# fwereade/trivy

Measured on AMD Instinct MI355X. Metric: packages matched/sec (node), higher is better.
Workload: dtype u8; 1 GPU; c2-dpkg-10000x400; packages=4000000, packages_rank0=4000000, matches_rank0=20482442, kernel_variant=fused_k4_m2400_wseg_rec_r16, db_keys=150005, db_advisories=1709707

## Files before the change

### include/trivy_amd.h

```cpp
#ifndef TRIVY_AMD_H
#define TRIVY_AMD_H

#include <stddef.h>
#include <stdint.h>

#ifdef __cplusplus
extern "C" {
#endif

#define TVM_ABI_VERSION 1

enum {
  TVM_OK = 0,
  TVM_EDETECT = 1,
  TVM_EUNSUPPORTED_OS = 2,
  TVM_EINVAL = 3,
  TVM_EDEVICE = 4,
  TVM_EUNSUPPORTED_TYPE = 5,
};

typedef struct tvm_db tvm_db;
typedef struct tvm_engine tvm_engine;
typedef struct tvm_batch tvm_batch;

typedef struct {
  const char* p;
  size_t n;
} tvm_str;

typedef struct {
  tvm_str id, name, version, release, arch;
  int64_t epoch;
  tvm_str src_name, src_version, src_release;
  int64_t src_epoch;
  tvm_str modularitylabel;
  int32_t has_build_info;
  const tvm_str* content_sets;
  size_t n_content_sets;
  tvm_str nvr, build_arch;
  tvm_str file_path;
} tvm_package;

typedef struct {
  tvm_str family, release;
} tvm_repository;

enum {
  TVM_COPY_PKG_ID = 1,
  TVM_COPY_PKG_NAME = 2,
  TVM_COPY_IDENTIFIER = 4,
  TVM_COPY_LAYER = 8,
};

typedef struct {
  uint32_t pkg_index;
  uint32_t copy_flags;
  const char* vulnerability_id;
  const char* const* vendor_ids;
  size_t n_vendor_ids;
  const char* pkg_id;
  const char* pkg_name;
  const char* pkg_path;
  const char* installed_version;
  const char* fixed_version;
  int32_t status;
  const char* severity_source;
  const char* severity;
  int32_t has_data_source;
  const char* data_source_id;
  const char* data_source_name;
  const char* data_source_url;
  const char* custom_json;
} tvm_vuln;

typedef struct {
  tvm_vuln* vulns;
  size_t n;
  int32_t eosl;
  void* priv;
} tvm_result;

const char* tvm_version(void);
int tvm_abi_version(void);

tvm_db* tvm_db_new(void);
void tvm_db_free(tvm_db* db);
int tvm_db_put(tvm_db* db, const tvm_str* path, size_t depth, const char* value, size_t vlen);
int tvm_db_put_many(tvm_db* db, size_t n, const tvm_str* paths, size_t depth, const tvm_str* values);
int tvm_db_put_arena(tvm_db* db, size_t n, size_t depth, const char* arena, const uint64_t* off,
                     const uint32_t* len);
int tvm_db_put_bbolt(tvm_db* db, const void* bytes, size_t len, char* err, size_t errlen);
typedef int (*tvm_bbolt_visit)(void* ctx, const tvm_str* path, size_t depth, const char* value, size_t vlen);
int tvm_bbolt_walk(const void* bytes, size_t len, tvm_bbolt_visit visit, void* ctx, char* err, size_t errlen);
int tvm_db_finalize(tvm_db* db, char* err, size_t errlen);
void tvm_db_stats(const tvm_db* db, uint64_t out[5]);
void tvm_db_layout_stats(const tvm_db* db, uint64_t out[6]);
void tvm_db_row16_stats(const tvm_db* db, uint64_t out[10]);
int tvm_row16_eval_host(const tvm_db* db, const char* bucket, const char* name, size_t name_len, const char* version,
                        size_t version_len, uint8_t* path, uint8_t* result, size_t cap);
int tvm_row16_pair_host(const uint8_t* key, size_t key_len, int valid, uint64_t pfx, uint32_t row_adv, uint32_t row_tail,
                        uint64_t row_head, int lex);

tvm_engine* tvm_engine_open(tvm_db* db, int device, char* err, size_t errlen);
void tvm_engine_close(tvm_engine* e);
int tvm_engine_swap(tvm_engine* e, tvm_db* db, char* err, size_t errlen);
uint64_t tvm_engine_table_bytes(const tvm_engine* e);
int tvm_engine_dropin_stats(tvm_engine* e, uint64_t* out3);
int tvm_engine_verify(tvm_engine* e, char* err, size_t errlen);
int tvm_engine_set_variant(tvm_engine* e, int v);
const char* tvm_variant_name(int v);
int tvm_variant_grammar_sets(int v);
int tvm_engine_last_variant(tvm_engine* e);

int tvm_ospkg_detect(tvm_engine* e, const char* os_family, const char* os_name, const tvm_repository* repo,
                     const tvm_package* pkgs, size_t n, int64_t now_unix, tvm_result* out, char* err,
                     size_t errlen);
int tvm_ospkg_driver_detect(tvm_engine* e, const char* os_family, const char* os_ver, const tvm_repository* repo,
                            const tvm_package* pkgs, size_t n, int64_t now_unix, tvm_result* out, char* err,
                            size_t errlen);
int tvm_ospkg_is_supported(const char* os_family, const char* os_ver, int64_t now_unix);
void tvm_result_free(tvm_result* r);

const char* tvm_library_type(const char* lib_type);
int tvm_library_detect(tvm_engine* e, const char* lib_type, const tvm_package* pkgs, size_t n, tvm_result* out,
                       char* err, size_t errlen);
int tvm_library_detect_vulnerabilities(tvm_engine* e, const char* lib_type, tvm_str pkg_id, tvm_str pkg_name,
                                       tvm_str pkg_ver, tvm_result* out, char* err, size_t errlen);

tvm_batch* tvm_batch_new(void);
void tvm_batch_free(tvm_batch* b);
int64_t tvm_batch_add(tvm_batch* b, tvm_engine* e, const char* bucket, tvm_str name, tvm_str version);
enum { TVM_ATTR_ARCH = 1, TVM_ATTR_KSPLICE = 2, TVM_ATTR_CPESET = 4 };
int64_t tvm_batch_add_many_ex(tvm_batch* b, tvm_engine* e, const char* bucket, size_t n, const char* arena,
                              const uint64_t* name_off, const uint32_t* name_len, const uint64_t* ver_off,
                              const uint32_t* ver_len, const uint64_t* arch_off, const uint32_t* arch_len,
                              uint32_t flags);
int64_t tvm_batch_cpe_set(tvm_batch* b, tvm_engine* e, const tvm_str* content_sets, size_t n, tvm_str nvr);
typedef struct {
  const uint64_t* arch_off;
  const uint32_t* arch_len;
  const uint32_t* cpe_set;
} tvm_attr_cols;
int64_t tvm_batch_add_many_attrs(tvm_batch* b, tvm_engine* e, const char* bucket, size_t n, const char* arena,
                                 const uint64_t* name_off, const uint32_t* name_len, const uint64_t* ver_off,
                                 const uint32_t* ver_len, const tvm_attr_cols* attrs, uint32_t flags);
int64_t tvm_batch_add_many(tvm_batch* b, tvm_engine* e, const char* bucket, size_t n, const char* arena,
                           const uint64_t* name_off, const uint32_t* name_len, const uint64_t* ver_off,
                           const uint32_t* ver_len);
int64_t tvm_batch_add_targets(tvm_batch* b, tvm_engine* e, size_t n_targets, const tvm_str* buckets,
                              const uint64_t* target_end, const char* arena, const uint64_t* name_off,
                              const uint32_t* name_len, const uint64_t* ver_off, const uint32_t* ver_len);
int64_t tvm_batch_add_targets_attrs(tvm_batch* b, tvm_engine* e, size_t n_targets, const tvm_str* buckets,
                                    const uint32_t* target_flags, const uint64_t* target_end, const char* arena,
                                    const uint64_t* name_off, const uint32_t* name_len, const uint64_t* ver_off,
                                    const uint32_t* ver_len, const tvm_attr_cols* attrs);
int64_t tvm_batch_size(const tvm_batch* b);
int tvm_batch_upload(tvm_engine* e, tvm_batch* b, uint64_t match_cap, char* err, size_t errlen);
int tvm_match_launch(tvm_engine* e, tvm_batch* b, char* err, size_t errlen);
int tvm_engine_sync(tvm_engine* e, char* err, size_t errlen);
int tvm_device_sync(int device, char* err, size_t errlen);
void tvm_shutdown(void);
int tvm_match_status(tvm_engine* e, tvm_batch* b, uint64_t* n_matches, int64_t* err_pkg, uint64_t* err_bits);
int tvm_match_fetch(tvm_engine* e, tvm_batch* b, uint32_t* pairs, uint64_t cap, uint64_t* n_out);
int tvm_match_copy_device(tvm_engine* e, tvm_batch* b, void* dst, uint64_t cap, uint64_t* n_out);
int tvm_match_order_into(tvm_engine* e, tvm_batch* b, void* csr_adv_dev, void* row_end_dev, uint64_t cap,
                         uint64_t* n_out, char* err, size_t errlen);
int tvm_match_time(tvm_engine* e, tvm_batch* b, int steps, double* ms, char* err, size_t errlen);
uint64_t tvm_match_algorithmic_bytes(tvm_engine* e, tvm_batch* b);
int tvm_version_key(int grammar, const char* s, size_t n, uint8_t* out, size_t cap);
int tvm_version_class(int grammar, const char* s, size_t n);
int tvm_deb_fast_key_host(const char* s, size_t n, uint32_t shift, uint8_t* out, size_t cap);
int tvm_deb_fast_key_slot_host(const char* s, size_t n, uint32_t shift, uint8_t* kb, size_t kb_len);
int tvm_enc_bal_buckets_host(void);
int tvm_enc_bal_bucket_host(uint32_t version_len);
int tvm_enc_bal_item_host(const uint32_t* counts, uint32_t item, uint32_t* bucket, uint32_t* index);
enum { TVM_ISVULN_PAIRWISE = 0x100 };
int tvm_lib_is_vulnerable_host(int grammar, const char* ver, size_t ver_len, const char* advisory_json,
                               size_t json_len);
const char* tvm_db_advisory_vuln_id(const tvm_db* db, uint32_t adv);

int tvm_db_rows_many(const tvm_db* db, const char* bucket, size_t n, const char* arena, const uint64_t* name_off,
                     const uint32_t* name_len, uint32_t* out);
int tvm_batch_set_package_base(tvm_batch* b, uint32_t base);
int tvm_batch_upload_into(tvm_engine* e, tvm_batch* b, void* pkg_dev, void* adv_dev, uint64_t cap, char* err,
                          size_t errlen);

enum { TVM_PIPE_RAW = 1, TVM_PIPE_ADV32 = 2, TVM_PIPE_RH_MERGE = 4 };
int tvm_pipeline_prepare(tvm_engine* e, tvm_batch* b, uint64_t match_cap, uint32_t chunk_packages, uint32_t flags,
                         char* err, size_t errlen);
int tvm_pipeline_run(tvm_engine* e, tvm_batch* b, uint64_t* n_matches, int64_t* err_pkg, double* ms, char* err,
                     size_t errlen);
int tvm_pipeline_result(tvm_batch* b, const uint32_t** adv, const uint32_t** row_end, uint64_t* n_matches);
int tvm_pipeline_result_raw(tvm_batch* b, const void** adv, uint32_t* width, const uint32_t** row_end,
                            uint64_t* n_matches);
int tvm_pipeline_stats(tvm_batch* b, uint64_t out[5]);
int tvm_wire_encode(size_t n, const uint32_t* plat, const char* arena, const uint64_t* name_off, const uint32_t* name_len,
                    const uint64_t* ver_off, const uint32_t* ver_len, uint32_t chunk_packages, int threads, void* out,
                    uint64_t cap, uint64_t* bytes,
                    uint64_t* chunks, uint64_t chunks_cap, uint64_t* n_chunks, uint32_t* plats, uint32_t plats_cap,
                    uint32_t* n_plats);
int tvm_pipeline_times(tvm_batch* b, uint64_t* encode_us, uint64_t* prepare_us);
void tvm_pool_stats(uint64_t out[4]);
void tvm_pool_trim(void);
int tvm_runtime_info(int* hip_runtime, int* hip_driver, char* path, size_t pathlen);

typedef struct tvm_sbom tvm_sbom;
enum { TVM_SBOM_BORROW = 1 };
int tvm_sbom_decode_cyclonedx(const char* text, size_t len, uint32_t flags, tvm_sbom** out, char* err, size_t errlen);
void tvm_sbom_free(tvm_sbom* s);
int tvm_sbom_info(const tvm_sbom* s, int32_t* has_os, tvm_str* os_family, tvm_str* os_name, tvm_str* serial,
                  int64_t* version, size_t* n_apps);
int tvm_sbom_packages(const tvm_sbom* s, int64_t app, tvm_str* type, tvm_str* file_path, const tvm_package** pkgs,
                      size_t* n);
typedef struct {
  tvm_str purl, bom_ref, layer_digest, layer_diff_id;
  uint32_t present;
} tvm_sbom_extra;
int tvm_sbom_package_extra(const tvm_sbom* s, int64_t app, size_t i, tvm_sbom_extra* out);

int tvm_match_redhat_result(tvm_engine* e, tvm_batch* b, tvm_result* out, char* err, size_t errlen);
int tvm_match_redhat_merge(tvm_engine* e, tvm_batch* b, char* err, size_t errlen);
int tvm_match_redhat_vulns(tvm_engine* e, tvm_batch* b, const uint32_t* pairs, uint64_t n, tvm_result* out,
                           char* err, size_t errlen);
int tvm_match_redhat_merge_time(tvm_engine* e, tvm_batch* b, int steps, double* ms, char* err, size_t errlen);

typedef struct {
  const uint32_t* row_end;
  size_t n_pkgs;
  uint32_t first_pkg;
  const uint8_t* rec;
  uint32_t rec_width;
  size_t n;
  const tvm_vuln* adv_recs;
  size_t n_adv_recs;
  const tvm_vuln* grp_recs;
  size_t n_grp_recs;
  void* priv;
} tvm_vuln_set;
int tvm_match_vulns(tvm_engine* e, tvm_batch* b, tvm_vuln_set* out, char* err, size_t errlen);
int tvm_pipeline_vulns(tvm_engine* e, tvm_batch* b, tvm_vuln_set* out, char* err, size_t errlen);
void tvm_vuln_set_free(tvm_vuln_set* s);
int tvm_vuln_set_walk(const tvm_vuln_set* s, const tvm_batch* b, uint64_t* n_out, uint64_t* digest);
int tvm_batch_report_get(const tvm_batch* b, uint64_t first, uint64_t n, tvm_str* names, tvm_str* versions,
                         tvm_str* paths);

typedef struct {
  tvm_str vulnerability_id;
  tvm_str data_source_id;
  tvm_str severity_source;
  tvm_str severity;
  int32_t status;
  int32_t has_fixed_version;
} tvm_fill_in;
typedef struct {
  int32_t found;
  int32_t status;
  const char* severity;
  const char* severity_source;
  const char* primary_url;
  const char* vulnerability_json;
} tvm_fill_out;
typedef struct {
  tvm_fill_out* items;
  size_t n;
  void* priv;
} tvm_fill_result;
int tvm_fill_info(tvm_engine* e, const tvm_fill_in* in, size_t n, tvm_fill_result* out, char* err, size_t errlen);
void tvm_fill_result_free(tvm_fill_result* r);
int tvm_match_fill(tvm_engine* e, tvm_batch* b, char* err, size_t errlen);
int tvm_match_fill_fetch(tvm_engine* e, tvm_batch* b, uint32_t* out4, uint64_t cap, uint64_t* n_out);
int tvm_match_fill_time(tvm_engine* e, tvm_batch* b, int steps, double* ms, char* err, size_t errlen);
uint64_t tvm_match_fill_algorithmic_bytes(tvm_engine* e, tvm_batch* b);
const char* tvm_fill_source_name(tvm_engine* e, uint32_t id);

int tvm_batch_set_report(tvm_batch* b, uint64_t first, uint64_t n, const tvm_str* names, const tvm_str* versions,
                         const tvm_str* paths);

typedef struct {
  const tvm_str* ids;
  size_t n_ids;
  const uint32_t* id_ranks;
  const uint32_t* all_id;
  const uint32_t* all_prec;
  size_t n_all;
  const uint32_t* pkg_pkg;
  const uint32_t* pkg_id;
  const uint32_t* pkg_prec;
  size_t n_pkg;
  const uint32_t* pkg_class;
  const uint32_t* cls_class;
  const uint32_t* cls_id;
  const uint32_t* cls_prec;
  size_t n_cls;
} tvm_ignore_rules;

typedef struct {
  uint32_t severity_mask;
  uint32_t ignore_status_mask;
  const tvm_ignore_rules* ignore;
  const uint32_t* vex_pkgs;
  const uint32_t* vex_id_index;
  size_t n_vex;
  const tvm_str* vex_ids;
  size_t n_vex_ids;
  const uint32_t* vex_id_ranks;
} tvm_filter_opts;
int tvm_vuln_rank_many(tvm_engine* e, const tvm_str* ids, size_t n, uint32_t* ranks);
int tvm_match_filter(tvm_engine* e, tvm_batch* b, const tvm_filter_opts* o, uint64_t* n_kept, uint64_t* n_ignored,
                     char* err, size_t errlen);
int tvm_match_filter_fetch(tvm_engine* e, tvm_batch* b, uint32_t* pairs, uint64_t cap, uint64_t* n_out);
int tvm_match_filter_ignored(tvm_engine* e, tvm_batch* b, uint32_t* triples, uint64_t cap, uint64_t* n_out);
int tvm_match_filter_time(tvm_engine* e, tvm_batch* b, const tvm_filter_opts* o, int steps, double* ms, char* err,
                          size_t errlen);

int tvm_pipeline_set_filter(tvm_engine* e, tvm_batch* b, const tvm_filter_opts* o, char* err, size_t errlen);
int tvm_pipeline_filter_stats(tvm_batch* b, uint64_t out[2]);

#ifdef __cplusplus
}
#endif
#endif
```

### trivy_amd/_lib.py

```python
import atexit
import ctypes
import os

_HERE = os.path.dirname(os.path.abspath(__file__))
LIB_PATH = os.environ.get("TVM_LIB_PATH") or os.path.join(_HERE, "libtrivy_amd.so")

TVM_OK, TVM_EDETECT, TVM_EUNSUPPORTED_OS, TVM_EINVAL, TVM_EDEVICE, TVM_EUNSUPPORTED_TYPE = 0, 1, 2, 3, 4, 5
COPY_PKG_ID, COPY_PKG_NAME, COPY_IDENTIFIER, COPY_LAYER = 1, 2, 4, 8


class Str(ctypes.Structure):
    _fields_ = [("p", ctypes.c_char_p), ("n", ctypes.c_size_t)]


class Package(ctypes.Structure):
    _fields_ = [
        ("id", Str), ("name", Str), ("version", Str), ("release", Str), ("arch", Str),
        ("epoch", ctypes.c_int64),
        ("src_name", Str), ("src_version", Str), ("src_release", Str),
        ("src_epoch", ctypes.c_int64),
        ("modularitylabel", Str),
        ("has_build_info", ctypes.c_int32),
        ("content_sets", ctypes.POINTER(Str)), ("n_content_sets", ctypes.c_size_t),
        ("nvr", Str), ("build_arch", Str),
        ("file_path", Str),
    ]


class RawStr(ctypes.Structure):
    _fields_ = [("p", ctypes.c_void_p), ("n", ctypes.c_size_t)]

    def bytes(self):
        return ctypes.string_at(self.p, self.n) if self.n else b""


class RawPackage(ctypes.Structure):
    _fields_ = [(n, RawStr if t is Str else t) for n, t in Package._fields_]


class SbomExtra(ctypes.Structure):
    _fields_ = [("purl", RawStr), ("bom_ref", RawStr), ("layer_digest", RawStr), ("layer_diff_id", RawStr),
                ("present", ctypes.c_uint32)]


class Repository(ctypes.Structure):
    _fields_ = [("family", Str), ("release", Str)]


class Vuln(ctypes.Structure):
    _fields_ = [
        ("pkg_index", ctypes.c_uint32), ("copy_flags", ctypes.c_uint32),
        ("vulnerability_id", ctypes.c_char_p),
        ("vendor_ids", ctypes.POINTER(ctypes.c_char_p)), ("n_vendor_ids", ctypes.c_size_t),
        ("pkg_id", ctypes.c_char_p), ("pkg_name", ctypes.c_char_p), ("pkg_path", ctypes.c_char_p),
        ("installed_version", ctypes.c_char_p), ("fixed_version", ctypes.c_char_p),
        ("status", ctypes.c_int32),
        ("severity_source", ctypes.c_char_p), ("severity", ctypes.c_char_p),
        ("has_data_source", ctypes.c_int32),
        ("data_source_id", ctypes.c_char_p), ("data_source_name", ctypes.c_char_p),
        ("data_source_url", ctypes.c_char_p),
        ("custom_json", ctypes.c_char_p),
    ]


class VulnSet(ctypes.Structure):
    _fields_ = [("row_end", ctypes.POINTER(ctypes.c_uint32)), ("n_pkgs", ctypes.c_size_t),
                ("first_pkg", ctypes.c_uint32), ("rec", ctypes.c_void_p), ("rec_width", ctypes.c_uint32),
                ("n", ctypes.c_size_t), ("adv_recs", ctypes.POINTER(Vuln)), ("n_adv_recs", ctypes.c_size_t),
                ("grp_recs", ctypes.POINTER(Vuln)), ("n_grp_recs", ctypes.c_size_t), ("priv", ctypes.c_void_p)]


class AttrCols(ctypes.Structure):
    _fields_ = [("arch_off", ctypes.c_void_p), ("arch_len", ctypes.c_void_p), ("cpe_set", ctypes.c_void_p)]


class Result(ctypes.Structure):
    _fields_ = [("vulns", ctypes.POINTER(Vuln)), ("n", ctypes.c_size_t), ("eosl", ctypes.c_int32),
                ("priv", ctypes.c_void_p)]


class FillIn(ctypes.Structure):
    _fields_ = [("vulnerability_id", Str), ("data_source_id", Str), ("severity_source", Str), ("severity", Str),
                ("status", ctypes.c_int32), ("has_fixed_version", ctypes.c_int32)]


class FillOut(ctypes.Structure):
    _fields_ = [("found", ctypes.c_int32), ("status", ctypes.c_int32), ("severity", ctypes.c_char_p),
                ("severity_source", ctypes.c_char_p), ("primary_url", ctypes.c_char_p),
                ("vulnerability_json", ctypes.c_char_p)]


class FillResult(ctypes.Structure):
    _fields_ = [("items", ctypes.POINTER(FillOut)), ("n", ctypes.c_size_t), ("priv", ctypes.c_void_p)]


class IgnoreRulesC(ctypes.Structure):
    _fields_ = [("ids", ctypes.POINTER(Str)), ("n_ids", ctypes.c_size_t), ("id_ranks", ctypes.c_void_p),
                ("all_id", ctypes.c_void_p), ("all_prec", ctypes.c_void_p), ("n_all", ctypes.c_size_t),
                ("pkg_pkg", ctypes.c_void_p), ("pkg_id", ctypes.c_void_p), ("pkg_prec", ctypes.c_void_p),
                ("n_pkg", ctypes.c_size_t), ("pkg_class", ctypes.c_void_p),
                ("cls_class", ctypes.c_void_p), ("cls_id", ctypes.c_void_p), ("cls_prec", ctypes.c_void_p),
                ("n_cls", ctypes.c_size_t)]


class FilterOpts(ctypes.Structure):
    _fields_ = [("severity_mask", ctypes.c_uint32), ("ignore_status_mask", ctypes.c_uint32),
                ("ignore", ctypes.POINTER(IgnoreRulesC)),
                ("vex_pkgs", ctypes.c_void_p), ("vex_id_index", ctypes.c_void_p), ("n_vex", ctypes.c_size_t),
                ("vex_ids", ctypes.POINTER(Str)), ("n_vex_ids", ctypes.c_size_t), ("vex_id_ranks", ctypes.c_void_p)]


_P = ctypes.c_void_p
_SIG = [
    ("tvm_version", ctypes.c_char_p, []),
    ("tvm_abi_version", ctypes.c_int, []),
    ("tvm_db_new", _P, []),
    ("tvm_db_free", None, [_P]),
    ("tvm_db_put", ctypes.c_int, [_P, ctypes.POINTER(Str), ctypes.c_size_t, ctypes.c_char_p, ctypes.c_size_t]),
    ("tvm_db_put_many", ctypes.c_int, [_P, ctypes.c_size_t, ctypes.c_void_p, ctypes.c_size_t, ctypes.c_void_p]),
    ("tvm_db_put_bbolt", ctypes.c_int, [_P, ctypes.c_char_p, ctypes.c_size_t, ctypes.c_char_p, ctypes.c_size_t]),
    ("tvm_bbolt_walk", ctypes.c_int, [ctypes.c_char_p, ctypes.c_size_t, ctypes.c_void_p, ctypes.c_void_p,
                                      ctypes.c_char_p, ctypes.c_size_t]),
    ("tvm_db_put_arena", ctypes.c_int, [_P, ctypes.c_size_t, ctypes.c_size_t, ctypes.c_void_p, ctypes.c_void_p,
                                        ctypes.c_void_p]),
    ("tvm_db_finalize", ctypes.c_int, [_P, ctypes.c_char_p, ctypes.c_size_t]),
    ("tvm_db_stats", None, [_P, ctypes.POINTER(ctypes.c_uint64)]),
    ("tvm_db_layout_stats", None, [_P, ctypes.POINTER(ctypes.c_uint64)]),
    ("tvm_db_row16_stats", None, [_P, ctypes.POINTER(ctypes.c_uint64)]),
    ("tvm_row16_eval_host", ctypes.c_int, [_P, ctypes.c_char_p, ctypes.c_char_p, ctypes.c_size_t, ctypes.c_char_p,
                                           ctypes.c_size_t, ctypes.c_void_p, ctypes.c_void_p, ctypes.c_size_t]),
    ("tvm_row16_pair_host", ctypes.c_int, [ctypes.c_char_p, ctypes.c_size_t, ctypes.c_int, ctypes.c_uint64, ctypes.c_uint32,
                                           ctypes.c_uint32, ctypes.c_uint64, ctypes.c_int]),
    ("tvm_engine_open", _P, [_P, ctypes.c_int, ctypes.c_char_p, ctypes.c_size_t]),
    ("tvm_engine_close", None, [_P]),
    ("tvm_engine_swap", ctypes.c_int, [_P, _P, ctypes.c_char_p, ctypes.c_size_t]),
    ("tvm_engine_table_bytes", ctypes.c_uint64, [_P]),
    ("tvm_engine_verify", ctypes.c_int, [_P, ctypes.c_char_p, ctypes.c_size_t]),
    ("tvm_engine_set_variant", ctypes.c_int, [_P, ctypes.c_int]),
    ("tvm_variant_name", ctypes.c_char_p, [ctypes.c_int]),
    ("tvm_variant_grammar_sets", ctypes.c_int, [ctypes.c_int]),
    ("tvm_engine_last_variant", ctypes.c_int, [_P]),
    ("tvm_ospkg_detect", ctypes.c_int, [_P, ctypes.c_char_p, ctypes.c_char_p, ctypes.POINTER(Repository),
                                        ctypes.POINTER(Package), ctypes.c_size_t, ctypes.c_int64,
                                        ctypes.POINTER(Result), ctypes.c_char_p, ctypes.c_size_t]),
    ("tvm_ospkg_driver_detect", ctypes.c_int, [_P, ctypes.c_char_p, ctypes.c_char_p, ctypes.POINTER(Repository),
                                               ctypes.POINTER(Package), ctypes.c_size_t, ctypes.c_int64,
                                               ctypes.POINTER(Result), ctypes.c_char_p, ctypes.c_size_t]),
    ("tvm_ospkg_is_supported", ctypes.c_int, [ctypes.c_char_p, ctypes.c_char_p, ctypes.c_int64]),
    ("tvm_result_free", None, [ctypes.POINTER(Result)]),
    ("tvm_batch_new", _P, []),
    ("tvm_batch_free", None, [_P]),
    ("tvm_batch_add", ctypes.c_int64, [_P, _P, ctypes.c_char_p, Str, Str]),
    ("tvm_batch_add_many", ctypes.c_int64, [_P, _P, ctypes.c_char_p, ctypes.c_size_t, ctypes.c_void_p,
                                             ctypes.c_void_p, ctypes.c_void_p, ctypes.c_void_p, ctypes.c_void_p]),
    ("tvm_batch_add_many_ex", ctypes.c_int64, [_P, _P, ctypes.c_char_p, ctypes.c_size_t, ctypes.c_char_p, ctypes.c_void_p,
                                               ctypes.c_void_p, ctypes.c_void_p, ctypes.c_void_p, ctypes.c_void_p,
                                               ctypes.c_void_p, ctypes.c_uint32]),
    ("tvm_batch_size", ctypes.c_int64, [_P]),
    ("tvm_batch_add_targets", ctypes.c_int64, [_P, _P, ctypes.c_size_t, ctypes.POINTER(Str), ctypes.c_void_p,
                                               ctypes.c_char_p, ctypes.c_void_p, ctypes.c_void_p, ctypes.c_void_p,
                                               ctypes.c_void_p]),
    ("tvm_batch_add_targets_attrs", ctypes.c_int64, [_P, _P, ctypes.c_size_t, ctypes.POINTER(Str), ctypes.c_void_p,
                                                     ctypes.c_void_p, ctypes.c_char_p, ctypes.c_void_p, ctypes.c_void_p,
                                                     ctypes.c_void_p, ctypes.c_void_p, ctypes.c_void_p]),
    ("tvm_batch_cpe_set", ctypes.c_int64, [_P, _P, ctypes.c_void_p, ctypes.c_size_t, Str]),
    ("tvm_batch_add_many_attrs", ctypes.c_int64, [_P, _P, ctypes.c_char_p, ctypes.c_size_t, ctypes.c_char_p,
                                                  ctypes.c_void_p, ctypes.c_void_p, ctypes.c_void_p, ctypes.c_void_p,
                                                  ctypes.c_void_p, ctypes.c_uint32]),
    ("tvm_match_redhat_result", ctypes.c_int, [_P, _P, ctypes.POINTER(Result), ctypes.c_char_p, ctypes.c_size_t]),
    ("tvm_match_redhat_merge", ctypes.c_int, [_P, _P, ctypes.c_char_p, ctypes.c_size_t]),
    ("tvm_match_redhat_merge_time", ctypes.c_int, [_P, _P, ctypes.c_int, ctypes.POINTER(ctypes.c_double),
                                                   ctypes.c_char_p, ctypes.c_size_t]),
    ("tvm_match_redhat_vulns", ctypes.c_int, [_P, _P, _P, ctypes.c_uint64, ctypes.POINTER(Result), ctypes.c_char_p,
                                              ctypes.c_size_t]),
    ("tvm_batch_upload", ctypes.c_int, [_P, _P, ctypes.c_uint64, ctypes.c_char_p, ctypes.c_size_t]),
    ("tvm_match_launch", ctypes.c_int, [_P, _P, ctypes.c_char_p, ctypes.c_size_t]),
    ("tvm_engine_sync", ctypes.c_int, [_P, ctypes.c_char_p, ctypes.c_size_t]),
    ("tvm_device_sync", ctypes.c_int, [ctypes.c_int, ctypes.c_char_p, ctypes.c_size_t]),
    ("tvm_shutdown", None, []),
    ("tvm_pipeline_times", ctypes.c_int, [_P, ctypes.POINTER(ctypes.c_uint64), ctypes.POINTER(ctypes.c_uint64)]),
    ("tvm_pool_stats", None, [ctypes.POINTER(ctypes.c_uint64)]),
    ("tvm_sbom_decode_cyclonedx", ctypes.c_int, [ctypes.c_void_p, ctypes.c_size_t, ctypes.c_uint32,
                                                 ctypes.POINTER(ctypes.c_void_p),
                                                 ctypes.c_char_p, ctypes.c_size_t]),
    ("tvm_sbom_free", None, [ctypes.c_void_p]),
    ("tvm_sbom_info", ctypes.c_int, [ctypes.c_void_p, ctypes.POINTER(ctypes.c_int32), ctypes.POINTER(RawStr),
                                     ctypes.POINTER(RawStr), ctypes.POINTER(RawStr), ctypes.POINTER(ctypes.c_int64),
                                     ctypes.POINTER(ctypes.c_size_t)]),
    ("tvm_sbom_packages", ctypes.c_int, [ctypes.c_void_p, ctypes.c_int64, ctypes.POINTER(RawStr), ctypes.POINTER(RawStr),
                                         ctypes.POINTER(ctypes.POINTER(RawPackage)), ctypes.POINTER(ctypes.c_size_t)]),
    ("tvm_sbom_package_extra", ctypes.c_int, [ctypes.c_void_p, ctypes.c_int64, ctypes.c_size_t,
                                              ctypes.POINTER(SbomExtra)]),
    ("tvm_wire_encode", ctypes.c_int, [ctypes.c_size_t, ctypes.c_void_p, ctypes.c_char_p, ctypes.c_void_p,
                                       ctypes.c_void_p, ctypes.c_void_p, ctypes.c_void_p,
                                       ctypes.c_uint32, ctypes.c_int, ctypes.c_void_p, ctypes.c_uint64,
                                       ctypes.POINTER(ctypes.c_uint64), ctypes.c_void_p, ctypes.c_uint64,
                                       ctypes.POINTER(ctypes.c_uint64), ctypes.c_void_p, ctypes.c_uint32,
                                       ctypes.POINTER(ctypes.c_uint32)]),
    ("tvm_pool_trim", None, []),
    ("tvm_match_status", ctypes.c_int, [_P, _P, ctypes.POINTER(ctypes.c_uint64), ctypes.POINTER(ctypes.c_int64),
                                        ctypes.POINTER(ctypes.c_uint64)]),
    ("tvm_match_fetch", ctypes.c_int, [_P, _P, ctypes.c_void_p, ctypes.c_uint64, ctypes.POINTER(ctypes.c_uint64)]),
    ("tvm_match_copy_device", ctypes.c_int, [_P, _P, ctypes.c_void_p, ctypes.c_uint64, ctypes.POINTER(ctypes.c_uint64)]),
    ("tvm_match_order_into", ctypes.c_int, [_P, _P, ctypes.c_void_p, ctypes.c_void_p, ctypes.c_uint64,
                                            ctypes.POINTER(ctypes.c_uint64), ctypes.c_char_p, ctypes.c_size_t]),
    ("tvm_match_time", ctypes.c_int, [_P, _P, ctypes.c_int, ctypes.POINTER(ctypes.c_double), ctypes.c_char_p,
                                      ctypes.c_size_t]),
    ("tvm_match_algorithmic_bytes", ctypes.c_uint64, [_P, _P]),
    ("tvm_db_rows_many", ctypes.c_int, [_P, ctypes.c_char_p, ctypes.c_size_t, ctypes.c_void_p, ctypes.c_void_p,
                                        ctypes.c_void_p, ctypes.c_void_p]),
    ("tvm_batch_set_package_base", ctypes.c_int, [_P, ctypes.c_uint32]),
    ("tvm_batch_upload_into", ctypes.c_int, [_P, _P, ctypes.c_void_p, ctypes.c_void_p, ctypes.c_uint64,
                                             ctypes.c_char_p, ctypes.c_size_t]),
    ("tvm_pipeline_prepare", ctypes.c_int, [_P, _P, ctypes.c_uint64, ctypes.c_uint32, ctypes.c_uint32, ctypes.c_char_p,
                                            ctypes.c_size_t]),
    ("tvm_pipeline_run", ctypes.c_int, [_P, _P, ctypes.POINTER(ctypes.c_uint64), ctypes.POINTER(ctypes.c_int64),
                                        ctypes.POINTER(ctypes.c_double), ctypes.c_char_p, ctypes.c_size_t]),
    ("tvm_pipeline_result", ctypes.c_int, [_P, ctypes.POINTER(ctypes.c_void_p), ctypes.POINTER(ctypes.c_void_p),
                                           ctypes.POINTER(ctypes.c_uint64)]),
    ("tvm_pipeline_result_raw", ctypes.c_int, [_P, ctypes.POINTER(ctypes.c_void_p), ctypes.POINTER(ctypes.c_uint32),
                                               ctypes.POINTER(ctypes.c_void_p), ctypes.POINTER(ctypes.c_uint64)]),
    ("tvm_pipeline_stats", ctypes.c_int, [_P, ctypes.POINTER(ctypes.c_uint64)]),
    ("tvm_version_key", ctypes.c_int, [ctypes.c_int, ctypes.c_char_p, ctypes.c_size_t, ctypes.c_void_p,
                                       ctypes.c_size_t]),
    ("tvm_engine_dropin_stats", ctypes.c_int, [_P, ctypes.POINTER(ctypes.c_uint64)]),
    ("tvm_deb_fast_key_host", ctypes.c_int, [ctypes.c_char_p, ctypes.c_size_t, ctypes.c_uint32, ctypes.c_void_p,
                                             ctypes.c_size_t]),
    ("tvm_deb_fast_key_slot_host", ctypes.c_int, [ctypes.c_char_p, ctypes.c_size_t, ctypes.c_uint32, ctypes.c_void_p,
                                                  ctypes.c_size_t]),
    ("tvm_enc_bal_buckets_host", ctypes.c_int, []),
    ("tvm_enc_bal_bucket_host", ctypes.c_int, [ctypes.c_uint32]),
    ("tvm_enc_bal_item_host", ctypes.c_int, [ctypes.POINTER(ctypes.c_uint32), ctypes.c_uint32,
                                             ctypes.POINTER(ctypes.c_uint32), ctypes.POINTER(ctypes.c_uint32)]),
    ("tvm_db_advisory_vuln_id", ctypes.c_char_p, [_P, ctypes.c_uint32]),
    ("tvm_version_class", ctypes.c_int, [ctypes.c_int, ctypes.c_char_p, ctypes.c_size_t]),
    ("tvm_lib_is_vulnerable_host", ctypes.c_int, [ctypes.c_int, ctypes.c_char_p, ctypes.c_size_t, ctypes.c_char_p,
                                                  ctypes.c_size_t]),
    ("tvm_library_type", ctypes.c_char_p, [ctypes.c_char_p]),
    ("tvm_library_detect", ctypes.c_int, [_P, ctypes.c_char_p, ctypes.POINTER(Package), ctypes.c_size_t,
                                          ctypes.POINTER(Result), ctypes.c_char_p, ctypes.c_size_t]),
    ("tvm_library_detect_vulnerabilities", ctypes.c_int, [_P, ctypes.c_char_p, Str, Str, Str, ctypes.POINTER(Result),
                                                          ctypes.c_char_p, ctypes.c_size_t]),
    ("tvm_fill_info", ctypes.c_int, [_P, ctypes.POINTER(FillIn), ctypes.c_size_t, ctypes.POINTER(FillResult),
                                     ctypes.c_char_p, ctypes.c_size_t]),
    ("tvm_fill_result_free", None, [ctypes.POINTER(FillResult)]),
    ("tvm_match_fill", ctypes.c_int, [_P, _P, ctypes.c_char_p, ctypes.c_size_t]),
    ("tvm_match_fill_fetch", ctypes.c_int, [_P, _P, ctypes.c_void_p, ctypes.c_uint64, ctypes.POINTER(ctypes.c_uint64)]),
    ("tvm_match_fill_time", ctypes.c_int, [_P, _P, ctypes.c_int, ctypes.POINTER(ctypes.c_double), ctypes.c_char_p,
                                           ctypes.c_size_t]),
    ("tvm_match_fill_algorithmic_bytes", ctypes.c_uint64, [_P, _P]),
    ("tvm_fill_source_name", ctypes.c_char_p, [_P, ctypes.c_uint32]),
    ("tvm_match_filter", ctypes.c_int, [_P, _P, ctypes.POINTER(FilterOpts), ctypes.POINTER(ctypes.c_uint64),
                                        ctypes.POINTER(ctypes.c_uint64), ctypes.c_char_p, ctypes.c_size_t]),
    ("tvm_match_filter_fetch", ctypes.c_int, [_P, _P, ctypes.c_void_p, ctypes.c_uint64,
                                              ctypes.POINTER(ctypes.c_uint64)]),
    ("tvm_match_filter_ignored", ctypes.c_int, [_P, _P, ctypes.c_void_p, ctypes.c_uint64,
                                                ctypes.POINTER(ctypes.c_uint64)]),
    ("tvm_vuln_rank_many", ctypes.c_int, [_P, ctypes.POINTER(Str), ctypes.c_size_t, ctypes.c_void_p]),
    ("tvm_batch_set_report", ctypes.c_int, [_P, ctypes.c_uint64, ctypes.c_uint64, ctypes.POINTER(Str),
                                            ctypes.POINTER(Str), ctypes.POINTER(Str)]),
    ("tvm_match_vulns", ctypes.c_int, [_P, _P, ctypes.POINTER(VulnSet), ctypes.c_char_p, ctypes.c_size_t]),
    ("tvm_runtime_info", ctypes.c_int, [ctypes.c_void_p, ctypes.c_void_p, ctypes.c_char_p, ctypes.c_size_t]),
    ("tvm_vuln_set_walk", ctypes.c_int, [ctypes.POINTER(VulnSet), _P, ctypes.c_void_p, ctypes.c_void_p]),
    ("tvm_pipeline_vulns", ctypes.c_int, [_P, _P, ctypes.POINTER(VulnSet), ctypes.c_char_p, ctypes.c_size_t]),
    ("tvm_vuln_set_free", None, [ctypes.POINTER(VulnSet)]),
    ("tvm_batch_report_get", ctypes.c_int, [_P, ctypes.c_uint64, ctypes.c_uint64, ctypes.POINTER(RawStr),
                                            ctypes.POINTER(RawStr), ctypes.POINTER(RawStr)]),
    ("tvm_match_filter_time", ctypes.c_int, [_P, _P, ctypes.POINTER(FilterOpts), ctypes.c_int,
                                             ctypes.POINTER(ctypes.c_double), ctypes.c_char_p, ctypes.c_size_t]),
    ("tvm_pipeline_set_filter", ctypes.c_int, [_P, _P, ctypes.POINTER(FilterOpts), ctypes.c_char_p, ctypes.c_size_t]),
    ("tvm_pipeline_filter_stats", ctypes.c_int, [_P, ctypes.POINTER(ctypes.c_uint64)]),
]

EXPORTED = [s[0] for s in _SIG]

_lib = None


def lib():
    global _lib
    if _lib is None:
        if not os.path.exists(LIB_PATH):
            raise RuntimeError(f"trivy_amd native library not built: {LIB_PATH} (run __graft_entry__.build())")
        L = ctypes.CDLL(LIB_PATH)
        for name, res, args in _SIG:
            f = getattr(L, name)
            f.restype = res
            f.argtypes = args
        _lib = L
        atexit.register(L.tvm_shutdown)
    return _lib


def s(x):
    if x is None:
        return Str(None, 0)
    b = x.encode() if isinstance(x, str) else bytes(x)
    st = Str(b, len(b))
    st._keep = b
    return st


def errbuf():
    return ctypes.create_string_buffer(4096)


def runtime_info():
    rt, drv, path = ctypes.c_int(), ctypes.c_int(), ctypes.create_string_buffer(1024)
    lib().tvm_runtime_info(ctypes.byref(rt), ctypes.byref(drv), path, len(path))
    fmt = lambda v: f"{v // 10_000_000}.{v // 100_000 % 100}.{v % 100_000}"
    return {"hip_runtime": fmt(rt.value), "hip_driver": fmt(drv.value), "libamdhip64": path.value.decode()}
```

### trivy_amd/csrc/capi.cpp

```cpp
#include "../../include/trivy_amd.h"

#include <dlfcn.h>

#include <algorithm>
#include <atomic>
#include <chrono>
#include <cstdio>
#include <cstring>
#include <deque>
#include <memory>
#include <mutex>
#include <new>
#include <shared_mutex>
#include <string>
#include <unordered_map>
#include <vector>

#include "db.h"
#include "drivers.h"
#include "export.h"
#include "engine.h"
#include "libdb.h"
#include "libver.h"
#include "bbolt.h"
// ... 321 lines not shown
      if (!(r.hi_len & KEY_INF)) {
        const int c = key_cmp(kw.data(), kl, d.key_words.data() + o.hi_off, r.hi_len & KEY_LEN_MASK);
        m = (r.hi_len & KEY_INCL) ? c <= 0 : c < 0;
      }
      if (m && !(r.lo_len & KEY_INF)) {
        const int c = key_cmp(kw.data(), kl, d.key_words.data() + o.lo_off, r.lo_len & KEY_LEN_MASK);
        m = (r.lo_len & KEY_INCL) ? c >= 0 : c > 0;
      }
      m = (m && valid) || (r.adv & ROW_ALWAYS);
    }
    if (path) path[i] = (h.tail & 0xFFu) == R16_FALLBACK ? 2 : slow ? 1 : 0;
    if (result) result[i] = m ? 1 : 0;
  }
  return int(cnt);
}

int tvm_row16_pair_host(const uint8_t* key, size_t key_len, int valid, uint64_t pfx, uint32_t row_adv, uint32_t row_tail,
                        uint64_t row_head, int lex) {
  if ((!key && key_len) || key_len > 0x3FFF) return -1;
  uint64_t k[3] = {0, 0, 0};
  for (size_t i = 0; i < key_len && i < 24; i++) k[i / 8] |= uint64_t(key[i]) << (8 * (7 - i % 8));
  const uint32_t kl = valid ? uint32_t(key_len) : 0u, P = uint32_t(pfx) & 0xFFu;
  if (!valid) k[0] = k[1] = k[2] = 0;
  Row16 r;
  r.adv = row_adv;
  r.tail = row_tail;
  r.head = row_head;
  uint64_t ph;
  uint32_t pt;
  bool slow = false, m;
  if (lex) {
    row16_pkg_lex(k[0], k[1], k[2], kl, P, row16_prefix_cmp(k[0], kl, pfx), valid != 0, ph, pt);
    m = row16_test_lex(ph, pt, r, slow);
  } else {
    row16_pkg(k[0], k[1], k[2], kl, P, row16_prefix_cmp(k[0], kl, pfx), valid != 0, ph, pt);
    m = row16_test(ph, pt, r, slow);
  }
  return (m ? 1 : 0) | (slow ? 2 : 0);
}

const char* tvm_db_advisory_vuln_id(const tvm_db* db, uint32_t adv) {
  return adv < db->db.advs.size() ? db->db.advs[adv].vuln_id.c_str() : nullptr;
}

static std::atomic<uint64_t> g_used_devices{0};

tvm_engine* tvm_engine_open(tvm_db* db, int device, char* err, size_t errlen) {
  if (device >= 0 && device < 64) g_used_devices.fetch_or(uint64_t(1) << device);
  if (!db || !db->finalized) {
    set_err(err, errlen, "tvm_engine_open: DB not finalized");
    return nullptr;
  }
  std::string e;
  Engine* eng = Engine::open(db->db, device, e);
  if (!eng) {
    set_err(err, errlen, e);
    return nullptr;
  }
  FillEngine* fill = FillEngine::open(db->vt, device, e);
  if (!fill) {
    delete eng;
    set_err(err, errlen, e);
    return nullptr;
  }
  auto* t = new tvm_engine();
  t->eng.reset(eng);
  t->fill.reset(fill);
  t->db = db;
  t->device = device;
  return t;
}

void tvm_engine_close(tvm_engine* e) { delete e; }

void tvm_shutdown(void) {
  const uint64_t used = g_used_devices.load();
  for (int d = 0; d < 64; d++)
    if ((used >> d) & 1u)
      if (hipSetDevice(d) == hipSuccess) (void)hipDeviceSynchronize();
  WorkerPool::shutdown_all();
  release_encoders();
  pool_close();
}

int tvm_device_sync(int device, char* err, size_t errlen) {
  int ndev = 0;
  if (hipGetDeviceCount(&ndev) != hipSuccess || device < 0 || device >= ndev) {
    set_err(err, errlen, "tvm_device_sync: no such HIP device");
    return TVM_EDEVICE;
  }
  (void)hipSetDevice(device);
  hipError_t st = hipDeviceSynchronize();
  if (st == hipSuccess) st = hipGetLastError();
  if (st != hipSuccess) {
    set_err(err, errlen, std::string("tvm_device_sync: ") + hipGetErrorString(st));
    return TVM_EDEVICE;
  }
  return TVM_OK;
}

int tvm_engine_swap(tvm_engine* e, tvm_db* db, char* err, size_t errlen) {
  if (!e || !db || !db->finalized) return TVM_EINVAL;
  std::string msg;
  Engine* fresh = Engine::open(db->db, e->device, msg);
  FillEngine* fresh_fill = fresh ? FillEngine::open(db->vt, e->device, msg) : nullptr;
  if (!fresh || !fresh_fill) {
    delete fresh;
    set_err(err, errlen, msg);
    return TVM_EDEVICE;
  }
  std::unique_lock<std::shared_mutex> lk(e->mu);
  (void)hipSetDevice(e->device);
  e->eng.reset(fresh);
  e->fill.reset(fresh_fill);
  e->db = db;
  e->gen++;
  if (e->rh_rank) {
    (void)hipFree(e->rh_rank);
    e->rh_rank = nullptr;
  }
  if (e->cls) {
    (void)hipFree(e->cls);
    e->cls = nullptr;
  }
  return TVM_OK;
}

uint64_t tvm_engine_table_bytes(const tvm_engine* e) { return e ? e->eng->table_bytes() : 0; }

int tvm_engine_dropin_stats(tvm_engine* e, uint64_t* out3) {
  if (!e || !out3) return TVM_EINVAL;
  std::shared_lock<std::shared_mutex> lk(e->mu);
  e->eng->dropin_stats(out3);
  return TVM_OK;
}

int tvm_engine_verify(tvm_engine* e, char* err, size_t errlen) {
  if (!e) return TVM_EINVAL;
  std::unique_lock<std::shared_mutex> lk(e->mu);
  std::string msg;
  if (!e->eng->verify(msg)) {
    set_err(err, errlen, msg);
    return TVM_EDEVICE;
  }
  return TVM_OK;
}

int tvm_engine_set_variant(tvm_engine* e, int v) {
  if (!e) return -1;
  std::unique_lock<std::shared_mutex> lk(e->mu);
  return v < 0 ? e->eng->variant() : e->eng->set_variant(v);
}

const char* tvm_variant_name(int v) { return variant_name(v); }
int tvm_variant_grammar_sets(int v) { return variant_grammar_sets(v); }

int tvm_engine_last_variant(tvm_engine* e) {
  if (!e) return -1;
  std::shared_lock<std::shared_mutex> lk(e->mu);
  return e->eng->last_launched();
}

static int detect_common(tvm_engine* e, bool full, const char* fam, const char* ver, const tvm_repository* repo,
                         const tvm_package* pkgs, size_t n, int64_t now, tvm_result* out, char* err,
                         size_t errlen) {
  if (!e || !fam || !ver || !out || (n && !pkgs)) return TVM_EINVAL;
  memset(out, 0, sizeof(*out));
  std::shared_lock<std::shared_mutex> lk(e->mu);
  std::vector<Pkg> p = to_pkgs(pkgs, n);
  Repo r;
  if (repo) {
    r.family = sv(repo->family);
    r.release = sv(repo->release);
  }
  std::vector<Vuln> vulns;
  std::string msg;
  bool eosl = false;
  if (full) {
    DetectStatus st = ospkg_detect(*e->eng, fam, ver, repo ? &r : nullptr, p, now, vulns, eosl, msg);
    if (st != DETECT_OK) {
      set_err(err, errlen, msg);
      return st == DETECT_UNSUPPORTED_OS ? TVM_EUNSUPPORTED_OS : TVM_EDETECT;
    }
  } else {
    const OsDriver* d = find_os_driver(fam);
    if (!d) {
      set_err(err, errlen, "unsupported os");
      return TVM_EUNSUPPORTED_OS;
    }
    if (!d->detect(*e->eng, ver, repo ? &r : nullptr, p, now, vulns, msg)) {
      set_err(err, errlen, msg);
      return TVM_EDETECT;
    }
  }
  export_result(e->eng->db(), std::move(vulns), eosl, out);
  return TVM_OK;
}

int tvm_ospkg_detect(tvm_engine* e, const char* f, const char* v, const tvm_repository* repo, const tvm_package* pkgs,
                     size_t n, int64_t now, tvm_result* out, char* err, size_t errlen) {
  return detect_common(e, true, f, v, repo, pkgs, n, now, out, err, errlen);
}

int tvm_ospkg_driver_detect(tvm_engine* e, const char* f, const char* v, const tvm_repository* repo,
                            const tvm_package* pkgs, size_t n, int64_t now, tvm_result* out, char* err,
                            size_t errlen) {
  return detect_common(e, false, f, v, repo, pkgs, n, now, out, err, errlen);
}

int tvm_ospkg_is_supported(const char* fam, const char* ver, int64_t now) {
  const OsDriver* d = fam ? find_os_driver(fam) : nullptr;
  if (!d || !ver) return -1;
  return d->is_supported(fam, ver, now) ? 1 : 0;
}

void tvm_result_free(tvm_result* r) {
  if (!r) return;
  delete static_cast<ResultStore*>(r->priv);
  memset(r, 0, sizeof(*r));
}


tvm_batch* tvm_batch_new(void) { return new tvm_batch(); }

void tvm_batch_free(tvm_batch* b) {
  if (!b) return;
  b->pipe.reset();
  if (b->order_scratch) {
    (void)hipSetDevice(b->device);
    (void)hipFree(b->order_scratch);
  }
  if (b->uploaded) {
    (void)hipSetDevice(b->device);
    for (void* p : {static_cast<void*>(b->dev.pk), static_cast<void*>(b->dev.tile_off), static_cast<void*>(b->dev.arena),
                    static_cast<void*>(b->dev.attr), static_cast<void*>(b->dev.cpe_bits), static_cast<void*>(b->dev.rec),
                    static_cast<void*>(b->dev.tail), static_cast<void*>(b->dev.spill),
                    static_cast<void*>(b->external_out ? nullptr : b->m.pkg),
                    static_cast<void*>(b->external_out ? nullptr : b->m.adv), static_cast<void*>(b->m.dir),
                    static_cast<void*>(b->m.ctl),
                    static_cast<void*>(b->fill_out)})
      if (p) (void)hipFree(p);
  }
  delete b;
}

static void reserve_more(HostBatch& hb, size_t n) {
  const size_t want = hb.pk.size() + n;
  if (want > hb.pk.capacity()) hb.pk.reserve(std::max(want, 2 * hb.pk.capacity()));
}

int64_t tvm_batch_add(tvm_batch* b, tvm_engine* e, const char* bucket, tvm_str name, tvm_str version) {
  if (!b || !e || !bucket || b->uploaded || b->pinned) return -1;
  std::shared_lock<std::shared_mutex> lk(e->mu);
  if (!bind(b, e)) return -1;
  b->target_begin.push_back(uint32_t(b->hb.pk.size()));
  int32_t plat = e->eng->db().find_plat(bucket);
  b->hb.add(plat < 0 ? 0xFFFFFFFFu : uint32_t(plat), sv(name), sv(version));
  return int64_t(b->hb.pk.size() - 1);
}

int64_t tvm_batch_add_many(tvm_batch* b, tvm_engine* e, const char* bucket, size_t n, const char* arena,
                           const uint64_t* name_off, const uint32_t* name_len, const uint64_t* ver_off,
                           const uint32_t* ver_len) {
  if (!b || !e || !bucket || b->uploaded || b->pinned ||
      (n && (!arena || !name_off || !name_len || !ver_off || !ver_len)))
    return -1;
  std::shared_lock<std::shared_mutex> lk(e->mu);
  if (!bind(b, e)) return -1;
  int32_t plat = e->eng->db().find_plat(bucket);
  const uint32_t pid = plat < 0 ? 0xFFFFFFFFu : uint32_t(plat);
  const int64_t first = int64_t(b->hb.pk.size());
  b->target_begin.push_back(uint32_t(first));
  reserve_more(b->hb, n);
  for (size_t i = 0; i < n; i++)
    b->hb.add(pid, std::string_view(arena + name_off[i], name_len[i]), std::string_view(arena + ver_off[i], ver_len[i]));
  return first;
}

int64_t tvm_batch_add_many_ex(tvm_batch* b, tvm_engine* e, const char* bucket, size_t n, const char* arena,
                              const uint64_t* name_off, const uint32_t* name_len, const uint64_t* ver_off,
                              const uint32_t* ver_len, const uint64_t* arch_off, const uint32_t* arch_len,
                              uint32_t flags) {
  if (flags & TVM_ATTR_CPESET) return -1;
  tvm_attr_cols cols{arch_off, arch_len, nullptr};
  return tvm_batch_add_many_attrs(b, e, bucket, n, arena, name_off, name_len, ver_off, ver_len, &cols, flags);
}

int64_t tvm_batch_cpe_set(tvm_batch* b, tvm_engine* e, const tvm_str* content_sets, size_t n, tvm_str nvr) {
  if (!b || !e || b->uploaded || b->pinned || (n && !content_sets)) return -1;
  std::shared_lock<std::shared_mutex> lk(e->mu);
  if (!bind(b, e)) return -1;
  const DB& db = e->eng->db();
  HostBatch& hb = b->hb;
  const uint32_t words = std::max<uint32_t>((db.n_cpe + 31) / 32, 1);
  if (hb.cpe_words == 0) hb.cpe_words = words;
  if (hb.cpe_words != words) return -1;
  std::vector<std::string_view> repos, nvrs;
  for (size_t i = 0; i < n; i++) repos.push_back(sv(content_sets[i]));
  nvrs.push_back(sv(nvr));
  const size_t id = hb.cpe_bits.size() / words;
  hb.cpe_bits.resize(hb.cpe_bits.size() + words, 0u);
  uint32_t* bits = hb.cpe_bits.data() + id * words;
  for (int64_t c : db.redhat_cpes(repos, nvrs))
    if (c >= 0 && uint64_t(c) < uint64_t(words) * 32) bits[c >> 5] |= 1u << (c & 31);
  return int64_t(id);
}

int64_t tvm_batch_add_many_attrs(tvm_batch* b, tvm_engine* e, const char* bucket, size_t n, const char* arena,
                                 const uint64_t* name_off, const uint32_t* name_len, const uint64_t* ver_off,
                                 const uint32_t* ver_len, const tvm_attr_cols* cols, uint32_t flags) {
  const uint32_t known = TVM_ATTR_ARCH | TVM_ATTR_KSPLICE | TVM_ATTR_CPESET;
  if (!b || !e || !bucket || b->uploaded || b->pinned || (flags & ~known) ||
      ((flags & TVM_ATTR_KSPLICE) && (flags & TVM_ATTR_CPESET)) ||
      (n && (!arena || !name_off || !name_len || !ver_off || !ver_len)) ||
      (n && (flags & (TVM_ATTR_ARCH | TVM_ATTR_CPESET)) && !cols) ||
      (n && (flags & TVM_ATTR_ARCH) && (!cols->arch_off || !cols->arch_len)) ||
      (n && (flags & TVM_ATTR_CPESET) && !cols->cpe_set))
    return -1;
  std::shared_lock<std::shared_mutex> lk(e->mu);
  if (!bind(b, e)) return -1;
  const DB& db = e->eng->db();
  const size_t n_sets = b->hb.cpe_words ? b->hb.cpe_bits.size() / b->hb.cpe_words : 0;
  if (flags & TVM_ATTR_CPESET)
    for (size_t i = 0; i < n; i++)
      if (cols->cpe_set[i] >= n_sets) return -1;
  int32_t plat = db.find_plat(bucket);
  const uint32_t pid = plat < 0 ? 0xFFFFFFFFu : uint32_t(plat);
  const int64_t first = int64_t(b->hb.pk.size());
  b->target_begin.push_back(uint32_t(first));
  reserve_more(b->hb, n);
  for (size_t i = 0; i < n; i++) {
    const std::string_view ver(arena + ver_off[i], ver_len[i]);
    uint2 a = make_uint2(PA_ARCH_NONE, 0xFFFFFFFFu);
    if (flags & TVM_ATTR_ARCH) {
      const std::string_view arch(arena + cols->arch_off[i], cols->arch_len[i]);
      a.x = db.arch_id(arch) | (arch == "noarch" ? PA_NOARCH : 0u);
    }
    if (flags & TVM_ATTR_KSPLICE) {
      const size_t dash = ver.find('-');
      a.y = db.ksplice_id(extract_ksplice(dash == std::string_view::npos ? std::string_view() : ver.substr(dash + 1)));
    }
    if (flags & TVM_ATTR_CPESET) a.y = cols->cpe_set[i];
    if (flags) b->hb.add(pid, std::string_view(arena + name_off[i], name_len[i]), ver, a);
    else b->hb.add(pid, std::string_view(arena + name_off[i], name_len[i]), ver);
  }
  return first;
}

static int64_t add_targets_bulk(tvm_batch* b, tvm_engine* e, size_t n_targets, const tvm_str* buckets,
                                const uint32_t* tflags, const uint64_t* target_end, const char* arena,
                                const uint64_t* name_off, const uint32_t* name_len, const uint64_t* ver_off,
                                const uint32_t* ver_len, const tvm_attr_cols* cols) {
  const uint32_t known = TVM_ATTR_ARCH | TVM_ATTR_KSPLICE | TVM_ATTR_CPESET;
  if (!b || !e || b->uploaded || b->pinned || (n_targets && (!buckets || !target_end))) return -1;
  const uint64_t n = n_targets ? target_end[n_targets - 1] : 0;
  if (n && (!arena || !name_off || !name_len || !ver_off || !ver_len)) return -1;
  uint32_t any_flags = 0;
  for (size_t t = 0; t < n_targets; t++) {
    if (t && target_end[t] < target_end[t - 1]) return -1;
    const uint32_t f = tflags ? tflags[t] : 0u;
    if ((f & ~known) || ((f & TVM_ATTR_KSPLICE) && (f & TVM_ATTR_CPESET))) return -1;
    any_flags |= f;
  }
  if (((any_flags & TVM_ATTR_ARCH) && (!cols || !cols->arch_off || !cols->arch_len)) ||
      ((any_flags & TVM_ATTR_CPESET) && (!cols || !cols->cpe_set)))
    return -1;
  std::shared_lock<std::shared_mutex> lk(e->mu);
  if (!bind(b, e)) return -1;
  const DB& db = e->eng->db();
  HostBatch& hb = b->hb;
  const uint64_t s0 = hb.pk.size(), a0 = hb.arena.size();
  if (s0 + n >= (uint64_t(1) << 32)) return -1;
  std::vector<uint32_t> pid(n_targets);
  std::string_view last_bucket;
  uint32_t last_pid = 0xFFFFFFFFu;
  for (size_t t = 0; t < n_targets; t++) {
    const std::string_view bk = sv(buckets[t]);
    if (t == 0 || bk != last_bucket) {
      const int32_t plat = db.find_plat(bk);
      last_pid = plat < 0 ? 0xFFFFFFFFu : uint32_t(plat);
      last_bucket = bk;
    }
    pid[t] = last_pid;
  }
  const size_t n_sets = hb.cpe_words ? hb.cpe_bits.size() / hb.cpe_words : 0;
  WorkerPool& wp = WorkerPool::get();
  const size_t K = n ? std::min<size_t>(size_t(wp.size()) * 8, std::max<uint64_t>(1, n / 4096)) : 0;
  auto piece = [&](size_t k) { return std::make_pair(n * k / K, n * (k + 1) / K); };
  auto target_of = [&](uint64_t j) {
// ... 254 lines not shown
  oa.pkg_base = b->dev.pkg_base;
  if (hipMemsetAsync(b->order_scratch, 0, size_t(nt + 1) * 8, st) != hipSuccess) return TVM_EDEVICE;
  launch_order(nt, st, oa);
  const hipError_t le = hipGetLastError();
  const hipError_t se = le == hipSuccess ? hipStreamSynchronize(st) : le;
  if (se != hipSuccess) {
    set_err(err, errlen, std::string("order kernel: ") + hipGetErrorString(se));
    return TVM_EDEVICE;
  }
  return TVM_OK;
}

int tvm_match_time(tvm_engine* e, tvm_batch* b, int steps, double* ms, char* err, size_t errlen) {
  if (!e || !b || !b->uploaded || steps <= 0 || !ms) return TVM_EINVAL;
  std::shared_lock<std::shared_mutex> lk(e->mu);
  if (!bind(b, e)) {
    set_err(err, errlen, kStale);
    return TVM_EINVAL;
  }
  (void)hipSetDevice(e->device);
  hipEvent_t t0 = nullptr, t1 = nullptr;
  hipStream_t st = e->eng->stream();
  std::string msg;
  int rc = TVM_OK;
  if (hipEventCreate(&t0) != hipSuccess || hipEventCreate(&t1) != hipSuccess || hipEventRecord(t0, st) != hipSuccess) {
    msg = "hipEvent setup failed";
    rc = TVM_EDEVICE;
  }
  b->merged = false;
  b->st_valid = false;
  for (int i = 0; rc == TVM_OK && i < steps; i++)
    if (!e->eng->launch(b->dev, b->m, st, msg)) rc = TVM_EDEVICE;
  float f = 0;
  if (rc == TVM_OK && (hipEventRecord(t1, st) != hipSuccess || hipEventSynchronize(t1) != hipSuccess ||
                       hipEventElapsedTime(&f, t0, t1) != hipSuccess)) {
    msg = "hipEvent timing failed";
    rc = TVM_EDEVICE;
  }
  if (t0) (void)hipEventDestroy(t0);
  if (t1) (void)hipEventDestroy(t1);
  if (rc != TVM_OK) {
    set_err(err, errlen, msg);
    return rc;
  }
  *ms = f;
  return TVM_OK;
}

uint64_t tvm_match_algorithmic_bytes(tvm_engine* e, tvm_batch* b) {
  if (!e || !b) return 0;
  const DB& db = e->eng->db();
  uint64_t bytes = 0, off = 0;
  for (const uint2& d : b->hb.pk) {
    const uint32_t nlen = d.y & 0xFFFF, vlen = d.y >> 16;
    const std::string_view name(reinterpret_cast<const char*>(b->hb.arena.data()) + off, nlen);
    off += nlen + vlen;
    bytes += 8 + nlen + vlen;
    if (d.x >= db.plats.size()) continue;
    bytes += 24;
    int32_t k = db.find_key(d.x, name);
    if (k < 0) continue;
    bytes += nlen;
    const std::string ks = db.keys[size_t(k)].name;
    uint64_t h = pkg_key_hash(d.x, reinterpret_cast<const uint8_t*>(ks.data()), uint32_t(ks.size()));
    for (uint64_t i = h & db.slot_mask; db.slot_hash[i]; i = (i + 1) & db.slot_mask) {
      if (db.slot_key[i] != uint32_t(k)) continue;
      const SlotVal& v = db.slot_val[i];
      uint32_t cls = 0;
      if (v.name_len & SLOT_CLS_SPLIT) {
        struct Sink {
          void put(uint8_t) {}
        } sk;
        const char* ver = name.data() + nlen;
        if (!encode_version_cls(db.plat_info[d.x].cmp, reinterpret_cast<const uint8_t*>(ver), vlen, sk, cls)) cls = 0;
      }
      const uint2 rr = slot_rows(v.name_len, v.row_begin, v.row_count, cls);
      for (uint32_t r = 0; r < rr.y; r++) {
        const Row& row = db.rows[rr.x + r];
        bytes += sizeof(Row);
        if (!(row.hi_len & KEY_INF) && (row.hi_len & KEY_LEN_MASK) > 16) bytes += (row.hi_len & KEY_LEN_MASK) - 16;
        if (!(row.lo_len & KEY_INF)) bytes += row.lo_len & KEY_LEN_MASK;
      }
      break;
    }
  }
  uint64_t m = 0;
  if (b->uploaded) tvm_match_status(e, b, &m, nullptr, nullptr);
  return bytes + 8 * m;
}

int tvm_version_key(int grammar, const char* s, size_t n, uint8_t* out, size_t cap) {
  struct Sink {
    uint8_t* o;
    size_t cap, n = 0;
    void put(uint8_t b) {
      if (n < cap) o[n] = b;
      n++;
    }
  } sink{out, cap};
  if (grammar <= 0 || grammar > 255 || !s) return -1;
  uint32_t cls = 0;
  if (!encode_version_cls(uint8_t(grammar), reinterpret_cast<const uint8_t*>(s), uint32_t(n), sink, cls)) return -1;
  return int(sink.n);
}

int tvm_version_class(int grammar, const char* s, size_t n) {
  struct Sink {
    void put(uint8_t) {}
  } sink;
  uint32_t cls = 0;
  if (grammar <= 0 || grammar > 255 || !s) return -1;
  if (!encode_version_cls(uint8_t(grammar), reinterpret_cast<const uint8_t*>(s), uint32_t(n), sink, cls)) return -1;
  return int(cls);
}

int tvm_deb_fast_key_host(const char* s, size_t n, uint32_t shift, uint8_t* out, size_t cap) {
  if (!s || n > 4096 || shift > 3) return -3;
  uint8_t tab[128];
  for (uint32_t c = 0; c < 128; c++) tab[c] = deb_fast_code(c);
  std::vector<uint32_t> buf((shift + n) / 4 + 4, 0xA5A5A5A5u);
  uint8_t* b = reinterpret_cast<uint8_t*>(buf.data()) + shift;
  std::memcpy(b, s, n);
  uint8_t kb[kFastKeyStride];
  std::memset(kb, 0xEE, sizeof kb);
  uint32_t len = 0;
  const uint32_t st = deb_fast_key(b, uint32_t(n), kb, tab, len);
  if (st == FAST_INVALID) return -1;
  if (st == FAST_FALLBACK) return -2;
  for (uint32_t i = 0; i < len && i < cap; i++) out[i] = kb[i];
  return int(len);
}

int tvm_deb_fast_key_slot_host(const char* s, size_t n, uint32_t shift, uint8_t* kb, size_t kb_len) {
  if (!s || !kb || n > 4096 || shift > 3 || kb_len < kFastKeyStride) return -3;
  uint8_t tab[128];
  for (uint32_t c = 0; c < 128; c++) tab[c] = deb_fast_code(c);
  std::vector<uint32_t> buf((shift + n) / 4 + 4, 0xA5A5A5A5u);
  uint8_t* b = reinterpret_cast<uint8_t*>(buf.data()) + shift;
  std::memcpy(b, s, n);
  uint32_t len = 0;
  const uint32_t st = deb_fast_key(b, uint32_t(n), kb, tab, len);
  return st == FAST_INVALID ? -1 : st == FAST_FALLBACK ? -2 : int(len);
}

int tvm_enc_bal_buckets_host(void) { return int(kEncBuckets); }
int tvm_enc_bal_bucket_host(uint32_t version_len) { return int(enc_bal_bucket(version_len)); }
int tvm_enc_bal_item_host(const uint32_t* counts, uint32_t item, uint32_t* bucket, uint32_t* index) {
  if (!counts || !bucket || !index) return -1;
  uint32_t b = 0, i = 0;
  if (!enc_bal_item(counts, item, b, i)) return 0;
  *bucket = b;
  *index = i;
  return 1;
}

int tvm_lib_is_vulnerable_host(int grammar, const char* ver, size_t ver_len, const char* advisory_json,
                               size_t json_len) {
  Advisory a;
  std::string e;
  if (!ver || !advisory_json || !decode_advisory(std::string_view(advisory_json, json_len), a, e)) return -1;
  const bool pairwise = (grammar & TVM_ISVULN_PAIRWISE) != 0;
  grammar &= ~TVM_ISVULN_PAIRWISE;
  if (grammar == CMP_MAVEN && (pairwise || !mvn_hybrid(a.vulnerable, a.patched, a.unaffected)))
    return mvn_is_vulnerable(a.vulnerable, a.patched, a.unaffected, std::string(ver, ver_len));
  const LibRows r = lib_compile_advisory(uint8_t(grammar), a.vulnerable, a.patched, a.unaffected);
  return lib_rows_contain(uint8_t(grammar), r, std::string(ver, ver_len)) ? 1 : 0;
}

int tvm_library_detect(tvm_engine* e, const char* lib_type, const tvm_package* pkgs, size_t n, tvm_result* out,
                       char* err, size_t errlen) {
  if (!e || !lib_type || !out || (n && !pkgs)) return TVM_EINVAL;
  memset(out, 0, sizeof(*out));
  std::shared_lock<std::shared_mutex> lk(e->mu);
  std::vector<Pkg> p = to_pkgs(pkgs, n);
  std::vector<Vuln> vulns;
  std::string msg;
  const DetectStatus st = library_detect(*e->eng, lib_type, p, vulns, msg);
  if (st == DETECT_UNSUPPORTED_OS) return TVM_EUNSUPPORTED_TYPE;
  if (st != DETECT_OK) {
    set_err(err, errlen, msg);
    return TVM_EDETECT;
  }
  export_result(e->eng->db(), std::move(vulns), false, out);
  return TVM_OK;
}

int tvm_library_detect_vulnerabilities(tvm_engine* e, const char* lib_type, tvm_str pkg_id, tvm_str pkg_name,
                                       tvm_str pkg_ver, tvm_result* out, char* err, size_t errlen) {
  if (!e || !lib_type || !out) return TVM_EINVAL;
  memset(out, 0, sizeof(*out));
  std::shared_lock<std::shared_mutex> lk(e->mu);
  std::vector<Pkg> p(1);
  p[0].id = sv(pkg_id);
  p[0].name = sv(pkg_name);
  p[0].version = sv(pkg_ver);
  std::vector<Vuln> vulns;
  std::string msg;
  const DetectStatus st = library_detect_vulnerabilities(*e->eng, lib_type, p, vulns, msg);
  if (st == DETECT_UNSUPPORTED_OS) return TVM_EUNSUPPORTED_TYPE;
  if (st != DETECT_OK) {
    set_err(err, errlen, msg);
    return TVM_EDETECT;
  }
  export_result(e->eng->db(), std::move(vulns), false, out);
  return TVM_OK;
}

const char* tvm_library_type(const char* lib_type) { return lib_type ? library_ecosystem(lib_type) : nullptr; }

}


namespace {

struct FillPriv {
  std::vector<tvm_fill_out> items;
  std::deque<std::string> strs;
};

}

int tvm_fill_info(tvm_engine* e, const tvm_fill_in* in, size_t n, tvm_fill_result* out, char* err, size_t errlen) {
  if (!e || !out || (n && !in)) return TVM_EINVAL;
  *out = tvm_fill_result{nullptr, 0, nullptr};
  std::shared_lock<std::shared_mutex> lk(e->mu);
  const VulnTable& vt = e->fill->table();
  std::vector<uint4> items(n);
  std::vector<uint8_t> arena;
  for (size_t i = 0; i < n; i++) {
    const tvm_fill_in& x = in[i];
    const size_t len = std::min<size_t>(x.vulnerability_id.n, 0xFFFF);
    const uint32_t src = vt.source_id(std::string_view(x.data_source_id.p ? x.data_source_id.p : "", x.data_source_id.n));
    uint4 it;
    it.x = uint32_t(arena.size());
    it.y = uint32_t(len) | (src << 16);
    it.z = uint32_t(x.status & 0xFF) | (x.has_fixed_version ? FI_FIXED : 0u) | (x.severity_source.n ? FI_SEV_SRC : 0u);
    it.w = FILL_NOT_FOUND;
    if (len) arena.insert(arena.end(), x.vulnerability_id.p, x.vulnerability_id.p + len);
    items[i] = it;
  }
  std::vector<uint4> dec;
  std::string msg;
  if (!e->fill->run_host(items, arena, dec, msg)) {
    set_err(err, errlen, msg);
    return TVM_EDEVICE;
  }
  auto* priv = new FillPriv();
  priv->items.resize(n);
  auto keep = [&](std::string s) -> const char* {
    priv->strs.push_back(std::move(s));
    return priv->strs.back().c_str();
  };
  for (size_t i = 0; i < n; i++) {
    const tvm_fill_in& x = in[i];
    const uint4 d = dec[i];
    tvm_fill_out& o = priv->items[i];
    o.status = int32_t(d.y);
    if (!x.has_fixed_version && x.status != 0 && (x.status & ~0xFF)) o.status = x.status;
    o.severity = o.severity_source = o.primary_url = "";
    o.vulnerability_json = nullptr;
    o.found = d.x != FILL_NOT_FOUND && x.vulnerability_id.n <= 0xFFFF;
    if (!o.found) continue;
    const uint32_t code = d.z & 0xFFFFu, ssrc = d.z >> 16;
    std::string_view extra_src;
    int64_t extra_val = 0;
    if (code == SEV_KEEP) {
      const std::string_view sev(x.severity.p ? x.severity.p : "", x.severity.n);
      extra_src = std::string_view(x.severity_source.p, x.severity_source.n);
      extra_val = fill_new_severity(sev);
      o.severity = keep(std::string(sev));
      o.severity_source = keep(std::string(extra_src));
    } else {
      o.severity = vt.severity_string(d.x, code).c_str();
      o.severity_source = ssrc == SRC_NONE ? "" : vt.source_name(ssrc).c_str();
    }
    o.primary_url = keep(vt.primary_url(d.x, d.w));
    o.vulnerability_json = keep(vt.vulnerability_json(d.x, o.severity, extra_src, extra_val));
  }
  out->items = priv->items.data();
  out->n = n;
  out->priv = priv;
  return TVM_OK;
}

void tvm_fill_result_free(tvm_fill_result* r) {
  if (!r) return;
  delete static_cast<FillPriv*>(r->priv);
  *r = tvm_fill_result{nullptr, 0, nullptr};
}

int tvm_match_fill(tvm_engine* e, tvm_batch* b, char* err, size_t errlen) {
  if (!e || !b || !b->uploaded) return TVM_EINVAL;
  std::shared_lock<std::shared_mutex> lk(e->mu);
  if (!bind(b, e)) {
    set_err(err, errlen, kStale);
    return TVM_EINVAL;
  }
  (void)hipSetDevice(e->device);
  const DevMatches& m = cur(b);
  if (b->fill_cap < m.cap) {
    if (b->fill_out) (void)hipFree(b->fill_out);
    b->fill_out = nullptr;
    b->fill_cap = 0;
    if (hipMalloc(&b->fill_out, std::max<uint64_t>(m.cap, 1) * (sizeof(uint4) + sizeof(uint2))) != hipSuccess) {
      set_err(err, errlen, "hipMalloc(fill decisions) failed");
      return TVM_EDEVICE;
// ... 1235 lines not shown
```

### trivy_amd/csrc/engine.h

```cpp
#pragma once
#include <hip/hip_runtime.h>

#include <atomic>
#include <memory>
#include <cstdint>
#include <mutex>
#include <string>
#include <string_view>
#include <utility>
#include <vector>

#include "common.h"

namespace tvm {

class DB;

constexpr int kTile = 256;
constexpr int kGroup = 64;
constexpr int kGroupsPerTile = kTile / kGroup;

struct DevDB {
  const Slot* slots = nullptr;
  const uint8_t* slot_fp = nullptr;
  uint64_t slot_mask = 0;
  const uint8_t* name_arena = nullptr;
  const Row* rows = nullptr;
  const RowOff* row_off = nullptr;
  const Row16* rows16 = nullptr;
  const uint64_t* key_words = nullptr;
  const PlatInfo* plats = nullptr;
  uint32_t n_plats = 0;
  const RowAux* aux = nullptr;
  const uint32_t* aux_ids = nullptr;
};

template <class T>
struct NoInitAlloc : std::allocator<T> {
  template <class U>
  struct rebind {
    using other = NoInitAlloc<U>;
  };
  NoInitAlloc() = default;
  template <class U>
  NoInitAlloc(const NoInitAlloc<U>&) noexcept {}
  template <class U>
  void construct(U* p) noexcept {
    ::new (static_cast<void*>(p)) U;
  }
  template <class U, class... A>
  void construct(U* p, A&&... a) {
    ::new (static_cast<void*>(p)) U(std::forward<A>(a)...);
  }
};
template <class T>
using BulkVec = std::vector<T, NoInitAlloc<T>>;

struct HostBatch {
  BulkVec<uint2> pk;
  BulkVec<uint8_t> arena;
  BulkVec<uint64_t> tile_off;
  BulkVec<uint2> attr;
  std::vector<uint32_t> cpe_bits;
  uint32_t cpe_words = 0;
  void add(uint32_t plat, std::string_view name, std::string_view ver);
  void add(uint32_t plat, std::string_view name, std::string_view ver, uint2 a);
  size_t size() const { return pk.size(); }
  uint32_t n_tiles() const { return uint32_t((pk.size() + kTile - 1) / kTile); }
  uint32_t n_groups() const { return uint32_t((pk.size() + kGroup - 1) / kGroup); }
  uint64_t name_off(size_t i) const;
  void name_offsets(std::vector<uint64_t>& off) const;
  std::string_view name(size_t i) const;
  std::string_view version(size_t i) const;
  void clear();
};

struct PkgRec {
  uint4 meta;
  uint64_t k0, k1, k2;
};

struct DevBatch {
  uint2* pk = nullptr;
  uint64_t* tile_off = nullptr;
  uint8_t* arena = nullptr;
  uint2* attr = nullptr;
  uint32_t* cpe_bits = nullptr;
  uint32_t cpe_words = 0;
  uint32_t n_cpe_sets = 0;
  uint32_t n = 0;
  uint32_t n_tiles = 0;
  uint64_t arena_bytes = 0;
  uint64_t spill_words = 0;
  uint32_t gm = 0;
  uint32_t pkg_base = 0;
  uint64_t* spill = nullptr;
  uint64_t spill_cap = 0;
  uint32_t* tile_map = nullptr;
  uint32_t n_lean_tiles = 0;
  PkgRec* rec = nullptr;
  uint4* tail = nullptr;
};

struct TileDir {
  unsigned long long base;
  uint32_t count;
  uint32_t pad;
};
struct DevMatches {
  uint32_t* pkg = nullptr;
  uint32_t* adv = nullptr;
  uint64_t cap = 0;
  TileDir* dir = nullptr;
  uint32_t dir_cap = 0;
  unsigned long long* ctl = nullptr;
  unsigned long long* ctl_next = nullptr;
  unsigned long long* ctl_mem = nullptr;
};
enum : uint32_t { ERR_SPILL = 1, ERR_TILES = 2, ERR_BOUNDS = 8 };

struct CopyOutArgs {
  const TileDir* dir = nullptr;
  const uint32_t* pkg = nullptr;
  const uint32_t* adv = nullptr;
  uint32_t* row_end_h = nullptr;
  uint32_t* adv_h = nullptr;
  unsigned long long* chunk_base = nullptr;
  uint32_t c = 0;
  uint32_t t0 = 0, t1 = 0;
  uint32_t pkg_base = 0;
  uint64_t cap = 0;
  uint32_t packed = 0;
  uint64_t adv_units = 0;
  uint64_t row_end_units = 0;
  unsigned long long* ctl = nullptr;
};
constexpr uint32_t kCopyRunMax = kTile;
constexpr uint32_t kCopyLdsWords = 2 * kCopyRunMax + 8 + (kTile / 64) * kTile;
constexpr uint32_t kCopyWorkgroups = 256;

__device__ __forceinline__ uint32_t copy_block_scan(uint32_t v, uint32_t* red, uint32_t tid, uint32_t& tot) {
  const uint32_t lane = tid & 63, wave = tid >> 6;
  uint32_t x = v;
#pragma unroll
  for (int o = 1; o < 64; o <<= 1) {
    const uint32_t y = __shfl_up(x, o, 64);
    if (lane >= uint32_t(o)) x += y;
  }
  __syncthreads();
  if (lane == 63) red[wave] = x;
  __syncthreads();
  uint32_t pre = 0;
  tot = 0;
#pragma unroll
  for (int w = 0; w < kTile / 64; w++) {
    const uint32_t r = red[w];
    pre += uint32_t(w) < wave ? r : 0u;
    tot += r;
  }
  return pre + x - v;
}

__device__ __forceinline__ uint32_t copy_block_sum(uint32_t v, uint32_t* red, uint32_t tid) {
#pragma unroll
  for (int o = 32; o > 0; o >>= 1) v += __shfl_xor(v, o, 64);
  __syncthreads();
  if ((tid & 63) == 0) red[tid >> 6] = v;
  __syncthreads();
  uint32_t s = 0;
#pragma unroll
  for (int w = 0; w < kTile / 64; w++) s += red[w];
  return s;
}

__device__ __forceinline__ void copy_out_tile_wave(const CopyOutArgs& a, uint32_t t, uint64_t b, uint32_t lane,
                                                   uint32_t* cw) {
  const TileDir d = a.dir[t];
  const bool fits = d.base + d.count <= a.cap && b + d.count <= a.cap;
  const uint32_t p_first = t * kTile;
  reinterpret_cast<uint4*>(cw)[lane] = make_uint4(0, 0, 0, 0);
  __builtin_amdgcn_fence(__ATOMIC_RELEASE, "wavefront");
  __builtin_amdgcn_wave_barrier();
  if (fits)
    for (uint32_t i0 = 0; i0 < d.count; i0 += 4 * 64) {
      uint32_t q[4];
#pragma unroll
      for (int u = 0; u < 4; u++) {
        const uint32_t i = i0 + u * 64 + lane;
        q[u] = i < d.count ? a.pkg[d.base + i] - a.pkg_base - p_first : kTile;
      }
#pragma unroll
      for (int u = 0; u < 4; u++)
        if (q[u] < kTile) atomicAdd(&cw[q[u]], 1u);
    }
  __builtin_amdgcn_fence(__ATOMIC_ACQ_REL, "wavefront");
  __builtin_amdgcn_wave_barrier();
  const uint4 c4 = reinterpret_cast<const uint4*>(cw)[lane];
  const uint32_t s0 = c4.x, s1 = s0 + c4.y, s2 = s1 + c4.z, s3 = s2 + c4.w;
  uint32_t x = s3;
#pragma unroll
  for (int o = 1; o < 64; o <<= 1) {
    const uint32_t y = __shfl_up(x, o, 64);
    if (lane >= uint32_t(o)) x += y;
  }
  const uint32_t e = uint32_t(b) + x - s3;
  if (p_first / 4 + lane < a.row_end_units)
    reinterpret_cast<uint4*>(a.row_end_h)[p_first / 4 + lane] = make_uint4(e + s0, e + s1, e + s2, e + s3);
  else
    atomicOr(a.ctl + 3, (unsigned long long)ERR_BOUNDS);
  if (a.packed) {
    const uint64_t B0 = 3 * b, B1 = 3 * (b + d.count), U0 = B0 >> 4;
    uint64_t nu = fits && d.count ? ((B1 + 15) >> 4) - U0 : 0;
    if (nu && U0 + nu > a.adv_units) {
      if (lane == 0) atomicOr(a.ctl + 3, (unsigned long long)ERR_BOUNDS);
      nu = 0;
    }
    uint8_t* dst = reinterpret_cast<uint8_t*>(a.adv_h);
    constexpr int kP = 2;
    for (uint64_t j0 = 0; j0 < nu; j0 += uint64_t(kP) * 64) {
      uint32_t id[kP][6];
#pragma unroll
      for (int k = 0; k < kP; k++) {
        const uint64_t j = j0 + uint64_t(k) * 64 + lane, g0 = ((U0 + j) * 16) / 3;
#pragma unroll
        for (int tt = 0; tt < 6; tt++) {
          const int64_t i = int64_t(g0 + tt) - int64_t(b);
          id[k][tt] = (j < nu && i >= 0 && i < int64_t(d.count)) ? a.adv[d.base + uint64_t(i)] : 0u;
        }
      }
#pragma unroll
      for (int k = 0; k < kP; k++) {
        const uint64_t j = j0 + uint64_t(k) * 64 + lane;
        if (j >= nu) continue;
        const uint64_t G0 = (U0 + j) * 16, g0 = G0 / 3;
        const uint32_t r = uint32_t(G0 - g0 * 3);
        uint32_t wv[4] = {0, 0, 0, 0};
#pragma unroll
        for (int q = 0; q < 16; q++) {
          const uint32_t tt = (r + q) / 3, kb = (r + q) % 3;
          wv[q >> 2] |= ((id[k][tt] >> (8 * kb)) & 0xFFu) << (8 * (q & 3));
        }
        if (G0 >= B0 && G0 + 16 <= B1) {
          reinterpret_cast<uint4*>(dst)[U0 + j] = make_uint4(wv[0], wv[1], wv[2], wv[3]);
        } else {
#pragma unroll
          for (int q = 0; q < 16; q++)
            if (G0 + q >= B0 && G0 + q < B1) dst[G0 + q] = uint8_t(wv[q >> 2] >> (8 * (q & 3)));
        }
      }
    }
    return;
  }
  const uint64_t u0 = b >> 2;
  uint64_t nu = fits && d.count ? ((b + d.count + 3) >> 2) - u0 : 0;
  if (nu && u0 + nu > a.adv_units) {
    if (lane == 0) atomicOr(a.ctl + 3, (unsigned long long)ERR_BOUNDS);
    nu = 0;
  }
  const uint32_t sh = uint32_t(b & 3);
  constexpr int kU = 4;
  for (uint64_t j0 = 0; j0 < nu; j0 += uint64_t(kU) * 64) {
    uint32_t v[kU][4];
#pragma unroll
    for (int k = 0; k < kU; k++) {
      const uint64_t j = j0 + uint64_t(k) * 64 + lane;
#pragma unroll
      for (int w = 0; w < 4; w++) {
        const int64_t i = int64_t(j * 4 + w) - int64_t(sh);
        v[k][w] = (j < nu && i >= 0 && i < int64_t(d.count)) ? a.adv[d.base + uint64_t(i)] : 0u;
      }
    }
#pragma unroll
    for (int k = 0; k < kU; k++) {
      const uint64_t j = j0 + uint64_t(k) * 64 + lane;
      if (j >= nu) continue;
      const int64_t i0 = int64_t(j * 4) - int64_t(sh);
      if (i0 >= 0 && i0 + 4 <= int64_t(d.count)) {
        reinterpret_cast<uint4*>(a.adv_h)[u0 + j] = make_uint4(v[k][0], v[k][1], v[k][2], v[k][3]);
      } else {
#pragma unroll
        for (int w = 0; w < 4; w++)
          if (i0 + w >= 0 && i0 + w < int64_t(d.count)) a.adv_h[(u0 + j) * 4 + w] = v[k][w];
      }
    }
  }
}

__device__ __forceinline__ void copy_out_tiles(const CopyOutArgs& a, uint32_t wg, uint32_t n_wg, uint32_t* lds) {
  unsigned long long* pre = reinterpret_cast<unsigned long long*>(lds);
  uint32_t* red = lds + 2 * kCopyRunMax;
  const uint32_t tid = threadIdx.x, lane = tid & 63, wave = tid >> 6;
  uint32_t* cw = red + 8 + wave * kTile;
  const uint32_t nt = a.t1 - a.t0;
  const uint32_t r0 = a.t0 + uint32_t(uint64_t(nt) * wg / n_wg), r1 = a.t0 + uint32_t(uint64_t(nt) * (wg + 1) / n_wg);
  uint32_t before = 0;
  for (uint32_t u = a.t0 + tid; u < r0; u += kTile) before += a.dir[u].count;
  unsigned long long b = a.chunk_base[a.c] + copy_block_sum(before, red, tid);
  for (uint32_t s0 = r0; s0 < r1; s0 += kCopyRunMax) {
    const uint32_t s1 = min(r1, s0 + kCopyRunMax);
    uint32_t tot;
    const uint32_t ex = copy_block_scan(s0 + tid < s1 ? a.dir[s0 + tid].count : 0u, red, tid, tot);
    pre[tid] = b + ex;
    __syncthreads();
    for (uint32_t t = s0 + wave; t < s1; t += kTile / 64) copy_out_tile_wave(a, t, pre[t - s0], lane, cw);
    b += tot;
    __syncthreads();
  }
  if (wg == n_wg - 1 && tid == 0) a.chunk_base[a.c + 1] = b;
}

class Engine {
 public:
  ~Engine();
  static Engine* open(const DB& db, int device, std::string& err);
  int device() const { return dev_; }
  hipStream_t stream() const { return stream_; }
  uint64_t table_bytes() const { return table_bytes_; }

  bool alloc_batch(const HostBatch& hb, DevBatch& b, std::string& err, bool pooled = false);
  bool upload(const HostBatch& hb, DevBatch& b, std::string& err);
  uint32_t grammar_set(const HostBatch& hb) const;
  uint64_t scratch_words(const HostBatch& hb) const;
  static void free_batch(int device, DevBatch& b, bool pooled = false);
  bool alloc_matches(uint64_t cap, uint32_t n_pkgs, DevMatches& m, std::string& err, bool pooled = false);
  static void free_matches(int device, DevMatches& m, bool pooled = false);

  bool launch(const DevBatch& b, DevMatches& m, hipStream_t stream, std::string& err);
  bool launch_tiles(const DevBatch& b, const DevMatches& m, uint32_t t_begin, uint32_t t_end, hipStream_t probe_st,
                    hipStream_t sweep_st, hipEvent_t ev, std::string& err, const CopyOutArgs* co = nullptr,
                    unsigned long long* ctl_zero = nullptr, const uint32_t* tmap = nullptr, uint32_t tmap_n = 0,
                    uint32_t gm = 0);

  static bool fetch_ordered(const DevMatches& m, uint32_t n_pkgs, uint64_t total, std::vector<uint2>& out,
                            hipStream_t st, std::string& err);

  bool match_host(const HostBatch& hb, std::vector<uint2>& out, int64_t& err_pkg, std::string& err);
  void dropin_stats(uint64_t out[3]);

  const DB& db() const { return *db_; }
  const PlatInfo* device_plats() const { return d_.plats; }

  int set_variant(int v);
  int last_launched() const { return last_launched_; }
  bool verify(std::string& err);
  int variant() const { return variant_; }

 private:
  int dev_ = 0;
  int variant_ = 0;
  std::atomic<int> last_launched_{-1};
  hipStream_t stream_ = nullptr;
  const DB* db_ = nullptr;
  DevDB d_;
  std::vector<void*> allocs_;
  uint64_t table_bytes_ = 0;
  struct Dropin;
  struct DropinReq;
  std::unique_ptr<Dropin> dropin_;
  std::mutex dropin_init_mu_;
  Dropin* dropin(std::string& err);
  bool dropin_run(Dropin& d, DropinReq* const* reqs, size_t n, std::string& err);
};

int num_variants();
const char* variant_name(int v);
int variant_grammar_sets(int v);
int resolve_variant(int v, uint32_t gm);

}
```

### trivy_amd/csrc/engine.hip

```cpp
#include "engine.h"
#include "host_par.h"
#include "pool.h"

#include <algorithm>
#include <mutex>
#include <memory>
#include <deque>
#include <condition_variable>
#include <cstdlib>
#include <cstring>

#include "db.h"
#include "match_kernel.h"
#include "match_variants.h"
#include "pipeline.h"

namespace tvm {

ProbeFn probe_fn_DEB();
#ifdef TVM_DIAG
ProbeFn probe_fn_DEB_diag(int d);
#endif
ProbeFn probe_fn_OS();
ProbeFn probe_fn_ALL();
// ... 20 lines not shown
constexpr int kNumVariants = 1 + kNumTuned;
constexpr bool kFusedVariant[] = {
#define TVM_F_(F, K, MB, NAME) F != 0,
    TVM_MATCH_VARIANTS(TVM_F_)
#undef TVM_F_
};

FusedFn fused_fn(uint32_t gm, int vi) {
  switch (grammar_index(gm)) {
    case 0: return fused_table_DEB()[vi - 1];
    case 1: return fused_table_OS()[vi - 1];
    case 3: return fused_table_LEAN()[vi - 1];
    default: return fused_table_ALL()[vi - 1];
  }
}


ProbeFn probe_fn(uint32_t gm) {
#ifdef TVM_DIAG
  static const int diag = std::getenv("TVM_PROBE_DIAG") ? std::atoi(std::getenv("TVM_PROBE_DIAG")) : 0;
  if (diag && grammar_index(gm) == 0) return probe_fn_DEB_diag(diag);
#endif
  switch (grammar_index(gm)) {
    case 0: return probe_fn_DEB();
    case 1: return probe_fn_OS();
    default: return probe_fn_ALL();
  }
}

bool hip_ok(hipError_t e, const char* what, std::string& err) {
  if (e == hipSuccess) return true;
  err = std::string(what) + ": " + hipGetErrorString(e);
  return false;
}

template <class T>
bool upload_vec(const std::vector<T>& v, T** dst, std::vector<void*>& allocs, uint64_t& bytes, std::string& err) {
  size_t n = std::max<size_t>(v.size(), 1) * sizeof(T);
  void* p = nullptr;
  if (!hip_ok(hipMalloc(&p, n), "hipMalloc(tables)", err)) return false;
  allocs.push_back(p);
  if (!v.empty() && !hip_ok(hipMemcpy(p, v.data(), v.size() * sizeof(T), hipMemcpyHostToDevice), "hipMemcpy(tables)", err))
    return false;
  bytes += n;
  *dst = static_cast<T*>(p);
  return true;
}

template <class T>
bool dmalloc(T** p, size_t count, const char* what, std::string& err, int pool_dev = -1) {
  void* q = nullptr;
  const size_t bytes = std::max<size_t>(count, 1) * sizeof(T);
  if (pool_dev >= 0) {
    q = pool_device_get(pool_dev, bytes, what, err);
    if (!q) return false;
  } else if (!hip_ok(hipMalloc(&q, bytes), what, err)) {
    return false;
  }
  *p = static_cast<T*>(q);
  return true;
}

void dfree(void* p, bool pooled, int device) {
  if (!p) return;
  if (pooled) pool_device_put(device, p);
  else (void)hipFree(p);
}

}

int num_variants() { return kNumVariants; }
const char* variant_name(int v) {
  if (v == 0) return "auto";
  return v > 0 && v < kNumVariants ? kVariantNames[v - 1] : nullptr;
}
int variant_grammar_sets(int v) {
  if (v == 0) return 15;
  if (v < 0 || v >= kNumVariants) return 0;
  if (!kFusedVariant[v - 1]) return 15;
  return (fused_table_DEB()[v - 1] ? 1 : 0) | (fused_table_OS()[v - 1] ? 2 : 0) | (fused_table_ALL()[v - 1] ? 4 : 0) |
         (fused_table_LEAN()[v - 1] ? 8 : 0);
}

int resolve_variant(int v, uint32_t gm) {
  if (v != 0) return v;
  const int gi = grammar_index(gm);
  return 1 + (gi == 0 ? kAutoVariant : gi == 1 ? kAutoVariantOS : gi == 3 ? kAutoVariantLean : kAutoVariantFiltered);
}


Engine::~Engine() {
  if (dev_ >= 0) (void)hipSetDevice(dev_);
  if (stream_) (void)hipStreamSynchronize(stream_);
  dropin_.reset();
  for (void* p : allocs_) (void)hipFree(p);
  if (stream_) (void)hipStreamDestroy(stream_);
}

Engine* Engine::open(const DB& db, int device, std::string& err) {
  int ndev = 0;
  if (hipGetDeviceCount(&ndev) != hipSuccess || ndev == 0) {
    err = "no HIP device available (trivy_amd requires an MI355X / gfx950 GPU)";
    return nullptr;
  }
  if (device < 0 || device >= ndev) {
    err = "invalid HIP device index";
    return nullptr;
  }
  Engine* e = new Engine();
  e->dev_ = device;
  e->db_ = &db;
  if (const char* v = std::getenv("TVM_VARIANT")) e->set_variant(std::atoi(v));
  if (!hip_ok(hipSetDevice(device), "hipSetDevice", err) ||
      !hip_ok(hipStreamCreateWithFlags(&e->stream_, hipStreamNonBlocking), "hipStreamCreate", err)) {
    delete e;
    return nullptr;
  }
  Slot* sl; uint8_t* fp; uint8_t* na; Row* rows; RowOff* ro; Row16* r16; uint64_t* kw; PlatInfo* pl; RowAux* ax; uint32_t* ai;
  bool ok = upload_vec(db.aux, &ax, e->allocs_, e->table_bytes_, err) &&
            upload_vec(db.aux_ids, &ai, e->allocs_, e->table_bytes_, err) &&
            upload_vec(db.slots, &sl, e->allocs_, e->table_bytes_, err) &&
            upload_vec(db.slot_fp, &fp, e->allocs_, e->table_bytes_, err) &&
            upload_vec(db.name_arena, &na, e->allocs_, e->table_bytes_, err) &&
            upload_vec(db.rows, &rows, e->allocs_, e->table_bytes_, err) &&
            upload_vec(db.row_off, &ro, e->allocs_, e->table_bytes_, err) &&
            upload_vec(db.rows16, &r16, e->allocs_, e->table_bytes_, err) &&
            upload_vec(db.key_words, &kw, e->allocs_, e->table_bytes_, err) &&
            upload_vec(db.plat_info, &pl, e->allocs_, e->table_bytes_, err);
  if (!ok) {
    delete e;
    return nullptr;
  }
  e->d_.slots = sl;
  e->d_.slot_fp = fp;
  e->d_.slot_mask = db.slot_mask;
  e->d_.name_arena = na;
  e->d_.rows = rows;
  e->d_.row_off = ro;
  e->d_.rows16 = r16;
  e->d_.key_words = kw;
  e->d_.plats = pl;
  e->d_.aux = ax;
  e->d_.aux_ids = ai;
  e->d_.n_plats = uint32_t(db.plats.size());
  return e;
}

int Engine::set_variant(int v) {
  const int old = variant_;
  if (v >= 0 && v < kNumVariants) variant_ = v;
  return old;
}

uint32_t Engine::grammar_set(const HostBatch& hb) const {
  const auto& pi = db_->plat_info;
  std::atomic<uint32_t> gm{0};
  range_for(hb.pk.size(), 1 << 18, [&](size_t a, size_t b) {
    uint32_t g = 0, last = 0xFFFFFFFFu;
    for (size_t i = a; i < b; i++) {
      const uint32_t p = hb.pk[i].x;
      if (p != last && p < pi.size()) g |= 1u << pi[p].cmp;
      last = p;
    }
    gm.fetch_or(g, std::memory_order_relaxed);
  });
  return gm.load() & GM_ALL;
}

uint64_t Engine::scratch_words(const HostBatch& hb) const {
  const auto& pi = db_->plat_info;
  std::atomic<uint64_t> total{0};
  range_for(hb.pk.size(), 1 << 18, [&](size_t a, size_t b) {
    uint64_t w = 0;
    for (size_t i = a; i < b; i++) {
      const uint2 d = hb.pk[i];
      const uint32_t vlen = d.y >> 16;
      const uint32_t need = (key_bound_any(vlen) + 7) / 8;
      const bool mvn = d.x < pi.size() && pi[d.x].cmp == CMP_MAVEN;
      if (need > (mvn ? 2u : kKeyWords)) w += need;
      if (mvn) w += (uint64_t(kMvnPackedWords) * std::min<uint32_t>(2 * vlen + 3, kMvnMaxTok) + 1) / 2;
    }
    total.fetch_add(w, std::memory_order_relaxed);
  });
  return total.load();
}

bool Engine::alloc_batch(const HostBatch& hb, DevBatch& b, std::string& err, bool pooled) {
  (void)hipSetDevice(dev_);
  const int pd = pooled ? dev_ : -1;
  b.n = uint32_t(hb.pk.size());
  b.n_tiles = hb.n_tiles();
  b.arena_bytes = hb.arena.size();
  b.gm = grammar_set(hb);
  b.spill_words = scratch_words(hb);
  if (!hb.attr.empty() && hb.attr.size() != hb.pk.size()) {
    err = "batch attributes do not cover every package";
    return false;
  }
  b.spill_cap = std::max<uint64_t>(b.spill_words, 64);
  const uint64_t alloc_words = b.spill_cap;
  if (const char* cap = std::getenv("TVM_TEST_SPILL_CAP"))
    b.spill_cap = std::min<uint64_t>(b.spill_cap, std::strtoull(cap, nullptr, 10));
  return dmalloc(&b.spill, alloc_words, "hipMalloc(batch scratch)", err, pd) &&
         dmalloc(&b.pk, hb.pk.size(), "hipMalloc(batch)", err, pd) &&
         dmalloc(&b.tile_off, size_t(b.n_tiles) * kGroupsPerTile + 1, "hipMalloc(group offsets)", err, pd) &&
         dmalloc(&b.arena, (hb.arena.size() + 32 + 15) & ~size_t(15), "hipMalloc(batch arena)", err, pd) &&
         (hb.attr.empty() || dmalloc(&b.attr, hb.attr.size(), "hipMalloc(batch attr)", err, pd)) &&
         dmalloc(&b.rec, hb.pk.size(), "hipMalloc(package records)", err, pd) &&
         dmalloc(&b.tail, hb.pk.size(), "hipMalloc(key tails)", err, pd);
}

static void xcd_order(const HostBatch& hb, const std::vector<uint64_t>& w, std::vector<uint32_t>& order) {
  const uint32_t n = uint32_t(order.size());
  std::vector<uint32_t> by_plat(n);
  for (uint32_t t = 0; t < n; t++) by_plat[t] = t;
  std::stable_sort(by_plat.begin(), by_plat.end(),
                   [&](uint32_t x, uint32_t y) { return hb.pk[size_t(x) * kTile].x < hb.pk[size_t(y) * kTile].x; });
  uint64_t total = 0;
  for (uint64_t x : w) total += x;
  std::vector<uint32_t> run_of(n);
  uint64_t acc = 0;
  for (uint32_t t : by_plat) {
    run_of[t] = uint32_t(std::min<uint64_t>(kXcds - 1, total ? acc * kXcds / total : 0));
    acc += w[t];
  }
  std::vector<std::vector<uint32_t>> runs(kXcds);
  for (uint32_t t : order) runs[run_of[t]].push_back(t);
  std::vector<size_t> next(kXcds, 0);
  for (uint32_t b = 0; b < n; b++) {
    uint32_t r = b % kXcds;
    for (uint32_t k = 0; k < kXcds && next[r] == runs[r].size(); k++) r = (r + 1) % kXcds;
    order[b] = runs[r][next[r]++];
  }
}

bool Engine::upload(const HostBatch& hb, DevBatch& b, std::string& err) {
  if (!alloc_batch(hb, b, err)) return false;
  std::vector<uint64_t> toff(hb.tile_off.begin(), hb.tile_off.end());
  toff.resize(size_t(hb.n_tiles()) * kGroupsPerTile + 1, hb.arena.size());
  if (!hb.pk.empty() && !hip_ok(hipMemcpy(b.pk, hb.pk.data(), hb.pk.size() * sizeof(uint2), hipMemcpyHostToDevice),
                                "H2D batch", err))
    return false;
  if (!hip_ok(hipMemcpy(b.tile_off, toff.data(), toff.size() * 8, hipMemcpyHostToDevice), "H2D tile offsets", err))
    return false;
  if (!hb.arena.empty() &&
      !hip_ok(hipMemcpy(b.arena, hb.arena.data(), hb.arena.size(), hipMemcpyHostToDevice), "H2D arena", err))
    return false;
  if (!hb.attr.empty() &&
      !hip_ok(hipMemcpy(b.attr, hb.attr.data(), hb.attr.size() * sizeof(uint2), hipMemcpyHostToDevice), "H2D attr", err))
    return false;
  static const bool no_order = std::getenv("TVM_NO_TILE_ORDER") != nullptr;
  if (((b.gm & ~GM_OS) != 0 ? b.n_tiles > 1 : b.n_tiles >= 1024) && !no_order) {
    const auto& pi = db_->plat_info;
    std::vector<uint64_t> off;
    hb.name_offsets(off);
    std::vector<uint64_t> w(b.n_tiles, 0);
    range_for(b.n_tiles, 64, [&](size_t t0, size_t t1) {
      for (size_t t = t0; t < t1; t++) {
        uint64_t s = 0;
        for (size_t p = t * kTile; p < std::min(hb.pk.size(), (t + 1) * kTile); p++) {
          const uint32_t plat = hb.pk[p].x;
          if (plat >= pi.size()) continue;
          const std::string_view name(reinterpret_cast<const char*>(hb.arena.data()) + off[p], hb.pk[p].y & 0xFFFFu);
          s += 1 + uint64_t(db_->key_rows(plat, name)) * (pi[plat].cmp == CMP_MAVEN ? 8 : 1);
        }
        w[t] = s;
      }
    });
    std::vector<uint8_t> full(b.n_tiles, 1);
    static const bool no_lean = std::getenv("TVM_NO_LEAN") != nullptr;
    if (grammar_index(b.gm) == 2 && !no_lean)
      range_for(b.n_tiles, 64, [&](size_t t0, size_t t1) {
        for (size_t t = t0; t < t1; t++) {
          bool f = false;
          for (size_t p = t * kTile; p < std::min(hb.pk.size(), (t + 1) * kTile) && !f; p++) {
            const uint32_t plat = hb.pk[p].x;
            f = plat < pi.size() && ((GM_LEAN >> pi[plat].cmp) & 1u) == 0;
          }
          full[t] = f;
        }
      });
    std::vector<uint32_t> order(b.n_tiles);
    for (uint32_t t = 0; t < b.n_tiles; t++) order[t] = t;
    b.n_lean_tiles = 0;
    for (uint32_t t = 0; t < b.n_tiles; t++) b.n_lean_tiles += full[t] ? 0 : 1;
    static const char* ord = std::getenv("TVM_TILE_ORDER");
    const uint32_t n_full = b.n_tiles - b.n_lean_tiles;
    const bool split = n_full && n_full < b.n_tiles && n_full * kSplitFull <= b.n_tiles;
    const int mode = split || (ord && std::strcmp(ord, "lean") == 0) ? 0 : (ord && std::strcmp(ord, "full") == 0) ? 1 : 2;
    std::stable_sort(order.begin(), order.end(), [&](uint32_t x, uint32_t y) {
      if (mode == 0 && full[x] != full[y]) return full[x] < full[y];
      if (mode == 1 && full[x] != full[y]) return full[x] > full[y];
      return w[x] > w[y];
    });
    if (mode == 2 && grammar_index(b.gm) == 2 && !(ord && std::strcmp(ord, "w") == 0) && b.n_tiles >= 8 * kXcds)
      xcd_order(hb, w, order);
    if (!dmalloc(&b.tile_map, order.size(), "hipMalloc(tile order)", err) ||
        !hip_ok(hipMemcpy(b.tile_map, order.data(), order.size() * 4, hipMemcpyHostToDevice), "H2D tile order", err))
      return false;
  }
  if (!hb.cpe_bits.empty() && hb.cpe_words) {
    if (!dmalloc(&b.cpe_bits, hb.cpe_bits.size(), "hipMalloc(cpe sets)", err) ||
        !hip_ok(hipMemcpy(b.cpe_bits, hb.cpe_bits.data(), hb.cpe_bits.size() * 4, hipMemcpyHostToDevice), "H2D cpe", err))
      return false;
    b.cpe_words = hb.cpe_words;
    b.n_cpe_sets = uint32_t(hb.cpe_bits.size() / hb.cpe_words);
  }
  return true;
}

void Engine::free_batch(int device, DevBatch& b, bool pooled) {
  (void)hipSetDevice(device);
  for (void* p : {static_cast<void*>(b.pk), static_cast<void*>(b.tile_off), static_cast<void*>(b.arena),
                  static_cast<void*>(b.attr), static_cast<void*>(b.rec), static_cast<void*>(b.tail),
                  static_cast<void*>(b.spill)})
    dfree(p, pooled, device);
  dfree(b.cpe_bits, false, device);
  dfree(b.tile_map, false, device);
  b = DevBatch{};
}

bool Engine::alloc_matches(uint64_t cap, uint32_t n_pkgs, DevMatches& m, std::string& err, bool pooled) {
  (void)hipSetDevice(dev_);
  const int pd = pooled ? dev_ : -1;
  m.cap = std::max<uint64_t>(cap, 1);
  m.dir_cap = std::max<uint32_t>((n_pkgs + kTile - 1) / kTile, 1);
  if (!dmalloc(&m.pkg, m.cap, "hipMalloc(matches)", err, pd) || !dmalloc(&m.adv, m.cap, "hipMalloc(matches)", err, pd) ||
      !dmalloc(&m.dir, m.dir_cap, "hipMalloc(tile dir)", err, pd) || !dmalloc(&m.ctl_mem, 16, "hipMalloc(ctl)", err, pd))
    return false;
  if (!hip_ok(hipMemset(m.ctl_mem, 0, 16 * sizeof(unsigned long long)), "memset(ctl)", err)) return false;
  m.ctl = m.ctl_mem;
  m.ctl_next = m.ctl_mem + 8;
  return true;
}

void Engine::free_matches(int device, DevMatches& m, bool pooled) {
  (void)hipSetDevice(device);
  for (void* p : {static_cast<void*>(m.pkg), static_cast<void*>(m.adv), static_cast<void*>(m.dir),
                  static_cast<void*>(m.ctl_mem ? m.ctl_mem : m.ctl)})
    dfree(p, pooled, device);
  m = DevMatches{};
}

bool Engine::fetch_ordered(const DevMatches& m, uint32_t n_pkgs, uint64_t total, std::vector<uint2>& out,
                           hipStream_t st, std::string& err) {
  out.clear();
  if (total > m.cap) {
    err = "match buffer too small";
    return false;
  }
  const uint32_t n_tiles = (n_pkgs + kTile - 1) / kTile;
  std::vector<TileDir> dir(n_tiles);
  std::vector<uint32_t> pk(total), ad(total);
  if ((n_tiles && !hip_ok(hipMemcpyAsync(dir.data(), m.dir, n_tiles * sizeof(TileDir), hipMemcpyDeviceToHost, st),
                          "D2H dir", err)) ||
      (total && (!hip_ok(hipMemcpyAsync(pk.data(), m.pkg, total * 4, hipMemcpyDeviceToHost, st), "D2H matches", err) ||
                 !hip_ok(hipMemcpyAsync(ad.data(), m.adv, total * 4, hipMemcpyDeviceToHost, st), "D2H matches", err))) ||
      !hip_ok(hipStreamSynchronize(st), "D2H matches", err))
    return false;
  out.reserve(total);
  for (const TileDir& d : dir)
    for (uint64_t i = d.base; i < d.base + d.count; i++) out.push_back(make_uint2(pk[i], ad[i]));
  return true;
}

bool Engine::launch_tiles(const DevBatch& b, const DevMatches& m, uint32_t t_begin, uint32_t t_end, hipStream_t pst,
                          hipStream_t sst, hipEvent_t ev, std::string& err, const CopyOutArgs* co,
                          unsigned long long* ctl_zero, const uint32_t* tmap, uint32_t tmap_n, uint32_t gm) {
  (void)hipSetDevice(dev_);
  if (t_end > b.n_tiles) t_end = b.n_tiles;
  if (t_begin >= t_end) return true;
  if (t_end > m.dir_cap) {
    err = "tile directory smaller than the batch";
    return false;
  }
  if (!gm) gm = b.gm;
  const int vi = resolve_variant(variant_, gm);
  if (tmap && (co || t_begin != 0 || t_end != b.n_tiles || !kFusedVariant[vi - 1] || tmap_n == 0)) {
    err = "a tile-list launch is a fused pass over the whole batch";
    return false;
  }
  last_launched_ = vi;
  const uint32_t nt = t_end - t_begin;
  const uint32_t p0 = t_begin * kTile;
  const uint32_t n = std::min<uint32_t>(b.n, t_end * kTile) - p0;
  ProbeArgs pa;
  pa.db = d_;
  pa.pk = b.pk + p0;
  pa.tile_off = b.tile_off + size_t(t_begin) * kGroupsPerTile;
  pa.arena = b.arena;
  pa.n = n;
  pa.p0 = p0;
  pa.n_total = b.n;
  pa.rec = b.rec + p0;
  pa.tail = b.tail + p0;
  pa.ctl = m.ctl;
  if (!b.spill || (b.spill_cap < b.spill_words && !std::getenv("TVM_TEST_SPILL_CAP"))) {
    err = "batch scratch missing or smaller than the batch needs";
    return false;
  }
  pa.spill = b.spill;
  pa.spill_cap = b.spill_cap;
  const bool fused = kFusedVariant[vi - 1];
  if (!fused && ctl_zero &&
      !hip_ok(hipMemsetAsync(ctl_zero, 0, 8 * sizeof(unsigned long long), pst), "memset(ctl)", err))
    return false;
  if (!fused) {
    if (co) launch_copy_out(pst, *co);
    probe_fn(b.gm)(nt, pst, pa);
    if (!hip_ok(hipGetLastError(), "probe kernel launch", err)) return false;
    if (sst != pst && (!hip_ok(hipEventRecord(ev, pst), "hipEventRecord", err) ||
                       !hip_ok(hipStreamWaitEvent(sst, ev, 0), "hipStreamWaitEvent", err)))
      return false;
  }
  SweepArgs sa;
  sa.db = d_;
  sa.rec = b.rec + p0;
  sa.tail = b.tail + p0;
  sa.spill = b.spill;
  sa.arena = b.arena;
  sa.attr = b.attr ? b.attr + p0 : nullptr;
  sa.cpe_bits = b.cpe_bits;
  sa.cpe_words = b.cpe_words;
  sa.n_cpe_sets = b.n_cpe_sets;
  sa.n = n;
  sa.p0 = p0;
  sa.out_base = b.pkg_base;
  sa.n_tiles = nt;
  sa.t0 = t_begin;
  sa.dir = m.dir;
  sa.out_pkg = m.pkg;
  sa.out_adv = m.adv;
  sa.out_cap = m.cap;
  sa.ctl = m.ctl;
  if (fused) {
    FusedArgs fa;
    fa.pa = pa;
    fa.sa = sa;
    if (co) {
      fa.co = *co;
      static const uint32_t n_copy = [] {
        const char* v = std::getenv("TVM_COPY_WG");
        return v ? uint32_t(std::max(1, std::atoi(v))) : 128u;
      }();
      fa.n_copy = n_copy;
    }
    if (!co && t_begin == 0 && t_end == b.n_tiles) fa.tile_map = tmap ? tmap : b.tile_map;
    fa.ctl_zero = co ? nullptr : ctl_zero;
    const FusedFn fn = fused_fn(gm, vi);
    if (!fn) {
      err = std::string("match-path variant ") + kVariantNames[vi - 1] + " is not built for this batch's grammar set";
      return false;
    }
    fn(tmap ? tmap_n : nt, pst, fa);
    return hip_ok(hipGetLastError(), "match kernel launch", err);
  }
  const bool filt = (b.gm & ~GM_DEB) != 0;
  sweep_table(filt)[vi - 1](nt, sst, sa);
  return hip_ok(hipGetLastError(), "sweep kernel launch", err);
}

bool Engine::launch(const DevBatch& b, DevMatches& m, hipStream_t st, std::string& err) {
  (void)hipSetDevice(dev_);
  unsigned long long* zero = nullptr;
  if (m.ctl_next) {
    std::swap(m.ctl, m.ctl_next);
    zero = m.ctl_next;
  } else if (!hip_ok(hipMemsetAsync(m.ctl, 0, 8 * sizeof(unsigned long long), st), "memset(ctl)", err)) {
    return false;
  }
  if (b.n_tiles == 0)
    return !zero || hip_ok(hipMemsetAsync(zero, 0, 8 * sizeof(unsigned long long), st), "memset(ctl)", err);
  const uint32_t nl = b.n_lean_tiles;
  if (nl && nl < b.n_tiles && (b.n_tiles - nl) * kSplitFull <= b.n_tiles && b.tile_map && grammar_index(b.gm) == 2 &&
      kFusedVariant[resolve_variant(variant_, b.gm) - 1] && kFusedVariant[resolve_variant(variant_, GM_LEAN) - 1]) {
    return launch_tiles(b, m, 0, b.n_tiles, st, st, nullptr, err, nullptr, zero, b.tile_map, nl, GM_LEAN) &&
           launch_tiles(b, m, 0, b.n_tiles, st, st, nullptr, err, nullptr, nullptr, b.tile_map + nl, b.n_tiles - nl,
                        b.gm);
  }
  return launch_tiles(b, m, 0, b.n_tiles, st, st, nullptr, err, nullptr, zero);
}

struct Engine::DropinReq {
  const HostBatch* hb = nullptr;
  std::vector<uint2>* out = nullptr;
  int64_t err_pkg = -1;
  std::string err;
  bool ok = false, done = false;
};

struct Engine::Dropin {
  int dev = 0;
  hipStream_t st = nullptr;
  DevBatch b;
  uint64_t cap_pk = 0, cap_rec = 0, cap_tail = 0, cap_groups = 0, cap_arena = 0, cap_attr = 0, cap_cpe = 0;
  uint64_t cap_dir = 0, cap_adv = 0;
  DevMatches m;
  uint8_t* pin = nullptr;
  size_t pin_cap = 0;
  std::mutex mu;
  std::condition_variable cv;
  std::deque<DropinReq*> pending;
  bool leading = false;
  uint64_t launches = 0, calls = 0, merged = 0;
  ~Dropin() {
    (void)hipSetDevice(dev);
    for (void* p : {static_cast<void*>(b.pk), static_cast<void*>(b.tile_off), static_cast<void*>(b.arena),
                    static_cast<void*>(b.attr), static_cast<void*>(b.cpe_bits), static_cast<void*>(b.rec),
                    static_cast<void*>(b.tail), static_cast<void*>(b.spill), static_cast<void*>(m.pkg),
                    static_cast<void*>(m.adv), static_cast<void*>(m.dir), static_cast<void*>(m.ctl)})
      if (p) (void)hipFree(p);
    if (pin) (void)hipHostFree(pin);
    if (st) (void)hipStreamDestroy(st);
  }
};

Engine::Dropin* Engine::dropin(std::string& err) {
  std::lock_guard<std::mutex> lk(dropin_init_mu_);
  if (!dropin_) {
    (void)hipSetDevice(dev_);
    auto d = std::make_unique<Dropin>();
    d->dev = dev_;
    if (!hip_ok(hipStreamCreateWithFlags(&d->st, hipStreamNonBlocking), "hipStreamCreate(drop-in)", err) ||
        !dmalloc(&d->m.ctl, 8, "hipMalloc(ctl)", err))
      return nullptr;
    dropin_ = std::move(d);
  }
  return dropin_.get();
}

void Engine::dropin_stats(uint64_t out[3]) {
  std::string e;
  Dropin* d = dropin(e);
  if (!d) {
    out[0] = out[1] = out[2] = 0;
    return;
  }
  std::lock_guard<std::mutex> lk(d->mu);
  out[0] = d->launches;
  out[1] = d->calls;
  out[2] = d->merged;
}

namespace {
template <class T>
bool grow_dev(T*& p, uint64_t& cap, uint64_t n, const char* what, std::string& err) {
  if (n <= cap && p) return true;
  if (p) (void)hipFree(p);
  p = nullptr;
  const uint64_t c = std::max<uint64_t>(n + n / 4, 64);
  if (!hip_ok(hipMalloc(reinterpret_cast<void**>(&p), c * sizeof(T)), what, err)) {
    cap = 0;
    return false;
  }
  cap = c;
  return true;
}
}

bool Engine::dropin_run(Dropin& d, DropinReq* const* reqs, size_t n, std::string& err) {
  (void)hipSetDevice(dev_);
  HostBatch merged;
  const HostBatch* hbp = reqs[0]->hb;
  std::vector<uint32_t> first(n + 1, 0);
  if (n > 1) {
    for (size_t k = 0; k < n; k++) {
      const HostBatch& h = *reqs[k]->hb;
      first[k] = uint32_t(merged.pk.size());
      merged.pk.insert(merged.pk.end(), h.pk.begin(), h.pk.end());
      merged.arena.insert(merged.arena.end(), h.arena.begin(), h.arena.end());
    }
    uint64_t o = 0;
    for (size_t j = 0; j < merged.pk.size(); j++) {
      if (j % kGroup == 0) merged.tile_off.push_back(o);
      o += (merged.pk[j].y & 0xFFFFu) + (merged.pk[j].y >> 16);
    }
    hbp = &merged;
  }
  const HostBatch& hb = *hbp;
  first[n] = uint32_t(hb.pk.size());
  DevBatch& b = d.b;
  b.n = uint32_t(hb.pk.size());
  b.n_tiles = hb.n_tiles();
  b.arena_bytes = hb.arena.size();
  b.gm = grammar_set(hb);
  b.spill_words = scratch_words(hb);
  if (!hb.attr.empty() && hb.attr.size() != hb.pk.size()) {
    err = "batch attributes do not cover every package";
    return false;
  }
  const uint64_t groups = uint64_t(b.n_tiles) * kGroupsPerTile + 1;
  const uint64_t arena_pad = (hb.arena.size() + 32 + 15) & ~uint64_t(15);
  if (!grow_dev(b.pk, d.cap_pk, b.n, "hipMalloc(drop-in batch)", err) ||
      !grow_dev(b.rec, d.cap_rec, b.n, "hipMalloc(drop-in records)", err) ||
      !grow_dev(b.tail, d.cap_tail, b.n, "hipMalloc(drop-in key tails)", err) ||
      !grow_dev(b.tile_off, d.cap_groups, groups, "hipMalloc(drop-in group offsets)", err) ||
      !grow_dev(b.arena, d.cap_arena, arena_pad, "hipMalloc(drop-in arena)", err) ||
      (!hb.attr.empty() && !grow_dev(b.attr, d.cap_attr, b.n, "hipMalloc(drop-in attr)", err)) ||
      (b.spill_words && !grow_dev(b.spill, b.spill_cap, b.spill_words, "hipMalloc(drop-in spill)", err)) ||
      (!hb.cpe_bits.empty() && !grow_dev(b.cpe_bits, d.cap_cpe, hb.cpe_bits.size(), "hipMalloc(drop-in cpe)", err)))
    return false;
  uint64_t mcap = std::max<uint64_t>(uint64_t(b.n) * 4, 1024);
  const uint32_t n_tiles = b.n_tiles;
  if (!grow_dev(d.m.dir, d.cap_dir, std::max<uint32_t>(n_tiles, 1), "hipMalloc(drop-in tile dir)", err)) return false;
  d.m.dir_cap = uint32_t(std::min<uint64_t>(d.cap_dir, 0xFFFFFFFFu));
  const size_t in_bytes = b.n * 8 + groups * 8 + hb.arena.size() + hb.attr.size() * 8 + hb.cpe_bits.size() * 4;
  auto stage = [&](size_t need) {
    if (need <= d.pin_cap) return true;
    if (d.pin) (void)hipHostFree(d.pin);
    d.pin = nullptr;
    d.pin_cap = 0;
    const size_t c = need + need / 4 + 4096;
    if (!hip_ok(hipHostMalloc(reinterpret_cast<void**>(&d.pin), c, hipHostMallocDefault), "hipHostMalloc(drop-in)",
                err))
      return false;
    d.pin_cap = c;
    return true;
  };
  if (!stage(in_bytes + 128)) return false;
  uint8_t* h = d.pin;
  size_t at = 0;
  auto h2d = [&](void* dst, const void* src, size_t bytes, const char* what) {
    if (!bytes) return true;
    std::memcpy(h + at, src, bytes);
    const bool r = hip_ok(hipMemcpyAsync(dst, h + at, bytes, hipMemcpyHostToDevice, d.st), what, err);
    at += bytes;
    return r;
  };
  std::vector<uint64_t> toff(hb.tile_off.begin(), hb.tile_off.end());
  toff.resize(groups, hb.arena.size());
// ... 151 lines not shown
```

### trivy_amd/csrc/match_kernel.h

```cpp
#pragma once
#include "engine.h"
#include "libver.h"
#include "match_variants.h"

namespace tvm {

constexpr uint32_t kStage = 12288;
constexpr uint32_t kKeyWords = 4;
constexpr uint32_t kMapCap = 4096;

struct ProbeArgs {
  DevDB db;
  const uint2* pk;
  const uint64_t* tile_off;
  const uint8_t* arena;
  uint32_t n;
  uint32_t p0;
  uint32_t n_total;
  PkgRec* rec;
  uint4* tail;
  unsigned long long* ctl;
  uint64_t* spill;
  uint64_t spill_cap;
};

struct SweepArgs {
  DevDB db;
  const PkgRec* rec;
  const uint4* tail;
  const uint64_t* spill;
  const uint8_t* arena;
  const uint2* attr;
  const uint32_t* cpe_bits;
  uint32_t cpe_words;
  uint32_t n_cpe_sets;
  uint32_t n;
  uint32_t p0;
  uint32_t out_base;
  uint32_t n_tiles;
  uint32_t t0;
  TileDir* dir;
  uint32_t* out_pkg;
  uint32_t* out_adv;
  uint64_t out_cap;
  unsigned long long* ctl;
};

struct FusedArgs {
  ProbeArgs pa;
  SweepArgs sa;
  CopyOutArgs co;
  uint32_t n_copy = 0;
  const uint32_t* tile_map = nullptr;
  unsigned long long* ctl_zero = nullptr;
};

using ProbeFn = void (*)(uint32_t n_tiles, hipStream_t st, const ProbeArgs& a);
using SweepFn = void (*)(uint32_t n_tiles, hipStream_t st, const SweepArgs& a);
using FusedFn = void (*)(uint32_t n_tiles, hipStream_t st, const FusedArgs& a);

namespace {

enum : uint32_t { KI_VALID = 1u << 31, KI_SPILL = 1u << 30, KI_MVN = 1u << 29, KI_H24 = 1u << 25, KI_LEN = 0x3FFFu,
                  KI_CLS_SHIFT = 26, KI_CLS_MASK = 7u, KI_P_SHIFT = 14, KI_P_MASK = 7u, KI_PFX_SHIFT = 17,
                  KI_PFX_MASK = 3u };

template <int T>
__device__ __forceinline__ uint32_t block_exscan(uint32_t* wsum, uint32_t v, uint32_t tid, uint32_t& excl) {
  constexpr int W = T / 64;
  const uint32_t lane = tid & 63, wave = tid >> 6;
  uint32_t x = v;
#pragma unroll
  for (int d = 1; d < 64; d <<= 1) {
    const uint32_t y = __shfl_up(x, d, 64);
    if (lane >= uint32_t(d)) x += y;
  }
  if (lane == 63) wsum[wave] = x;
  __syncthreads();
  uint32_t off = 0, tot = 0;
#pragma unroll
  for (int w = 0; w < W; w++) {
    const uint32_t t = wsum[w];
    off += (uint32_t(w) < wave) ? t : 0;
    tot += t;
  }
  excl = off + x - v;
  __syncthreads();
  return tot;
}


struct HeadSink {
  uint64_t* tail;
  uint64_t acc = 0, w0 = 0, w1 = 0, w2 = 0;
  uint32_t n = 0;
  __device__ explicit HeadSink(uint64_t* t) : tail(t) {}
  __device__ __forceinline__ void word(uint32_t w) {
    if (w == 0) w0 = acc;
    else if (w == 1) w1 = acc;
    else if (w < kKeyWords) tail[w - 2] = acc;
    if (w == 2) w2 = acc;
  }
  __device__ __forceinline__ void put(uint8_t b) {
    acc |= uint64_t(b) << (8 * (n & 7));
    if ((n & 7) == 7) {
      word(n >> 3);
      acc = 0;
    }
    n++;
  }
  __device__ __forceinline__ void flush() {
    if (n & 7) word(n >> 3);
  }
};

__device__ __forceinline__ uint64_t be_word(uint64_t w, uint32_t bytes) {
  if (bytes < 8) w &= (1ull << (8 * bytes)) - 1ull;
  return __builtin_bswap64(w);
}

template <class P>
__device__ __forceinline__ uint64_t name_word(const P* base, uint32_t sh, uint32_t i, uint32_t n) {
  const uint32_t d0 = base[2 * i], d1 = base[2 * i + 1], d2 = base[2 * i + 2];
  const uint32_t lo = __builtin_amdgcn_alignbyte(d1, d0, sh), hi = __builtin_amdgcn_alignbyte(d2, d1, sh);
  uint64_t w = uint64_t(lo) | (uint64_t(hi) << 32);
  const uint32_t left = n - 8 * i;
  if (left < 8) w &= (1ull << (8 * left)) - 1ull;
  return w;
}

template <class P>
__device__ __forceinline__ uint64_t name_hash(uint32_t plat, const uint8_t* s, uint32_t n) {
  const uintptr_t a = reinterpret_cast<uintptr_t>(s);
  const P* base = reinterpret_cast<const P*>(a & ~uintptr_t(3));
  const uint32_t sh = uint32_t(a & 3);
  uint64_t h = key_hash_seed2(plat, n);
  for (uint32_t i = 0; 8 * i < n; i++) h = key_hash_word(h, name_word(base, sh, i, n));
  return key_hash_fin(h);
}

template <class P>
__device__ __forceinline__ bool name_eq_slot(const uint8_t* s, uint32_t n, const uint4 q1, const uint4 q2,
                                             const uint4 q3, const uint8_t* arena) {
  static_assert(kSlotNameWords == 4, "four inline name words (q3.z / q3.w: Slot::pfx)");
  const uintptr_t a = reinterpret_cast<uintptr_t>(s);
  const P* base = reinterpret_cast<const P*>(a & ~uintptr_t(3));
  const uint32_t sh = uint32_t(a & 3);
  const uint64_t y[kSlotNameWords] = {q1.z | (uint64_t(q1.w) << 32), q2.x | (uint64_t(q2.y) << 32),
                                      q2.z | (uint64_t(q2.w) << 32), q3.x | (uint64_t(q3.y) << 32)};
  bool eq = true;
#pragma unroll
  for (uint32_t i = 0; i < kSlotNameWords; i++) eq &= (8 * i < n ? name_word(base, sh, i, n) : 0ull) == y[i];
  if (eq && n > 8 * kSlotNameWords) {
    const uint8_t* full = arena + q1.y;
    for (uint32_t i = 8 * kSlotNameWords; eq && i < n; i++) eq = full[i] == s[i];
  }
  return eq;
}

template <class P>
__device__ __forceinline__ void probe_lookup(const ProbeArgs& a, uint32_t p, uint32_t plat, const PlatInfo& pi,
                                            uint32_t nlen, const uint8_t* name, bool valid, uint64_t h,
                                            uint64_t start, bool found, uint4 q0, uint4 q0n, bool has_q0n,
                                            uint32_t& rbeg, uint32_t& cnt, uint32_t* sflags = nullptr,
                                            uint32_t cls = 0, uint64_t* pfx = nullptr);

__device__ __forceinline__ uint4 slot_head(const ProbeArgs& a, uint64_t i) {
  return reinterpret_cast<const uint4*>(a.db.slots + (i & a.db.slot_mask))[0];
}

__device__ __forceinline__ bool fp_chain(const ProbeArgs& a, uint64_t h, uint64_t& i) {
  i = h & a.db.slot_mask;
#ifdef TVM_EXP_NOFP
  return true;
#else
  const uint8_t want = slot_fp_of(h);
  for (;;) {
    const uint8_t f = a.db.slot_fp[i];
    if (f == 0) return false;
    if (f == want) return true;
    i = (i + 1) & a.db.slot_mask;
  }
#endif
}

struct ProbePre {
  uint64_t h, start;
  uint4 q0, q0n;
  bool found, has_q0n;
  uint32_t fast_st, fast_kl;
};

template <uint32_t GM, class P, int DIAG = 0, int PRE = 0>
__device__ __forceinline__ void probe_one(const ProbeArgs& a, uint32_t p, uint32_t plat, uint32_t nlen, uint32_t vlen,
                                          const uint8_t* name, const uint8_t* ver, uint64_t vglob, PkgRec& r,
                                          uint8_t* kb = nullptr, const uint8_t* tab = nullptr,
                                          const ProbePre* pre = nullptr) {
  const PlatInfo pi = a.db.plats[plat];
  constexpr bool kPre = GM == GM_DEB;
  uint64_t h = 0, start = 0;
  bool found = false;
  uint4 q0 = make_uint4(0, 0, 0, 0), q0n = q0;
  bool has_q0n = false;
  if constexpr (PRE != 0) {
    static_assert(GM == GM_DEB && DIAG == 0, "the balanced kernel is dpkg-only");
    h = pre->h;
    start = pre->start;
    found = pre->found;
    q0 = pre->q0;
    q0n = pre->q0n;
    has_q0n = pre->has_q0n;
  } else if (!(DIAG & 2)) {
    h = name_hash<P>(plat, name, nlen);
    found = fp_chain(a, h, start);
  }
  auto heads = [&]() {
    if ((DIAG & 2) || !found) return;
    q0 = slot_head(a, start);
    if constexpr (kPre) {
      has_q0n = !(start & 1);
      if (has_q0n) q0n = slot_head(a, start + 1);
    }
  };
  if constexpr (kPre && PRE == 0) heads();
  if (!(DIAG & 1) && kb && ((GM >> CMP_DEB) & 1u) && pi.cmp == CMP_DEB) {
    uint32_t kl = 0, st;
    if constexpr (PRE == 2) {
      st = pre->fast_st;
      kl = pre->fast_kl;
    } else {
      st = deb_fast_key(ver, (DIAG & 8) ? min(vlen, 12u) : vlen, kb, tab, kl);
    }
    if (st != FAST_FALLBACK) {
      const bool valid = st == FAST_OK;
      const uint32_t* kw = reinterpret_cast<const uint32_t*>(kb);
      uint32_t kinfo = (valid ? (kl & KI_LEN) | KI_VALID : 0u) | KI_H24, koff = 0;
      r.k0 = r.k1 = r.k2 = 0;
      if (valid) {
        const uint64_t m0 = uint64_t(kw[0]) | (uint64_t(kw[1]) << 32), m1 = uint64_t(kw[2]) | (uint64_t(kw[3]) << 32);
        r.k0 = be_word(m0, kl < 8 ? kl : 8);
        r.k1 = kl > 8 ? be_word(m1, kl < 16 ? kl - 8 : 8) : 0ull;
        r.k2 = kl > 16 ? be_word(uint64_t(kw[4]) | (uint64_t(kw[5]) << 32), kl < 24 ? kl - 16 : 8) : 0ull;
        static_assert(kFastKeyCap <= kKeyWords * 8, "fast keys fit head + tail slot");
        if (kl > (GM == GM_DEB ? 24u : 16u)) a.tail[p] = make_uint4(kw[4], kw[5], kw[6], kw[7]);
      }
      uint32_t cnt = 0, rbeg = 0;
      if constexpr (!kPre) heads();
      uint64_t pfx = 0;
      if (!(DIAG & 2)) probe_lookup<P>(a, p, plat, pi, nlen, name, (kinfo & KI_VALID) != 0, h, start, found, q0, q0n, has_q0n,
                                          rbeg, cnt, nullptr, 0, GM == GM_DEB ? &pfx : nullptr);
      if constexpr (GM == GM_DEB)
        kinfo |= ((uint32_t(pfx) & KI_P_MASK) << KI_P_SHIFT) | (row16_prefix_cmp(r.k0, kl, pfx) << KI_PFX_SHIFT);
      r.meta = make_uint4(rbeg, cnt, kinfo, koff);
      return;
    }
  }
  uint64_t* tslot = reinterpret_cast<uint64_t*>(a.tail + p);
  HeadSink hs(tslot);
  uint32_t cls = 0;
  bool valid = true;
  if (DIAG & 1) {
    hs.n = vlen;
    hs.w0 = vlen;
  } else {
    valid = encode_version_gm<GM>(pi.cmp, ver, vlen, hs, cls);
  }
  hs.flush();
  uint32_t kinfo = 0, koff = 0;
  const bool mvn_pkg = ((GM >> CMP_MAVEN) & 1u) && pi.cmp == CMP_MAVEN;
  if (valid && hs.n > (mvn_pkg ? 16u : kKeyWords * 8)) {
    const uint32_t need = (hs.n + 7) / 8;
    const unsigned long long o = atomicAdd(&a.ctl[2], (unsigned long long)need);
    if (o + need > a.spill_cap) {
      atomicOr(&a.ctl[3], (unsigned long long)ERR_SPILL);
      valid = false;
    } else {
      WordSink ws(a.spill + o);
      uint32_t cls2 = 0;
      encode_version_gm<GM>(pi.cmp, ver, vlen, ws, cls2);
      ws.flush();
      koff = uint32_t(o);
      kinfo |= KI_SPILL;
    }
  }
  uint32_t cnt = 0, rbeg = 0, sflags = 0;
  if constexpr (!kPre) heads();
  uint64_t pfx = 0;
  if (!(DIAG & 2)) probe_lookup<P>(a, p, plat, pi, nlen, name, valid, h, start, found, q0, q0n, has_q0n, rbeg, cnt,
                                   &sflags, cls, GM == GM_DEB ? &pfx : nullptr);
  if (((GM >> CMP_MAVEN) & 1u) && pi.cmp == CMP_MAVEN) {
    uint32_t off = 0, nt = 0;
    if (valid && (sflags & (cls == 1 ? SLOT_MVN_C1 : SLOT_MVN_C0))) {
      MvnParse mp;
      if (mvn_parse(ver, vlen, mp)) {
        const uint32_t need = (kMvnPackedWords * mp.n + 1) / 2;
        const unsigned long long o = atomicAdd(&a.ctl[2], (unsigned long long)need);
        if (o + need > a.spill_cap) {
          atomicOr(&a.ctl[3], (unsigned long long)ERR_SPILL);
          valid = false;
          cnt = rbeg = 0;
        } else {
          mvn_pack(mp, ver, reinterpret_cast<uint32_t*>(a.spill + o));
          off = uint32_t(o);
          nt = uint32_t(mp.n);
        }
      }
    }
    a.tail[p] = make_uint4(off, nt | (vlen << 16), uint32_t(vglob), uint32_t(vglob >> 32));
  }
  const uint32_t kl = hs.n;
  kinfo |= (kl & KI_LEN) | (valid ? KI_VALID : 0u) | ((cls & KI_CLS_MASK) << KI_CLS_SHIFT);
  if (pi.cmp == CMP_DEB) kinfo |= KI_H24;
  if (((GM >> CMP_MAVEN) & 1u) && pi.cmp == CMP_MAVEN && (sflags & (SLOT_MVN_C0 | SLOT_MVN_C1))) kinfo |= KI_MVN;
  r.k0 = valid && kl ? be_word(hs.w0, kl < 8 ? kl : 8) : 0ull;
  r.k1 = valid && kl > 8 ? be_word(hs.w1, kl < 16 ? kl - 8 : 8) : 0ull;
  r.k2 = valid && kl > 16 ? be_word(hs.w2, kl < 24 ? kl - 16 : 8) : 0ull;
  if constexpr (GM == GM_DEB)
    kinfo |= ((uint32_t(pfx) & KI_P_MASK) << KI_P_SHIFT) | (row16_prefix_cmp(r.k0, kl, pfx) << KI_PFX_SHIFT);
  r.meta = make_uint4(rbeg, cnt, kinfo, koff);
}

template <class P>
__device__ __forceinline__ void probe_lookup(const ProbeArgs& a, uint32_t p, uint32_t plat, const PlatInfo& pi,
                                            uint32_t nlen, const uint8_t* name, bool valid, uint64_t h,
                                            uint64_t start, bool found, uint4 q0, uint4 q0n, bool has_q0n,
                                            uint32_t& rbeg, uint32_t& cnt, uint32_t* sflags, uint32_t cls, uint64_t* pfx) {
  if (found && (valid || (pi.flags & PLAT_LOOKUP_FIRST))) {
    uint32_t step = 0;
    for (uint64_t i = start;; i = (i + 1) & a.db.slot_mask, step++) {
      const uint4* sp = reinterpret_cast<const uint4*>(a.db.slots + i);
      if (step == 1 && has_q0n) q0 = q0n;
      else if (step > 0) q0 = sp[0];
      const uint4 q1 = sp[1], q2 = sp[2], q3 = sp[3];
      const uint64_t sh = q0.x | (uint64_t(q0.y) << 32);
      if (sh == 0) break;
      if (sh != h) continue;
      if ((q1.x & SLOT_LEN_MASK) != nlen || !name_eq_slot<P>(name, nlen, q1, q2, q3, a.db.name_arena)) continue;
      if (q1.x & SLOT_POISONED) {
        atomicMax(&a.ctl[1], (unsigned long long)(a.n_total - (a.p0 + p)));
      } else if (valid) {
        const uint2 rr = slot_rows(q1.x, q0.z, q0.w, cls);
        rbeg = rr.x;
        cnt = rr.y;
        if (sflags) *sflags = q1.x & (SLOT_MVN_C0 | SLOT_MVN_C1);
        if (pfx) *pfx = q3.z | (uint64_t(q3.w) << 32);
      }
      break;
    }
  }
}

template <uint32_t STG = kStage>
__device__ __forceinline__ void stage_window(uint4* buf, const uint8_t* src8, uint32_t nv, uint32_t tid) {
  constexpr uint32_t SV = (STG / 16 + kTile - 1) / kTile;
  const uint4* src = reinterpret_cast<const uint4*>(src8);
  if (nv) {
    uint4 v[SV];
#pragma unroll
    for (uint32_t k = 0; k < SV; k++) v[k] = src[min(tid + k * kTile, nv - 1)];
#pragma unroll
    for (uint32_t k = 0; k < SV; k++)
      if (tid + k * kTile < nv) buf[tid + k * kTile] = v[k];
  }
  if (tid < 2) buf[nv + tid] = make_uint4(0, 0, 0, 0);
}

__device__ __forceinline__ uint32_t wave_exscan(uint32_t v, uint32_t lane) {
  uint32_t x = v;
#pragma unroll
  for (int d = 1; d < 64; d <<= 1) {
    const uint32_t y = __shfl_up(x, d, 64);
    if (lane >= uint32_t(d)) x += y;
  }
  return x - v;
}

template <uint32_t STG = kStage>
__device__ __forceinline__ void stage_window_wave(uint4* buf, const uint8_t* src8, uint32_t nv, uint32_t lane) {
  constexpr uint32_t SV = (STG / 4 / 16 + 63) / 64;
  const uint4* src = reinterpret_cast<const uint4*>(src8);
  if (nv) {
    uint4 v[SV];
#pragma unroll
    for (uint32_t k = 0; k < SV; k++) v[k] = src[min(lane + k * 64, nv - 1)];
#pragma unroll
    for (uint32_t k = 0; k < SV; k++)
      if (lane + k * 64 < nv) buf[lane + k * 64] = v[k];
  }
  if (lane < 2) buf[nv + lane] = make_uint4(0, 0, 0, 0);
}

template <uint32_t GM, int DIAG = 0>
__global__ __launch_bounds__(kTile) void probe_kernel(ProbeArgs a) {
  __shared__ uint4 stage[kStage / 16 + 2];
  __shared__ uint32_t wsum[kTile / 64];
  __shared__ uint32_t kbuf[kTile * kFastKeyStride / 4];
  __shared__ uint8_t tab[128];
  const uint32_t tid = threadIdx.x, t = blockIdx.x;
  if (tid < 128) tab[tid] = deb_fast_code(tid);
  const uint32_t p = t * kTile + tid;
  uint2 d = make_uint2(0xFFFFFFFFu, 0);
  if (p < a.n) d = a.pk[p];
  const uint64_t w0 = a.tile_off[t * kGroupsPerTile], w1 = a.tile_off[(t + 1) * kGroupsPerTile];
  const uint32_t nlen = d.y & 0xFFFFu, vlen = d.y >> 16;
  uint32_t off = 0;
  block_exscan<kTile>(wsum, nlen + vlen, tid, off);
  const uint64_t base16 = w0 & ~uint64_t(15);
  const bool staged = w1 - base16 <= kStage;
  if (staged) stage_window(stage, a.arena + base16, uint32_t((w1 - base16 + 15) / 16), tid);
  __syncthreads();
  PkgRec r;
  r.meta = make_uint4(0, 0, 0, 0);
  r.k0 = r.k1 = r.k2 = 0;
  if (p < a.n && d.x < a.db.n_plats) {
    if (staged) {
      const uint8_t* sb = reinterpret_cast<const uint8_t*>(stage) + uint32_t(w0 - base16) + off;
      probe_one<GM, uint32_t, DIAG>(a, p, d.x, nlen, vlen, sb, sb + nlen, w0 + off + nlen, r,
                                    reinterpret_cast<uint8_t*>(kbuf) + tid * kFastKeyStride, tab);
    } else {
      const uint8_t* gb = a.arena + w0 + off;
      probe_one<GM, uint32_t, DIAG>(a, p, d.x, nlen, vlen, gb, gb + nlen, w0 + off + nlen, r);
    }
  }
  if (p < a.n) a.rec[p] = r;
}


template <int FILT>
struct SweepShared {
  uint64_t k0[kTile], k1[kTile], k2[FILT < 2 ? kTile : 1];
  uint32_t kinfo[kTile];
  uint32_t koff[kTile];
  uint2 pattr[FILT ? kTile : 1];
  uint32_t nz_scan[kTile + 1];
  uint32_t nz_rd[kTile];
  uint32_t nz_q[kTile];
  uint32_t wsum[2][kTile / 64];
  uint32_t wsum2[2][8 * (kTile / 64)];
  uint32_t tile;
  unsigned long long base;
};

__device__ __forceinline__ uint32_t map_shift(uint32_t total) {
  uint32_t sh = 0;
  while ((total + (1u << sh) - 1) >> sh > kMapCap) sh++;
  return sh;
}

template <int FILT>
__device__ __forceinline__ bool mvn_pair(const SweepArgs& a, const uint32_t* ids, uint32_t p) {
  const uint4 t = a.tail[p];
  const MvnPackedView V{reinterpret_cast<const uint32_t*>(a.spill + t.x), int(t.y & 0xFFFFu),
                        a.arena + (uint64_t(t.z) | (uint64_t(t.w) << 32))};
  return mvn_program_eval(ids, V);
}

__device__ __forceinline__ uint32_t inline_pass(const SweepArgs& a, const Row& row, uint2 pa) {
  const uint32_t kind = row.lo_len & 15u, na = (row.lo_len >> 4) & 3u, nc = (row.lo_len >> 6) & 3u;
  if (kind & AUX_TAG) return row.off.lo_off == pa.y ? 1u : 0u;
  const uint32_t w[2] = {row.off.lo_off, row.off.hi_off};
  auto id = [&](uint32_t i) { return (w[i >> 1] >> (16 * (i & 1))) & 0xFFFFu; };
  if (kind & (AUX_ARCH_RH | AUX_ARCH_IN)) {
    bool ok = (kind & AUX_ARCH_RH) && (na == 0 || (pa.x & PA_NOARCH));
    const uint32_t arch = pa.x & PA_ARCH_MASK;
    for (uint32_t i = 0; i < na; i++) ok |= id(i) == arch;
    if (!ok) return 0;
  }
  if (kind & AUX_CPE) {
    if (pa.y >= a.n_cpe_sets) return 0;
    const uint32_t* set = a.cpe_bits + size_t(pa.y) * a.cpe_words;
    bool ok = false;
    for (uint32_t i = 0; i < nc; i++) {
      const uint32_t c = id(na + i);
      ok |= (c >> 5) < a.cpe_words && ((set[c >> 5] >> (c & 31)) & 1u);
    }
    if (!ok) return 0;
  }
  return 1;
}

template <int FILT, bool DEFER = false>
__device__ __forceinline__ uint32_t aux_pass(const SweepArgs& a, uint32_t ridx, uint2 pa, uint32_t ki, uint32_t p) {
#ifdef TVM_EXP_NOAUX
  if (FILT < 2) return 1;
#endif
  const RowAux x = a.db.aux[ridx];
  const uint32_t* ids = a.db.aux_ids + x.list_off;
  if ((x.kind & AUX_CLASS) && !((x.tag >> ((ki >> KI_CLS_SHIFT) & KI_CLS_MASK)) & 1u)) return 0;
  if (FILT >= 2 && (x.kind & AUX_MVN)) {
    if constexpr (DEFER) return 2;
    return mvn_pair<FILT>(a, ids, p) ? 1u : 0u;
  }
  if (x.kind & (AUX_ARCH_RH | AUX_ARCH_IN)) {
    bool ok = (x.kind & AUX_ARCH_RH) && (x.n_arch == 0 || (pa.x & PA_NOARCH));
    const uint32_t arch = pa.x & PA_ARCH_MASK;
    for (uint32_t i = 0; i < x.n_arch && !ok; i++) ok = ids[i] == arch;
    if (!ok) return 0;
  }
  if (x.kind & AUX_CPE) {
    if (pa.y >= a.n_cpe_sets) return 0;
    const uint32_t* set = a.cpe_bits + size_t(pa.y) * a.cpe_words;
    bool ok = false;
    for (uint32_t i = 0; i < x.n_cpe && !ok; i++) {
      const uint32_t c = ids[x.n_arch + i];
      ok = (c >> 5) < a.cpe_words && ((set[c >> 5] >> (c & 31)) & 1u);
    }
    if (!ok) return 0;
  }
  if ((x.kind & AUX_TAG) && x.tag != pa.y) return 0;
  return 1;
}

__device__ __forceinline__ int cmp_be(uint64_t a0, uint64_t a1, const uint64_t* atail, uint32_t na, uint64_t b0,
                                      uint64_t b1, const uint64_t* btail, uint32_t nb) {
  if (a0 != b0) return a0 < b0 ? -1 : 1;
  if (a1 != b1) return a1 < b1 ? -1 : 1;
  if (na <= 16 || nb <= 16) return (na > nb) - (na < nb);
  return key_cmp(atail, na - 16, btail, nb - 16);
}

__device__ __forceinline__ int cmp_head(uint64_t a0, uint64_t a1, uint64_t a2, uint32_t na, uint64_t b0, uint64_t b1,
                                        uint64_t b2, uint32_t nb, uint32_t hl, bool& tie) {
  const bool eq0 = a0 == b0, eq1 = eq0 && a1 == b1, eq = eq1 && a2 == b2;
  const bool lt = a0 < b0 || (eq0 && a1 < b1) || (eq1 && a2 < b2);
  tie = eq && na > hl && nb > hl;
  const int byl = (na > nb) - (na < nb);
  return eq ? byl : (lt ? -1 : 1);
}

template <int FILT, bool DEFER = false, class S>
__device__ __forceinline__ uint32_t eval_row(const SweepArgs& a, const S& s, uint32_t q, uint32_t p, const Row& row,
                                             uint32_t ridx) {
  const uint32_t ki = s.kinfo[q];
  const uint32_t kl = ki & KI_LEN;
  const bool h24 = FILT == 0 || (ki & KI_H24), c24 = FILT < 2 && h24;
  const uint64_t k0 = s.k0[q], k1 = s.k1[q], k2 = c24 ? s.k2[q] : 0ull;
  const uint32_t nh = row.hi_len & KEY_LEN_MASK, hl = c24 ? 24u : 16u;
  bool tie = false;
  int c = cmp_head(k0, k1, k2, kl, row.hi_pre0, row.hi_pre1, c24 ? row.hi_pre2 : 0ull, nh, hl, tie);
  const bool hi_inf = (row.hi_len & KEY_INF) != 0;
  if (tie && !hi_inf) {
    const uint64_t* ktail =
        (ki & KI_SPILL) ? a.spill + s.koff[q] + 2 : reinterpret_cast<const uint64_t*>(a.tail + p);
    const uint32_t w = hl / 8;
    const uint32_t hi_off = (h24 || (row.adv & ROW_INLINE)) ? a.db.row_off[ridx].hi_off : row.off.hi_off;
    c = key_cmp(ktail + (w - 2), kl - hl, a.db.key_words + hi_off + w, nh - hl);
  }
  bool m = hi_inf || ((row.hi_len & KEY_INCL) ? c <= 0 : c < 0);
  if (!(row.lo_len & KEY_INF) && m) {
    const uint64_t t24[2] = {__builtin_bswap64(c24 ? k2 : 0ull), 0ull};
    const uint64_t* ktail = (ki & KI_SPILL) ? a.spill + s.koff[q] + 2
                            : (c24 && kl <= 24) ? t24
                                                : reinterpret_cast<const uint64_t*>(a.tail + p);
    const uint64_t* lw = a.db.key_words + (h24 ? a.db.row_off[ridx].lo_off : row.off.lo_off);
    const uint32_t nl = row.lo_len & KEY_LEN_MASK;
    const uint64_t l0 = nl ? be_word(lw[0], nl < 8 ? nl : 8) : 0ull;
    const uint64_t l1 = nl > 8 ? be_word(lw[1], nl < 16 ? nl - 8 : 8) : 0ull;
    const int cl = cmp_be(k0, k1, ktail, kl, l0, l1, lw + 2, nl);
    m = (row.lo_len & KEY_INCL) ? cl >= 0 : cl > 0;
  }
  m = m && (ki & KI_VALID);
// ... 290 lines not shown
    s.nz_scan[nrank] = excl;
    s.nz_rd[nrank] = r.meta.x - excl;
    s.nz_q[nrank] = tid;
    if constexpr (kRec) {
      const uint32_t ki = r.meta.z;
      uint64_t hh;
      uint32_t ht;
      row16_pkg_lex(r.k0, r.k1, r.k2, ki & KI_LEN, (ki >> KI_P_SHIFT) & KI_P_MASK, (ki >> KI_PFX_SHIFT) & KI_PFX_MASK,
                    (ki & KI_VALID) != 0, hh, ht);
      hot.head[nrank] = hh;
      hot.tail[nrank] = ht;
    }
  }
  if (tid == 0) s.nz_scan[nnz] = total;
  __syncthreads();
  {
    const uint32_t shift = map_shift(total), nb = (total + (1u << shift) - 1) >> shift;
    const uint32_t per = (nb + kTile - 1) / kTile;
    uint32_t b = tid * per;
    const uint32_t be = min(b + per, nb);
    if (b < be) {
      uint32_t rr = pair_rank(s, nnz, b << shift);
      for (; b < be; b++) {
        while (s.nz_scan[rr + 1] <= (b << shift)) rr++;
        map[b] = uint8_t(rr);
      }
    }
    __syncthreads();
  }

  if constexpr (SEG != 0) {
    constexpr int MBW = MB / 4;
    constexpr int R16 = (SEG >> 2) & 3;
    const uint32_t seg = ((total + 4 * 64 - 1) / (4 * 64)) * 64;
    const uint32_t s0 = min(total, wave * seg), s1 = min(total, s0 + seg);
    uint32_t* madv_w = madv + wave * MBW;
    uint8_t* mq_w = mq + wave * MBW;
    const uint32_t nmw = sweep_seg<K, MBW, FILT, false, R16, kRec>(a, s, madv_w, mq_w, map, nnz, total, s0, s1, lane, 0, hot);
    if (lane == 0) s.wsum[0][wave] = nmw;
    __syncthreads();
    uint32_t woff = 0, nm = 0;
#pragma unroll
    for (int w = 0; w < kTile / 64; w++) {
      const uint32_t c = s.wsum[0][w];
      woff += (uint32_t(w) < wave) ? c : 0;
      nm += c;
    }
    if (tid == 0) {
      s.base = nm ? atomicAdd(&a.ctl[0], (unsigned long long)nm) : 0ull;
      TileDir e;
      e.base = s.base;
      e.count = nm;
      e.pad = 0;
      a.dir[a.t0 + t] = e;
    }
    __syncthreads();
    const unsigned long long base = s.base + woff;
    if (nmw <= uint32_t(MBW)) {
      const uint32_t pb = a.out_base + a.p0 + t * kTile;
      for (uint32_t i = lane; i < nmw; i += 64) {
        if (base + i < a.out_cap) {
          a.out_pkg[base + i] = pb + mq_w[i];
          a.out_adv[base + i] = madv_w[i];
        }
      }
    } else {
      sweep_seg<K, MBW, FILT, true, R16, kRec>(a, s, madv_w, mq_w, map, nnz, total, s0, s1, lane, base, hot);
    }
    return;
  }
  const bool mvn = FILT >= 2 && dq.cap && __syncthreads_or((r.meta.z & KI_MVN) != 0);
  const uint32_t nm = sweep<K, MB, FILT, false>(a, s, madv, mq, map, nnz, total, tid, 0, mvn, dq);

  if (tid == 0) {
    s.base = nm ? atomicAdd(&a.ctl[0], (unsigned long long)nm) : 0ull;
    TileDir e;
    e.base = s.base;
    e.count = nm;
    e.pad = 0;
    a.dir[a.t0 + t] = e;
  }
  __syncthreads();
  const unsigned long long base = s.base;
  if (nm <= uint32_t(MB)) {
    const uint32_t pb = a.out_base + a.p0 + t * kTile;
    for (uint32_t i = tid; i < nm; i += kTile) {
      if (base + i < a.out_cap) {
        a.out_pkg[base + i] = pb + mq[i];
        a.out_adv[base + i] = madv[i];
      }
    }
  } else {
    sweep<K, MB, FILT, true>(a, s, madv, mq, map, nnz, total, tid, base, mvn, dq);
  }
}

template <int K, int MB, int FILT>
__global__ __launch_bounds__(kTile) void sweep_kernel(SweepArgs a) {
  __shared__ SweepShared<FILT> s;
  __shared__ uint32_t madv[MB];
  __shared__ uint8_t mq[MB];
  __shared__ uint8_t map[kMapCap];
  constexpr uint32_t kQ = FILT >= 2 ? 512 : 1;
  __shared__ uint32_t dqj[kQ], dqres[FILT >= 2 ? kTile / 8 : 1];
  const uint32_t tid = threadIdx.x, t = blockIdx.x;
  const uint32_t p = t * kTile + tid;
  PkgRec r;
  r.meta = make_uint4(0, 0, 0, 0);
  r.k0 = r.k1 = r.k2 = 0;
  if (p < a.n) r = a.rec[p];
  sweep_tile<K, MB, FILT>(a, s, madv, mq, map, t, tid, r, DeferQ{dqj, dqres, FILT >= 2 ? kQ : 0u});
}

template <uint32_t GM, int K, int MB, int FILT, int DIAG = 0, int WPE = 1, int SEG = 0, uint32_t STG = kStage,
          bool MOVE = false>
__global__ __launch_bounds__(kTile, WPE) void fused_kernel(FusedArgs fa) {
  constexpr uint32_t kStageVec = STG / 16 + 8;
  constexpr uint32_t kMbufVec = (MB * 5 + 15) / 16;
  __shared__ uint4 buf[kStageVec > kMbufVec ? kStageVec : kMbufVec];
  struct SweepPart {
    SweepShared<FILT> s;
    uint8_t map[kMapCap];
  };
  constexpr bool kBal = (SEG & 32) != 0;
  static_assert(!kBal || (GM == GM_DEB && (SEG & 2) && DIAG == 0), "encoder balance: dpkg-only, per-wave staging");
  struct ProbePart {
    uint32_t kbuf[kTile * kFastKeyStride / 4];
    uint8_t tab[128];
    uint32_t bal_cnt[kBal ? kEncBuckets : 1];
    uint32_t bal_mixed;
    uint32_t bal_ver[kBal ? kTile : 1];
    uint8_t bal_list[kBal ? kEncBuckets * kTile : 1];
  };
  static_assert(sizeof(ProbePart) <= sizeof(SweepPart), "the probe's LDS fits in the sweep's");
  __shared__ union {
    SweepPart sw;
    ProbePart pr;
  } u;
  SweepShared<FILT>& s = u.sw.s;
  uint8_t* map = u.sw.map;
  constexpr bool kHot = ((SEG >> 2) & 3) == 3;
  __shared__ uint64_t hot_head[kHot ? kTile : 1];
  __shared__ uint32_t hot_tail[kHot ? kTile : 1];
  const ProbeArgs& a = fa.pa;
  if constexpr (MOVE) {
    if (blockIdx.x < fa.n_copy) {
      static_assert(sizeof(buf) >= kCopyLdsWords * 4, "the result move borrows the staging buffer");
      __builtin_amdgcn_s_setprio(3);
      copy_out_tiles(fa.co, blockIdx.x, fa.n_copy, reinterpret_cast<uint32_t*>(buf));
      return;
    }
  }
  const uint32_t tid = threadIdx.x;
  if (!MOVE && fa.ctl_zero && blockIdx.x == 0 && tid < 8) fa.ctl_zero[tid] = 0ull;
  const uint32_t t = MOVE ? blockIdx.x - fa.n_copy : (fa.tile_map ? fa.tile_map[blockIdx.x] : blockIdx.x);
  const uint32_t p = t * kTile + tid;
  uint2 d = make_uint2(0xFFFFFFFFu, 0);
  if (p < a.n) d = a.pk[p];
  constexpr bool kWaveStage = (SEG & 2) != 0;
  const uint32_t g = t * kGroupsPerTile + (kWaveStage ? (tid >> 6) : 0u);
  const uint64_t w0 = a.tile_off[g], w1 = a.tile_off[kWaveStage ? g + 1 : (t + 1) * kGroupsPerTile];
  if constexpr (kBal) {
    if (tid < kEncBuckets) u.pr.bal_cnt[tid] = 0;
    if (tid == kEncBuckets) u.pr.bal_mixed = 0;
    __syncthreads();
  }
  const uint32_t nlen = d.y & 0xFFFFu, vlen = d.y >> 16;
  uint32_t off = 0;
  uint4* sbuf = buf;
  const uint64_t base16 = w0 & ~uint64_t(15);
  bool staged;
  const bool own = p < a.n && d.x < a.db.n_plats;
  ProbePre pre;
  pre.h = pre.start = 0;
  pre.q0 = pre.q0n = make_uint4(0, 0, 0, 0);
  pre.found = pre.has_q0n = false;
  pre.fast_st = pre.fast_kl = 0;
  bool listed = false;
  if constexpr (kWaveStage) {
    off = wave_exscan(nlen + vlen, tid & 63);
    sbuf = buf + (tid >> 6) * (STG / 4 / 16 + 2);
    staged = w1 - base16 <= STG / 4;
    if (staged) stage_window_wave<STG>(sbuf, a.arena + base16, uint32_t((w1 - base16 + 15) / 16), tid & 63);
    if (tid < 128) u.pr.tab[tid] = deb_fast_code(tid);
    if constexpr (kBal) {
      if (!staged) {
        if ((tid & 63) == 0) u.pr.bal_mixed = 1;
      } else if (own) {
        const uint32_t noff = uint32_t(reinterpret_cast<const uint8_t*>(sbuf) - reinterpret_cast<const uint8_t*>(buf)) +
                              uint32_t(w0 - base16) + off;
        pre.h = name_hash<uint32_t>(d.x, reinterpret_cast<const uint8_t*>(buf) + noff, nlen);
        pre.found = fp_chain(a, pre.h, pre.start);
        if (pre.found) {
          pre.q0 = slot_head(a, pre.start);
          pre.has_q0n = !(pre.start & 1);
          if (pre.has_q0n) pre.q0n = slot_head(a, pre.start + 1);
          listed = a.db.plats[d.x].cmp == CMP_DEB;
          if (listed) {
            const uint32_t b = enc_bal_bucket(vlen);
            const uint32_t rank = atomicAdd(&u.pr.bal_cnt[b], 1u);
            u.pr.bal_list[b * kTile + rank] = uint8_t(tid);
            u.pr.bal_ver[tid] = (noff + nlen) | (vlen << 16);
          }
        }
      }
    }
    __syncthreads();
  } else {
    block_exscan<kTile>(s.wsum[0], nlen + vlen, tid, off);
    staged = w1 - base16 <= STG;
    if (staged) stage_window<STG>(buf, a.arena + base16, uint32_t((w1 - base16 + 15) / 16), tid);
    if (tid < 128) u.pr.tab[tid] = deb_fast_code(tid);
    __syncthreads();
  }
  PkgRec r;
  r.meta = make_uint4(0, 0, 0, 0);
  r.k0 = r.k1 = r.k2 = 0;
  if constexpr (kBal) {
    uint8_t* const kbytes = reinterpret_cast<uint8_t*>(u.pr.kbuf);
    const uint8_t* sb = reinterpret_cast<const uint8_t*>(sbuf) + uint32_t(w0 - base16) + off;
    const bool packed = u.pr.bal_mixed == 0;
    if (packed) {
      uint32_t cnt[kEncBuckets];
#pragma unroll
      for (uint32_t i = 0; i < kEncBuckets; i++) cnt[i] = u.pr.bal_cnt[i];
      uint32_t b = 0, idx = 0;
      if (enc_bal_item(cnt, tid, b, idx)) {
        const uint32_t q = u.pr.bal_list[b * kTile + idx], e = u.pr.bal_ver[q];
        uint8_t* kb = kbytes + q * kFastKeyStride;
        uint32_t kl = 0;
        const uint32_t st = deb_fast_key(reinterpret_cast<const uint8_t*>(buf) + (e & 0xFFFFu), e >> 16, kb, u.pr.tab, kl);
        static_assert(kFastKeyStride == 44 && kFastKeyCap + 5 <= 40, "slot bytes 40..43 are free");
        reinterpret_cast<uint32_t*>(kb)[10] = st | (kl << 8);
      }
      __syncthreads();
    }
    if (packed && listed) {
      const uint32_t w = reinterpret_cast<const uint32_t*>(kbytes + tid * kFastKeyStride)[10];
      pre.fast_st = w & 0xFFu;
      pre.fast_kl = w >> 8;
      probe_one<GM, uint32_t, 0, 2>(a, p, d.x, nlen, vlen, sb, sb + nlen, w0 + off + nlen, r,
                                    kbytes + tid * kFastKeyStride, u.pr.tab, &pre);
    } else if (own && (!packed || pre.found)) {
      if (staged) {
        probe_one<GM, uint32_t, 0>(a, p, d.x, nlen, vlen, sb, sb + nlen, w0 + off + nlen, r,
                                   kbytes + tid * kFastKeyStride, u.pr.tab);
      } else {
        const uint8_t* gb = a.arena + w0 + off;
        probe_one<GM, uint32_t, 0>(a, p, d.x, nlen, vlen, gb, gb + nlen, w0 + off + nlen, r);
      }
    }
  } else if (p < a.n && d.x < a.db.n_plats) {
    if (staged) {
      const uint8_t* sb = reinterpret_cast<const uint8_t*>(sbuf) + uint32_t(w0 - base16) + off;
      probe_one<GM, uint32_t, DIAG & 11>(a, p, d.x, nlen, vlen, sb, sb + nlen, w0 + off + nlen, r,
                                         reinterpret_cast<uint8_t*>(u.pr.kbuf) + tid * kFastKeyStride, u.pr.tab);
    } else {
      const uint8_t* gb = a.arena + w0 + off;
      probe_one<GM, uint32_t, DIAG & 3>(a, p, d.x, nlen, vlen, gb, gb + nlen, w0 + off + nlen, r);
    }
  }
  if (DIAG & 4) r.meta.y = 0;
  __syncthreads();
  uint32_t* madv = reinterpret_cast<uint32_t*>(buf);
  constexpr uint32_t kBufWords = sizeof(buf) / 4, kMbWords = (uint32_t(MB) * 5 + 3) / 4;
  constexpr uint32_t kQ = kBufWords > kMbWords + kTile / 8 + 16 ? kBufWords - kMbWords - kTile / 8 : 0;
  static_assert(FILT < 2 || kQ >= 16, "no room for the Maven program queue");
  const DeferQ dq{madv + kMbWords + kTile / 8, madv + kMbWords, FILT >= 2 ? kQ : 0u};
  sweep_tile<K, MB, FILT, SEG>(fa.sa, s, madv, reinterpret_cast<uint8_t*>(madv + MB), map, t, tid, r, dq,
                               Hot16{hot_head, hot_tail});
}

template <uint32_t GM, int DIAG = 0>
void launch_probe(uint32_t n_tiles, hipStream_t st, const ProbeArgs& a) {
  hipLaunchKernelGGL((probe_kernel<GM, DIAG>), dim3(n_tiles), dim3(kTile), 0, st, a);
}

template <int K, int MB, int FILT>
void launch_sweep(uint32_t n_tiles, hipStream_t st, const SweepArgs& a) {
  hipLaunchKernelGGL((sweep_kernel<K, MB, FILT>), dim3(n_tiles), dim3(kTile), 0, st, a);
}

template <uint32_t GM, int K, int MB, int FILT, int DIAG = 0, int WPE = 1, int SEG = 0, uint32_t STG = kStage>
void launch_fused(uint32_t n_tiles, hipStream_t st, const FusedArgs& a) {
  if (a.n_copy)
    hipLaunchKernelGGL((fused_kernel<GM, K, MB, FILT, DIAG, WPE, SEG, STG, true>), dim3(n_tiles + a.n_copy), dim3(kTile), 0,
                       st, a);
  else
    hipLaunchKernelGGL((fused_kernel<GM, K, MB, FILT, DIAG, WPE, SEG, STG, false>), dim3(n_tiles), dim3(kTile), 0, st, a);
}

template <uint32_t GM, int FILT, int F, int K, int MB>
constexpr FusedFn fused_entry() {
  if constexpr (F == 0) return nullptr;
  else if constexpr (F == 4) return &launch_fused<GM, K, MB, FILT, 0, 1, 1>;
  else if constexpr (F == 5) return &launch_fused<GM, K, MB, FILT, 0, 1, 3>;
  else if constexpr (F == 6) return &launch_fused<GM, K, MB, FILT, 0, 6, 3>;
  else if constexpr (F == 7) {
    if constexpr (GM == GM_DEB) return &launch_fused<GM, K, MB, FILT, 0, 1, 3 | 12>;
    else return nullptr;
  } else if constexpr (F == 8) {
    if constexpr (GM == GM_DEB) return &launch_fused<GM, K, MB, FILT, 0, 1, 3 | 12 | 16>;
    else return nullptr;
  } else if constexpr (F == 9) {
    if constexpr (GM == GM_DEB) return &launch_fused<GM, K, MB, FILT, 0, 1, 3 | 12 | 16 | 32>;
    else return nullptr;
  } else if constexpr (F == 25 || F == 26) {
    if constexpr (GM == GM_DEB) return &launch_fused<GM, K, MB, FILT, 0, 1, 3 | (F == 25 ? 4 : 8)>;
    else return nullptr;
  } else if constexpr (F == 28) {
    if constexpr (GM == GM_DEB) return &launch_fused<GM, K, MB, FILT, 8, 1, 3 | 12 | 16>;
    else return nullptr;
  }
  else return &launch_fused<GM, K, MB, FILT, (F >= 10 ? F - 10 : 0), (FILT >= 2 && K <= 2 && F == 1) ? 5 : TVM_FUSED_WPE(F)>;
}

}
}
```

Measured before the change: 11.14 billion packages/s.

## Precompute per-tile head records and issue arena window loads earlier

Builds a host-side TileHead array, one 32-byte record per ordered tile holding the tile id, base offset and group deltas. The fused kernel then reads that single record instead of a dependent tile_map lookup followed by tile_off loads. It also issues the wave-staged arena window loads before the bal-counter setup and stores them unconditionally, and clamps the package load instead of branching, to shorten the dependent-load chain at kernel start. The cost is an extra device buffer and H2D copy per batch, and more live registers while the window loads are in flight.

```diff
diff --git a/include/trivy_amd.h b/include/trivy_amd.h
--- a/include/trivy_amd.h
+++ b/include/trivy_amd.h
@@ -108,6 +108,8 @@
 int tvm_engine_dropin_stats(tvm_engine* e, uint64_t* out3);
 int tvm_engine_verify(tvm_engine* e, char* err, size_t errlen);
 int tvm_engine_set_variant(tvm_engine* e, int v);
+int64_t tvm_engine_set_order_min_tiles(tvm_engine* e, uint32_t n);
+int tvm_engine_last_head_launches(tvm_engine* e);
 const char* tvm_variant_name(int v);
 int tvm_variant_grammar_sets(int v);
 int tvm_engine_last_variant(tvm_engine* e);
@@ -174,6 +176,10 @@
 int tvm_enc_bal_buckets_host(void);
 int tvm_enc_bal_bucket_host(uint32_t version_len);
 int tvm_enc_bal_item_host(const uint32_t* counts, uint32_t item, uint32_t* bucket, uint32_t* index);
+int64_t tvm_tile_heads_host(const tvm_db* db, size_t n_runs, const char* const* run_bucket, const uint64_t* run_n,
+                            const char* arena, const uint64_t* name_off, const uint32_t* name_len,
+                            const uint64_t* ver_off, const uint32_t* ver_len, uint32_t min_tiles, uint32_t* order_out,
+                            uint8_t* heads_out, uint64_t* toff_out, size_t cap_tiles);
 enum { TVM_ISVULN_PAIRWISE = 0x100 };
 int tvm_lib_is_vulnerable_host(int grammar, const char* ver, size_t ver_len, const char* advisory_json,
                                size_t json_len);
diff --git a/trivy_amd/_lib.py b/trivy_amd/_lib.py
--- a/trivy_amd/_lib.py
+++ b/trivy_amd/_lib.py
@@ -137,6 +137,8 @@
     ("tvm_engine_table_bytes", ctypes.c_uint64, [_P]),
     ("tvm_engine_verify", ctypes.c_int, [_P, ctypes.c_char_p, ctypes.c_size_t]),
     ("tvm_engine_set_variant", ctypes.c_int, [_P, ctypes.c_int]),
+    ("tvm_engine_set_order_min_tiles", ctypes.c_int64, [_P, ctypes.c_uint32]),
+    ("tvm_engine_last_head_launches", ctypes.c_int, [_P]),
     ("tvm_variant_name", ctypes.c_char_p, [ctypes.c_int]),
     ("tvm_variant_grammar_sets", ctypes.c_int, [ctypes.c_int]),
     ("tvm_engine_last_variant", ctypes.c_int, [_P]),
@@ -232,6 +234,10 @@
     ("tvm_enc_bal_bucket_host", ctypes.c_int, [ctypes.c_uint32]),
     ("tvm_enc_bal_item_host", ctypes.c_int, [ctypes.POINTER(ctypes.c_uint32), ctypes.c_uint32,
                                              ctypes.POINTER(ctypes.c_uint32), ctypes.POINTER(ctypes.c_uint32)]),
+    ("tvm_tile_heads_host", ctypes.c_int64, [_P, ctypes.c_size_t, ctypes.POINTER(ctypes.c_char_p), ctypes.c_void_p,
+                                             ctypes.c_char_p, ctypes.c_void_p, ctypes.c_void_p, ctypes.c_void_p,
+                                             ctypes.c_void_p, ctypes.c_uint32, ctypes.c_void_p, ctypes.c_void_p,
+                                             ctypes.c_void_p, ctypes.c_size_t]),
     ("tvm_db_advisory_vuln_id", ctypes.c_char_p, [_P, ctypes.c_uint32]),
     ("tvm_version_class", ctypes.c_int, [ctypes.c_int, ctypes.c_char_p, ctypes.c_size_t]),
     ("tvm_lib_is_vulnerable_host", ctypes.c_int, [ctypes.c_int, ctypes.c_char_p, ctypes.c_size_t, ctypes.c_char_p,
diff --git a/trivy_amd/csrc/capi.cpp b/trivy_amd/csrc/capi.cpp
--- a/trivy_amd/csrc/capi.cpp
+++ b/trivy_amd/csrc/capi.cpp
@@ -497,6 +497,12 @@
   return v < 0 ? e->eng->variant() : e->eng->set_variant(v);
 }
 
+int64_t tvm_engine_set_order_min_tiles(tvm_engine* e, uint32_t n) {
+  if (!e) return -1;
+  std::unique_lock<std::shared_mutex> lk(e->mu);
+  return int64_t(e->eng->set_order_min_tiles(n));
+}
+
 const char* tvm_variant_name(int v) { return variant_name(v); }
 int tvm_variant_grammar_sets(int v) { return variant_grammar_sets(v); }
 
@@ -504,6 +510,12 @@
   if (!e) return -1;
   std::shared_lock<std::shared_mutex> lk(e->mu);
   return e->eng->last_launched();
+}
+
+int tvm_engine_last_head_launches(tvm_engine* e) {
+  if (!e) return -1;
+  std::shared_lock<std::shared_mutex> lk(e->mu);
+  return e->eng->last_head_launches();
 }
 
 static int detect_common(tvm_engine* e, bool full, const char* fam, const char* ver, const tvm_repository* repo,
@@ -580,6 +592,7 @@
     for (void* p : {static_cast<void*>(b->dev.pk), static_cast<void*>(b->dev.tile_off), static_cast<void*>(b->dev.arena),
                     static_cast<void*>(b->dev.attr), static_cast<void*>(b->dev.cpe_bits), static_cast<void*>(b->dev.rec),
                     static_cast<void*>(b->dev.tail), static_cast<void*>(b->dev.spill),
+                    static_cast<void*>(b->dev.tile_map), static_cast<void*>(b->dev.tile_head),
                     static_cast<void*>(b->external_out ? nullptr : b->m.pkg),
                     static_cast<void*>(b->external_out ? nullptr : b->m.adv), static_cast<void*>(b->m.dir),
                     static_cast<void*>(b->m.ctl),
@@ -1140,6 +1153,36 @@
   *bucket = b;
   *index = i;
   return 1;
+}
+
+int64_t tvm_tile_heads_host(const tvm_db* db, size_t n_runs, const char* const* run_bucket, const uint64_t* run_n,
+                            const char* arena, const uint64_t* name_off, const uint32_t* name_len,
+                            const uint64_t* ver_off, const uint32_t* ver_len, uint32_t min_tiles, uint32_t* order_out,
+                            uint8_t* heads_out, uint64_t* toff_out, size_t cap_tiles) {
+  if (!db || !db->finalized || (n_runs && (!run_bucket || !run_n))) return -1;
+  HostBatch hb;
+  size_t i = 0;
+  for (size_t r = 0; r < n_runs; r++) {
+    if (!run_bucket[r] || (run_n[r] && (!arena || !name_off || !name_len || !ver_off || !ver_len))) return -1;
+    const int32_t plat = db->db.find_plat(run_bucket[r]);
+    for (uint64_t k = 0; k < run_n[r]; k++, i++)
+      hb.add(plat < 0 ? 0xFFFFFFFFu : uint32_t(plat), std::string_view(arena + name_off[i], name_len[i]),
+             std::string_view(arena + ver_off[i], ver_len[i]));
+  }
+  const uint32_t nt = hb.n_tiles();
+  if (nt > cap_tiles) return -1;
+  std::vector<uint64_t> toff(hb.tile_off.begin(), hb.tile_off.end());
+  toff.resize(size_t(nt) * kGroupsPerTile + 1, hb.arena.size());
+  if (toff_out) std::memcpy(toff_out, toff.data(), toff.size() * 8);
+  std::vector<uint32_t> order;
+  uint32_t n_lean = 0;
+  if (!tile_order(db->db, hb, batch_grammar_set(db->db, hb), min_tiles ? min_tiles : kOrderMinTiles, order, n_lean))
+    return 0;
+  std::vector<TileHead> heads;
+  build_tile_heads(toff, order, heads);
+  if (order_out) std::memcpy(order_out, order.data(), order.size() * 4);
+  if (heads_out) std::memcpy(heads_out, heads.data(), heads.size() * sizeof(TileHead));
+  return int64_t(order.size());
 }
 
 int tvm_lib_is_vulnerable_host(int grammar, const char* ver, size_t ver_len, const char* advisory_json,
diff --git a/trivy_amd/csrc/engine.h b/trivy_amd/csrc/engine.h
--- a/trivy_amd/csrc/engine.h
+++ b/trivy_amd/csrc/engine.h
@@ -80,6 +80,20 @@
   uint64_t k0, k1, k2;
 };
 
+struct alignas(32) TileHead {
+  uint64_t base;
+  uint32_t tile;
+  uint32_t d[kGroupsPerTile];
+  uint32_t pad;
+};
+static_assert(sizeof(TileHead) == 32, "one record per 32 bytes");
+
+void build_tile_heads(const std::vector<uint64_t>& toff, const std::vector<uint32_t>& order, std::vector<TileHead>& out);
+constexpr uint32_t kOrderMinTiles = 1024;
+uint32_t batch_grammar_set(const DB& db, const HostBatch& hb);
+bool tile_order(const DB& db, const HostBatch& hb, uint32_t gm, uint32_t min_tiles, std::vector<uint32_t>& order,
+                uint32_t& n_lean_tiles);
+
 struct DevBatch {
   uint2* pk = nullptr;
   uint64_t* tile_off = nullptr;
@@ -97,6 +111,7 @@
   uint64_t* spill = nullptr;
   uint64_t spill_cap = 0;
   uint32_t* tile_map = nullptr;
+  TileHead* tile_head = nullptr;
   uint32_t n_lean_tiles = 0;
   PkgRec* rec = nullptr;
   uint4* tail = nullptr;
@@ -328,7 +343,7 @@
   bool launch(const DevBatch& b, DevMatches& m, hipStream_t stream, std::string& err);
   bool launch_tiles(const DevBatch& b, const DevMatches& m, uint32_t t_begin, uint32_t t_end, hipStream_t probe_st,
                     hipStream_t sweep_st, hipEvent_t ev, std::string& err, const CopyOutArgs* co = nullptr,
-                    unsigned long long* ctl_zero = nullptr, const uint32_t* tmap = nullptr, uint32_t tmap_n = 0,
+                    unsigned long long* ctl_zero = nullptr, uint32_t tmap_off = 0, uint32_t tmap_n = 0,
                     uint32_t gm = 0);
 
   static bool fetch_ordered(const DevMatches& m, uint32_t n_pkgs, uint64_t total, std::vector<uint2>& out,
@@ -341,14 +356,18 @@
   const PlatInfo* device_plats() const { return d_.plats; }
 
   int set_variant(int v);
+  uint32_t set_order_min_tiles(uint32_t n);
   int last_launched() const { return last_launched_; }
+  int last_head_launches() const { return last_head_launches_; }
   bool verify(std::string& err);
   int variant() const { return variant_; }
 
  private:
   int dev_ = 0;
   int variant_ = 0;
+  uint32_t order_min_tiles_ = kOrderMinTiles;
   std::atomic<int> last_launched_{-1};
+  std::atomic<int> last_head_launches_{0};
   hipStream_t stream_ = nullptr;
   const DB* db_ = nullptr;
   DevDB d_;
diff --git a/trivy_amd/csrc/engine.hip b/trivy_amd/csrc/engine.hip
--- a/trivy_amd/csrc/engine.hip
+++ b/trivy_amd/csrc/engine.hip
@@ -196,8 +196,16 @@
   return old;
 }
 
-uint32_t Engine::grammar_set(const HostBatch& hb) const {
-  const auto& pi = db_->plat_info;
+uint32_t Engine::set_order_min_tiles(uint32_t n) {
+  const uint32_t old = order_min_tiles_;
+  if (n) order_min_tiles_ = n;
+  return old;
+}
+
+uint32_t Engine::grammar_set(const HostBatch& hb) const { return batch_grammar_set(*db_, hb); }
+
+uint32_t batch_grammar_set(const DB& db, const HostBatch& hb) {
+  const auto& pi = db.plat_info;
   std::atomic<uint32_t> gm{0};
   range_for(hb.pk.size(), 1 << 18, [&](size_t a, size_t b) {
     uint32_t g = 0, last = 0xFFFFFFFFu;
@@ -293,28 +301,70 @@
   if (!hb.attr.empty() &&
       !hip_ok(hipMemcpy(b.attr, hb.attr.data(), hb.attr.size() * sizeof(uint2), hipMemcpyHostToDevice), "H2D attr", err))
     return false;
+  std::vector<uint32_t> order;
+  if (tile_order(*db_, hb, b.gm, order_min_tiles_, order, b.n_lean_tiles)) {
+    if (!dmalloc(&b.tile_map, order.size(), "hipMalloc(tile order)", err) ||
+        !hip_ok(hipMemcpy(b.tile_map, order.data(), order.size() * 4, hipMemcpyHostToDevice), "H2D tile order", err))
+      return false;
+    if (!std::getenv("TVM_NO_TILE_HEAD")) {
+      std::vector<TileHead> heads;
+      build_tile_heads(toff, order, heads);
+      if (!dmalloc(&b.tile_head, heads.size(), "hipMalloc(tile heads)", err) ||
+          !hip_ok(hipMemcpy(b.tile_head, heads.data(), heads.size() * sizeof(TileHead), hipMemcpyHostToDevice),
+                  "H2D tile heads", err))
+        return false;
+    }
+  }
+  if (!hb.cpe_bits.empty() && hb.cpe_words) {
+    if (!dmalloc(&b.cpe_bits, hb.cpe_bits.size(), "hipMalloc(cpe sets)", err) ||
+        !hip_ok(hipMemcpy(b.cpe_bits, hb.cpe_bits.data(), hb.cpe_bits.size() * 4, hipMemcpyHostToDevice), "H2D cpe", err))
+      return false;
+    b.cpe_words = hb.cpe_words;
+    b.n_cpe_sets = uint32_t(hb.cpe_bits.size() / hb.cpe_words);
+  }
+  return true;
+}
+
+void build_tile_heads(const std::vector<uint64_t>& toff, const std::vector<uint32_t>& order, std::vector<TileHead>& out) {
+  out.resize(order.size());
+  for (size_t i = 0; i < order.size(); i++) {
+    const uint64_t* o = toff.data() + size_t(order[i]) * kGroupsPerTile;
+    TileHead& h = out[i];
+    h.base = o[0];
+    h.tile = order[i];
+    for (int k = 0; k < kGroupsPerTile; k++) h.d[k] = uint32_t(o[k + 1] - o[0]);
+    h.pad = 0;
+  }
+}
+
+bool tile_order(const DB& db, const HostBatch& hb, uint32_t gm, uint32_t min_tiles, std::vector<uint32_t>& order,
+                uint32_t& n_lean_tiles) {
+  const uint32_t n_tiles = hb.n_tiles();
+  order.clear();
+  n_lean_tiles = 0;
   static const bool no_order = std::getenv("TVM_NO_TILE_ORDER") != nullptr;
-  if (((b.gm & ~GM_OS) != 0 ? b.n_tiles > 1 : b.n_tiles >= 1024) && !no_order) {
-    const auto& pi = db_->plat_info;
+  if (no_order || !((gm & ~GM_OS) != 0 ? n_tiles > 1 : n_tiles >= std::max(min_tiles, 1u))) return false;
+  {
+    const auto& pi = db.plat_info;
     std::vector<uint64_t> off;
     hb.name_offsets(off);
-    std::vector<uint64_t> w(b.n_tiles, 0);
-    range_for(b.n_tiles, 64, [&](size_t t0, size_t t1) {
+    std::vector<uint64_t> w(n_tiles, 0);
+    range_for(n_tiles, 64, [&](size_t t0, size_t t1) {
       for (size_t t = t0; t < t1; t++) {
         uint64_t s = 0;
         for (size_t p = t * kTile; p < std::min(hb.pk.size(), (t + 1) * kTile); p++) {
           const uint32_t plat = hb.pk[p].x;
           if (plat >= pi.size()) continue;
           const std::string_view name(reinterpret_cast<const char*>(hb.arena.data()) + off[p], hb.pk[p].y & 0xFFFFu);
-          s += 1 + uint64_t(db_->key_rows(plat, name)) * (pi[plat].cmp == CMP_MAVEN ? 8 : 1);
+          s += 1 + uint64_t(db.key_rows(plat, name)) * (pi[plat].cmp == CMP_MAVEN ? 8 : 1);
         }
         w[t] = s;
       }
     });
-    std::vector<uint8_t> full(b.n_tiles, 1);
+    std::vector<uint8_t> full(n_tiles, 1);
     static const bool no_lean = std::getenv("TVM_NO_LEAN") != nullptr;
-    if (grammar_index(b.gm) == 2 && !no_lean)
-      range_for(b.n_tiles, 64, [&](size_t t0, size_t t1) {
+    if (grammar_index(gm) == 2 && !no_lean)
+      range_for(n_tiles, 64, [&](size_t t0, size_t t1) {
         for (size_t t = t0; t < t1; t++) {
           bool f = false;
           for (size_t p = t * kTile; p < std::min(hb.pk.size(), (t + 1) * kTile) && !f; p++) {
@@ -324,31 +374,20 @@
           full[t] = f;
         }
       });
-    std::vector<uint32_t> order(b.n_tiles);
-    for (uint32_t t = 0; t < b.n_tiles; t++) order[t] = t;
-    b.n_lean_tiles = 0;
-    for (uint32_t t = 0; t < b.n_tiles; t++) b.n_lean_tiles += full[t] ? 0 : 1;
+    order.resize(n_tiles);
+    for (uint32_t t = 0; t < n_tiles; t++) order[t] = t;
+    for (uint32_t t = 0; t < n_tiles; t++) n_lean_tiles += full[t] ? 0 : 1;
     static const char* ord = std::getenv("TVM_TILE_ORDER");
-    const uint32_t n_full = b.n_tiles - b.n_lean_tiles;
-    const bool split = n_full && n_full < b.n_tiles && n_full * kSplitFull <= b.n_tiles;
+    const uint32_t n_full = n_tiles - n_lean_tiles;
+    const bool split = n_full && n_full < n_tiles && n_full * kSplitFull <= n_tiles;
     const int mode = split || (ord && std::strcmp(ord, "lean") == 0) ? 0 : (ord && std::strcmp(ord, "full") == 0) ? 1 : 2;
     std::stable_sort(order.begin(), order.end(), [&](uint32_t x, uint32_t y) {
       if (mode == 0 && full[x] != full[y]) return full[x] < full[y];
       if (mode == 1 && full[x] != full[y]) return full[x] > full[y];
       return w[x] > w[y];
     });
-    if (mode == 2 && grammar_index(b.gm) == 2 && !(ord && std::strcmp(ord, "w") == 0) && b.n_tiles >= 8 * kXcds)
+    if (mode == 2 && grammar_index(gm) == 2 && !(ord && std::strcmp(ord, "w") == 0) && n_tiles >= 8 * kXcds)
       xcd_order(hb, w, order);
-    if (!dmalloc(&b.tile_map, order.size(), "hipMalloc(tile order)", err) ||
-        !hip_ok(hipMemcpy(b.tile_map, order.data(), order.size() * 4, hipMemcpyHostToDevice), "H2D tile order", err))
-      return false;
-  }
-  if (!hb.cpe_bits.empty() && hb.cpe_words) {
-    if (!dmalloc(&b.cpe_bits, hb.cpe_bits.size(), "hipMalloc(cpe sets)", err) ||
-        !hip_ok(hipMemcpy(b.cpe_bits, hb.cpe_bits.data(), hb.cpe_bits.size() * 4, hipMemcpyHostToDevice), "H2D cpe", err))
-      return false;
-    b.cpe_words = hb.cpe_words;
-    b.n_cpe_sets = uint32_t(hb.cpe_bits.size() / hb.cpe_words);
   }
   return true;
 }
@@ -361,6 +400,7 @@
     dfree(p, pooled, device);
   dfree(b.cpe_bits, false, device);
   dfree(b.tile_map, false, device);
+  dfree(b.tile_head, false, device);
   b = DevBatch{};
 }
 
@@ -410,7 +450,7 @@
 
 bool Engine::launch_tiles(const DevBatch& b, const DevMatches& m, uint32_t t_begin, uint32_t t_end, hipStream_t pst,
                           hipStream_t sst, hipEvent_t ev, std::string& err, const CopyOutArgs* co,
-                          unsigned long long* ctl_zero, const uint32_t* tmap, uint32_t tmap_n, uint32_t gm) {
+                          unsigned long long* ctl_zero, uint32_t tmap_off, uint32_t tmap_n, uint32_t gm) {
   (void)hipSetDevice(dev_);
   if (t_end > b.n_tiles) t_end = b.n_tiles;
   if (t_begin >= t_end) return true;
@@ -420,8 +460,10 @@
   }
   if (!gm) gm = b.gm;
   const int vi = resolve_variant(variant_, gm);
-  if (tmap && (co || t_begin != 0 || t_end != b.n_tiles || !kFusedVariant[vi - 1] || tmap_n == 0)) {
-    err = "a tile-list launch is a fused pass over the whole batch";
+  const bool part = tmap_n != 0;
+  if (part && (co || t_begin != 0 || t_end != b.n_tiles || !kFusedVariant[vi - 1] || !b.tile_map ||
+               uint64_t(tmap_off) + tmap_n > b.n_tiles)) {
+    err = "a tile-list launch is a fused pass over the whole batch, on a part of its tile order";
     return false;
   }
   last_launched_ = vi;
@@ -489,14 +531,19 @@
       }();
       fa.n_copy = n_copy;
     }
-    if (!co && t_begin == 0 && t_end == b.n_tiles) fa.tile_map = tmap ? tmap : b.tile_map;
+    if (!co && t_begin == 0 && t_end == b.n_tiles) {
+      const uint32_t off = part ? tmap_off : 0u;
+      if (b.tile_map) fa.tile_map = b.tile_map + off;
+      if (b.tile_map && b.tile_head) fa.tile_head = b.tile_head + off;
+    }
+    if (fa.tile_head) last_head_launches_++;
     fa.ctl_zero = co ? nullptr : ctl_zero;
     const FusedFn fn = fused_fn(gm, vi);
     if (!fn) {
       err = std::string("match-path variant ") + kVariantNames[vi - 1] + " is not built for this batch's grammar set";
       return false;
     }
-    fn(tmap ? tmap_n : nt, pst, fa);
+    fn(part ? tmap_n : nt, pst, fa);
     return hip_ok(hipGetLastError(), "match kernel launch", err);
   }
   const bool filt = (b.gm & ~GM_DEB) != 0;
@@ -506,6 +553,7 @@
 
 bool Engine::launch(const DevBatch& b, DevMatches& m, hipStream_t st, std::string& err) {
   (void)hipSetDevice(dev_);
+  last_head_launches_ = 0;
   unsigned long long* zero = nullptr;
   if (m.ctl_next) {
     std::swap(m.ctl, m.ctl_next);
@@ -518,8 +566,8 @@
   const uint32_t nl = b.n_lean_tiles;
   if (nl && nl < b.n_tiles && (b.n_tiles - nl) * kSplitFull <= b.n_tiles && b.tile_map && grammar_index(b.gm) == 2 &&
       kFusedVariant[resolve_variant(variant_, b.gm) - 1] && kFusedVariant[resolve_variant(variant_, GM_LEAN) - 1]) {
-    return launch_tiles(b, m, 0, b.n_tiles, st, st, nullptr, err, nullptr, zero, b.tile_map, nl, GM_LEAN) &&
-           launch_tiles(b, m, 0, b.n_tiles, st, st, nullptr, err, nullptr, nullptr, b.tile_map + nl, b.n_tiles - nl,
+    return launch_tiles(b, m, 0, b.n_tiles, st, st, nullptr, err, nullptr, zero, 0, nl, GM_LEAN) &&
+           launch_tiles(b, m, 0, b.n_tiles, st, st, nullptr, err, nullptr, nullptr, nl, b.n_tiles - nl,
                         b.gm);
   }
   return launch_tiles(b, m, 0, b.n_tiles, st, st, nullptr, err, nullptr, zero);
diff --git a/trivy_amd/csrc/match_kernel.h b/trivy_amd/csrc/match_kernel.h
--- a/trivy_amd/csrc/match_kernel.h
+++ b/trivy_amd/csrc/match_kernel.h
@@ -52,6 +52,7 @@
   CopyOutArgs co;
   uint32_t n_copy = 0;
   const uint32_t* tile_map = nullptr;
+  const TileHead* tile_head = nullptr;
   unsigned long long* ctl_zero = nullptr;
 };
 
@@ -350,19 +351,43 @@
   }
 }
 
+template <uint32_t SV, uint32_t W>
+__device__ __forceinline__ void window_issue(uint4 (&v)[SV], const uint8_t* src8, uint32_t nv, uint32_t i) {
+  const uint4* src = reinterpret_cast<const uint4*>(src8);
+  const uint32_t last = max(nv, 1u) - 1;
+#pragma unroll
+  for (uint32_t k = 0; k < SV; k++) v[k] = src[min(i + k * W, last)];
+}
+
+template <uint32_t SV, uint32_t W, bool ZERO>
+__device__ __forceinline__ void window_store(uint4* buf, const uint4 (&v)[SV], uint32_t nv, uint32_t i) {
+#pragma unroll
+  for (uint32_t k = 0; k < SV; k++) buf[i + k * W] = (!ZERO || i + k * W < nv) ? v[k] : make_uint4(0, 0, 0, 0);
+  if (i < 2) buf[nv + i] = make_uint4(0, 0, 0, 0);
+}
+
+template <uint32_t STG>
+struct StageGeom {
+  static constexpr uint32_t kTileSV = (STG / 16 + kTile - 1) / kTile;
+  static constexpr uint32_t kWaveSV = (STG / 4 / 16 + 63) / 64;
+  static_assert(kTileSV * kTile <= STG / 16 + 2, "an unconditional store stays inside the tile's window");
+  static_assert(kWaveSV * 64 <= STG / 4 / 16 + 2, "an unconditional store stays inside the wave's window");
+};
+
 template <uint32_t STG = kStage>
 __device__ __forceinline__ void stage_window(uint4* buf, const uint8_t* src8, uint32_t nv, uint32_t tid) {
-  constexpr uint32_t SV = (STG / 16 + kTile - 1) / kTile;
-  const uint4* src = reinterpret_cast<const uint4*>(src8);
   if (nv) {
-    uint4 v[SV];
-#pragma unroll
-    for (uint32_t k = 0; k < SV; k++) v[k] = src[min(tid + k * kTile, nv - 1)];
-#pragma unroll
-    for (uint32_t k = 0; k < SV; k++)
-      if (tid + k * kTile < nv) buf[tid + k * kTile] = v[k];
-  }
-  if (tid < 2) buf[nv + tid] = make_uint4(0, 0, 0, 0);
+    uint4 v[StageGeom<STG>::kTileSV];
+    window_issue<StageGeom<STG>::kTileSV, kTile>(v, src8, nv, tid);
+    window_store<StageGeom<STG>::kTileSV, kTile, true>(buf, v, nv, tid);
+  } else if (tid < 2) {
+    buf[tid] = make_uint4(0, 0, 0, 0);
+  }
+}
+
+__device__ __forceinline__ uint64_t wave_uniform(uint64_t v) {
+  return uint64_t(__builtin_amdgcn_readfirstlane(uint32_t(v))) |
+         (uint64_t(__builtin_amdgcn_readfirstlane(uint32_t(v >> 32))) << 32);
 }
 
 __device__ __forceinline__ uint32_t wave_exscan(uint32_t v, uint32_t lane) {
@@ -373,21 +398,6 @@
     if (lane >= uint32_t(d)) x += y;
   }
   return x - v;
-}
-
-template <uint32_t STG = kStage>
-__device__ __forceinline__ void stage_window_wave(uint4* buf, const uint8_t* src8, uint32_t nv, uint32_t lane) {
-  constexpr uint32_t SV = (STG / 4 / 16 + 63) / 64;
-  const uint4* src = reinterpret_cast<const uint4*>(src8);
-  if (nv) {
-    uint4 v[SV];
-#pragma unroll
-    for (uint32_t k = 0; k < SV; k++) v[k] = src[min(lane + k * 64, nv - 1)];
-#pragma unroll
-    for (uint32_t k = 0; k < SV; k++)
-      if (lane + k * 64 < nv) buf[lane + k * 64] = v[k];
-  }
-  if (lane < 2) buf[nv + lane] = make_uint4(0, 0, 0, 0);
 }
 
 template <uint32_t GM, int DIAG = 0>
@@ -399,14 +409,14 @@
   const uint32_t tid = threadIdx.x, t = blockIdx.x;
   if (tid < 128) tab[tid] = deb_fast_code(tid);
   const uint32_t p = t * kTile + tid;
-  uint2 d = make_uint2(0xFFFFFFFFu, 0);
-  if (p < a.n) d = a.pk[p];
+  uint2 d = a.pk[min(p, a.n - 1)];
+  if (p >= a.n) d = make_uint2(0xFFFFFFFFu, 0);
   const uint64_t w0 = a.tile_off[t * kGroupsPerTile], w1 = a.tile_off[(t + 1) * kGroupsPerTile];
   const uint32_t nlen = d.y & 0xFFFFu, vlen = d.y >> 16;
+  const uint64_t base16 = w0 & ~uint64_t(15);
+  const bool staged = w1 - base16 <= kStage;
   uint32_t off = 0;
   block_exscan<kTile>(wsum, nlen + vlen, tid, off);
-  const uint64_t base16 = w0 & ~uint64_t(15);
-  const bool staged = w1 - base16 <= kStage;
   if (staged) stage_window(stage, a.arena + base16, uint32_t((w1 - base16 + 15) / 16), tid);
   __syncthreads();
   PkgRec r;
@@ -1003,14 +1013,42 @@
     }
   }
   const uint32_t tid = threadIdx.x;
+  constexpr bool kWaveStage = (SEG & 2) != 0;
+  const bool has_head = !MOVE && fa.tile_head != nullptr;
+  uint32_t t;
+  uint64_t w0 = 0, w1 = 0;
+  if (has_head) {
+    const TileHead h = fa.tile_head[blockIdx.x];
+    t = h.tile;
+    if constexpr (kWaveStage) {
+      const uint32_t w = __builtin_amdgcn_readfirstlane(tid >> 6);
+      const uint32_t lo = w == 0 ? 0u : w == 1 ? h.d[0] : w == 2 ? h.d[1] : h.d[2];
+      const uint32_t hi = w == 0 ? h.d[0] : w == 1 ? h.d[1] : w == 2 ? h.d[2] : h.d[3];
+      w0 = h.base + lo;
+      w1 = h.base + hi;
+    } else {
+      w0 = h.base;
+      w1 = h.base + h.d[kGroupsPerTile - 1];
+    }
+  } else {
+    t = MOVE ? blockIdx.x - fa.n_copy : (fa.tile_map ? fa.tile_map[blockIdx.x] : blockIdx.x);
+  }
   if (!MOVE && fa.ctl_zero && blockIdx.x == 0 && tid < 8) fa.ctl_zero[tid] = 0ull;
-  const uint32_t t = MOVE ? blockIdx.x - fa.n_copy : (fa.tile_map ? fa.tile_map[blockIdx.x] : blockIdx.x);
   const uint32_t p = t * kTile + tid;
-  uint2 d = make_uint2(0xFFFFFFFFu, 0);
-  if (p < a.n) d = a.pk[p];
-  constexpr bool kWaveStage = (SEG & 2) != 0;
-  const uint32_t g = t * kGroupsPerTile + (kWaveStage ? (tid >> 6) : 0u);
-  const uint64_t w0 = a.tile_off[g], w1 = a.tile_off[kWaveStage ? g + 1 : (t + 1) * kGroupsPerTile];
+  uint2 d = a.pk[min(p, a.n - 1)];
+  if (p >= a.n) d = make_uint2(0xFFFFFFFFu, 0);
+  if (!has_head) {
+    const uint32_t g = t * kGroupsPerTile + (kWaveStage ? (tid >> 6) : 0u);
+    const uint64_t x0 = a.tile_off[g], x1 = a.tile_off[kWaveStage ? g + 1 : (t + 1) * kGroupsPerTile];
+    w0 = kWaveStage ? wave_uniform(x0) : x0;
+    w1 = kWaveStage ? wave_uniform(x1) : x1;
+  }
+  constexpr uint32_t kSV = kWaveStage ? StageGeom<STG>::kWaveSV : 1u, kSW = 64;
+  const uint64_t base16 = w0 & ~uint64_t(15);
+  const bool staged = w1 - base16 <= (kWaveStage ? STG / 4 : STG);
+  const uint32_t nv = staged ? uint32_t((w1 - base16 + 15) / 16) : 0u;
+  uint4 wv[kSV];
+  if constexpr (kWaveStage) window_issue<kSV, kSW>(wv, a.arena + base16, nv, tid & 63);
   if constexpr (kBal) {
     if (tid < kEncBuckets) u.pr.bal_cnt[tid] = 0;
     if (tid == kEncBuckets) u.pr.bal_mixed = 0;
@@ -1019,8 +1057,6 @@
   const uint32_t nlen = d.y & 0xFFFFu, vlen = d.y >> 16;
   uint32_t off = 0;
   uint4* sbuf = buf;
-  const uint64_t base16 = w0 & ~uint64_t(15);
-  bool staged;
   const bool own = p < a.n && d.x < a.db.n_plats;
   ProbePre pre;
   pre.h = pre.start = 0;
@@ -1031,8 +1067,7 @@
   if constexpr (kWaveStage) {
     off = wave_exscan(nlen + vlen, tid & 63);
     sbuf = buf + (tid >> 6) * (STG / 4 / 16 + 2);
-    staged = w1 - base16 <= STG / 4;
-    if (staged) stage_window_wave<STG>(sbuf, a.arena + base16, uint32_t((w1 - base16 + 15) / 16), tid & 63);
+    window_store<kSV, kSW, false>(sbuf, wv, nv, tid & 63);
     if (tid < 128) u.pr.tab[tid] = deb_fast_code(tid);
     if constexpr (kBal) {
       if (!staged) {
@@ -1059,8 +1094,7 @@
     __syncthreads();
   } else {
     block_exscan<kTile>(s.wsum[0], nlen + vlen, tid, off);
-    staged = w1 - base16 <= STG;
-    if (staged) stage_window<STG>(buf, a.arena + base16, uint32_t((w1 - base16 + 15) / 16), tid);
+    if (staged) stage_window<STG>(buf, a.arena + base16, nv, tid);
     if (tid < 128) u.pr.tab[tid] = deb_fast_code(tid);
     __syncthreads();
   }
```

After: 11.56 billion packages/s (median of 6 runs). 1.04x the previous value.
